# mdolab/dafoam

Hardware: AMD Instinct MI355X
Metric: adjoint_gmres_iterations_per_sec (higher is better)
Workload: dtype f64

## Files before the change

dafoam_amd/_capi.py:

```python
from __future__ import annotations

import ctypes as C
import os

import numpy as np

from .meshgen import FoamCase

_HERE = os.path.dirname(os.path.abspath(__file__))
LIB_PATH = os.environ.get("DAFOAM_AMD_LIB") or os.path.join(_HERE, "lib", "libdafoam_amd.so")

SOLVER_IDS = {"DASimpleFoam": 0, "DAScalarTransportFoam": 1, "DARhoSimpleFoam": 2, "DATurboFoam": 3}
PATCH_TYPES = {"patch": 0, "wall": 1, "symmetry": 2, "cyclic": 3}

c_double_p = C.POINTER(C.c_double)
c_int_p = C.POINTER(C.c_int)
c_ll_p = C.POINTER(C.c_longlong)


class das_case_t(C.Structure):
    _fields_ = [
        ("solver", C.c_int),
        ("n_points", C.c_int),
        ("n_faces", C.c_int),
# ... 193 lines not shown
    "das_op_format_bytes": (C.c_longlong, [_VP]),
    "das_op_export": (C.c_int, [_VP, c_ll_p, c_int_p, c_double_p]),
    "das_calc_drdwold_t_psi": (C.c_int, [_VP, C.c_int, c_double_p, c_double_p]),
    "das_set_old_time_fields": (C.c_int, [_VP, c_double_p, c_double_p]),
    "das_calc_jac_vec_product": (C.c_int, [_VP, c_double_p, c_double_p]),
    "das_set_patch_value": (C.c_int, [_VP, c_int_p, C.c_int, C.c_char_p, c_double_p]),
    "das_get_patch_value": (C.c_int, [_VP, C.c_int, C.c_char_p, c_double_p]),
    "das_set_field": (C.c_int, [_VP, C.c_char_p, c_double_p]),
    "das_get_field": (C.c_int, [_VP, C.c_char_p, c_double_p]),
    "das_calc_dfield_product": (C.c_int, [_VP, C.c_char_p, C.c_char_p, C.c_char_p, c_double_p, c_double_p]),
    "das_calc_dvolcoord_product": (C.c_int, [_VP, C.c_char_p, C.c_char_p, c_double_p, c_double_p, c_double_p]),
    "das_point_influence_build": (C.c_int, [_VP, C.POINTER(C.c_int), C.POINTER(C.c_longlong)]),
    "das_point_influence_get": (C.c_int, [_VP, c_int_p, c_ll_p, c_int_p, c_double_p]),
    "das_debug_device_geometry": (C.c_int, [_VP, c_double_p, c_double_p, c_double_p]),
    "das_debug_strength_aggregates": (C.c_int, [_VP, C.c_int, c_int_p, C.POINTER(C.c_int)]),
    "das_calc_dbc_product": (C.c_int, [_VP, c_int_p, C.c_int, C.c_char_p, c_double_p, C.c_char_p, C.c_char_p, c_double_p, c_double_p]),
    "das_define_force_function": (C.c_int, [_VP, C.c_char_p, c_int_p, C.c_int, c_double_p, C.c_double]),
    "das_define_face_function": (C.c_int, [_VP, C.c_char_p, C.c_char_p, c_int_p, c_int_p, C.c_int, c_double_p, c_double_p, C.c_double, C.c_double]),
    "das_define_patch_field_function": (C.c_int, [_VP, C.c_char_p, C.c_char_p, c_int_p, C.c_int, C.c_char_p, c_int_p, C.c_int, c_double_p, C.c_int, C.c_double, C.c_double]),
    "das_define_cell_function": (C.c_int, [_VP, C.c_char_p, C.c_char_p, c_int_p, C.c_int, C.c_char_p, c_int_p, C.c_int, c_double_p, C.c_int, C.c_double, C.c_double]),
    "das_calc_function": (C.c_int, [_VP, C.c_char_p, c_double_p]),
    "das_get_input_size": (C.c_int, [_VP, C.c_char_p, C.c_char_p]),
    "das_get_output_size": (C.c_int, [_VP, C.c_char_p, C.c_char_p]),
    "das_calc_jac_t_vec_product": (
        C.c_int,
        [_VP, C.c_char_p, C.c_char_p, c_double_p, C.c_char_p, C.c_char_p, c_double_p, c_double_p],
    ),
    "das_drdwt_mult_device": (C.c_int, [_VP, _VP, _VP]),
    "das_create_ml_rksp_matrix_free": (C.c_int, [_VP, _VP, C.POINTER(_VP)]),
    "das_solve_linear_eqn": (C.c_int, [_VP, _VP, c_double_p, c_double_p]),
    "das_solve_linear_eqn_block": (C.c_int, [_VP, _VP, C.c_int, c_double_p, c_double_p, c_double_p, c_double_p]),
    "das_ksp_apply_pc": (C.c_int, [_VP, _VP, c_double_p, c_double_p]),
    "das_ksp_get_n_blocks": (C.c_int, [_VP]),
    "das_ksp_get_factor_nnz": (C.c_longlong, [_VP]),
    "das_ksp_get_n_ext": (C.c_longlong, [_VP]),
    "das_ksp_get_blocks": (C.c_int, [_VP, c_int_p, c_ll_p]),
    "das_pc_structure_build": (C.c_int, [_VP, c_int_p, c_ll_p, c_int_p, c_int_p]),
    "das_pc_structure_get": (C.c_int, [_VP, c_int_p, c_ll_p, c_int_p, c_int_p, c_int_p]),
    "das_ksp_get_pc_structure_sizes": (C.c_int, [_VP, c_int_p, c_ll_p, c_int_p]),
    "das_ksp_get_pc_structure": (C.c_int, [_VP, c_int_p, c_ll_p, c_int_p, c_int_p, c_int_p]),
    "das_ksp_get_info": (C.c_int, [_VP, c_int_p, c_double_p, c_double_p, c_double_p]),
    "das_ksp_get_history": (C.c_int, [_VP, c_double_p, C.c_int]),
    "das_ksp_get_cycle_lengths": (C.c_int, [_VP, c_int_p, C.c_int]),
    "das_ksp_get_basis_info": (C.c_int, [_VP, c_int_p, c_double_p, c_double_p]),
    "das_ksp_get_n_refine": (C.c_int, [_VP]),
    "das_set_dense_eig_callback": (C.c_int, [_VP]),
    "das_debug_gmres_dr_host": (C.c_int, [C.c_longlong, _VP, _VP, _VP, c_double_p, c_double_p, C.c_int, C.c_int, C.c_double, C.c_double, C.c_longlong, c_double_p, C.c_int,
                                          c_double_p, c_double_p]),
    "das_debug_gmres_dr_restart": (C.c_int, [C.c_int, C.c_int, c_double_p, c_double_p, c_double_p, c_double_p, c_double_p]),
    "das_ksp_get_status": (C.c_int, [_VP, c_int_p, c_int_p, c_int_p, c_int_p]),
    "das_ksp_get_pc_stability": (C.c_int, [_VP, C.POINTER(C.c_double), c_int_p]),
    "das_ksp_get_pc_subdomains": (C.c_int, [_VP, c_int_p, c_double_p]),
    "das_ksp_get_pc_node_out": (C.c_int, [_VP, c_int_p]),
    "das_mesh_metrics": (C.c_int, [C.c_int, c_double_p, C.c_int, C.c_int, C.c_int, c_int_p, c_int_p, c_int_p, c_int_p, c_double_p, c_double_p, c_double_p, c_double_p, c_double_p]),
    "das_ksp_get_coarse": (C.c_int, [_VP, c_int_p]),
    "das_ksp_coarse_sparse_az_active": (C.c_int, [_VP]),
    "das_ksp_set_global_coarse": (C.c_int, [_VP, _VP, C.c_int, C.c_int, c_int_p]),
    "das_ksp_run_fixed_device": (C.c_int, [_VP, _VP, _VP, _VP, C.c_int]),
    "das_ksp_begin_device": (C.c_int, [_VP, _VP, _VP, _VP, C.c_int]),
    "das_ksp_advance": (C.c_int, [_VP, _VP, C.c_int]),
    "das_ksp_end": (C.c_int, [_VP, _VP]),
    "das_ksp_destroy": (None, [_VP]),
    "das_set_owned_mask": (C.c_int, [_VP, C.POINTER(C.c_ubyte)]),
    "das_comm_load_rccl": (C.c_int, []),
    "das_comm_unique_id": (C.c_int, [C.c_char_p]),
    "das_comm_init_rccl": (C.c_int, [_VP, C.c_int, C.c_int, C.c_char_p]),
    "das_comm_set_halo": (C.c_int, [_VP, C.c_int, c_int_p, c_ll_p, c_int_p, c_ll_p, c_int_p, C.c_longlong, c_int_p]),
    "das_set_exchange_cb": (C.c_int, [_VP, _VP, _VP]),
    "das_set_pc_overlap": (C.c_int, [_VP, C.POINTER(C.c_ubyte), C.c_int, c_ll_p, c_int_p, c_ll_p, c_int_p]),
    "das_set_gather_cb": (C.c_int, [_VP, _VP, _VP]),
    "das_comm_is_native": (C.c_int, [_VP]),
    "das_comm_reset": (C.c_int, [_VP]),
    "das_set_comm": (C.c_int, [_VP, _VP, _VP, _VP]),
    "das_set_stream": (C.c_int, [_VP, _VP]),
    "das_get_elapsed_clock_time": (C.c_double, [_VP]),
    "das_get_elapsed_cpu_time": (C.c_double, [_VP]),
    "das_timer_avg_ms": (C.c_double, [_VP, C.c_char_p]),
    "das_debug_orth_bench": (C.c_int, [C.c_longlong, C.c_int, C.c_int, C.c_int, C.c_int, C.c_int, C.POINTER(C.c_double), C.POINTER(C.c_double)]),
    "das_debug_orth_bench_split": (C.c_int, [C.c_longlong, C.c_int, C.c_int, C.c_int, C.c_int, C.c_int, C.c_int, C.c_int, C.POINTER(C.c_double), C.POINTER(C.c_double)]),
    "das_debug_set_orth_wide": (C.c_int, [C.c_int, C.POINTER(C.c_int)]),
    "das_debug_krylov_wide_eligible": (C.c_int, [C.c_longlong, C.c_int, C.c_longlong, C.POINTER(C.c_int), C.POINTER(C.c_int)]),
    "das_debug_krylov_dots2": (C.c_int, [C.c_longlong, C.c_int, C.c_int, _VP, C.c_longlong, c_double_p, c_double_p]),
    "das_debug_krylov_dcgs2_update": (C.c_int, [C.c_longlong, C.c_int, C.c_int, _VP, C.c_longlong, C.c_int, c_double_p, C.c_double, C.c_double, c_double_p]),
    "das_debug_krylov_multidot": (C.c_int, [C.c_longlong, C.c_int, C.c_int, _VP, C.c_longlong, c_double_p, c_double_p]),
    "das_debug_krylov_multiaxpy": (C.c_int, [C.c_longlong, C.c_int, C.c_int, _VP, C.c_longlong, c_double_p, C.c_int, _VP, C.c_longlong]),
    "das_debug_krylov_lincomb": (C.c_int, [C.c_longlong, C.c_int, C.c_int, _VP, C.c_longlong, c_double_p, c_double_p, C.c_longlong]),
    "das_debug_krylov_scale_to": (C.c_int, [C.c_longlong, C.c_double, C.c_int, _VP, _VP, C.c_longlong]),
    "das_debug_krylov_block_tn": (C.c_int, [C.c_longlong, C.c_int, C.c_int, c_double_p, C.c_longlong, C.c_longlong, c_double_p, C.c_longlong, c_double_p]),
    "das_debug_krylov_block_nn_sub": (C.c_int, [C.c_longlong, C.c_int, C.c_int, c_double_p, C.c_longlong, c_double_p, c_double_p, C.c_longlong]),
    "das_debug_krylov_block_right_mult": (C.c_int, [C.c_longlong, C.c_int, c_double_p, C.c_longlong, c_double_p]),
    "das_debug_krylov_block_lincomb": (C.c_int, [C.c_longlong, C.c_int, C.c_int, c_double_p, C.c_longlong, c_double_p, c_double_p, C.c_longlong]),
    "das_debug_krylov_block_spmm": (C.c_int, [C.c_longlong, C.c_int, c_ll_p, c_int_p, c_double_p, c_double_p, C.c_longlong, c_double_p, C.c_longlong]),
    "das_timer_count": (C.c_longlong, [_VP, C.c_char_p]),
    "das_timer_reset": (None, [_VP]),
    "das_timer_enable": (None, [_VP, C.c_int]),
}

_lib = None


def declared_symbols():
    return sorted(_SIGS)


def lib():
    global _lib
    if _lib is None:
        if not os.path.exists(LIB_PATH):
            raise ImportError(
                f"{LIB_PATH} not found: build the HIP extension first (python -c 'import __graft_entry__ as g; g.build()'). "
                "dafoam_amd has no CPU fallback."
            )
        L = C.CDLL(LIB_PATH)
        for name, (res, args) in _SIGS.items():
            fn = getattr(L, name)
            fn.restype = res
            fn.argtypes = args
        _lib = L
        _install_dense_eig(L)
    return _lib


_DENSE_EIG_FN = C.CFUNCTYPE(C.c_int, C.c_int, c_double_p, c_double_p, c_double_p, c_double_p, c_double_p)
_dense_eig_keepalive = []


def _install_dense_eig(L):

    def eig(m, A, wr, wi, vr, vi):
        try:
            G = np.ctypeslib.as_array(A, shape=(m * m,)).reshape(m, m)
            w, v = np.linalg.eig(G)
            np.ctypeslib.as_array(wr, shape=(m,))[:] = w.real
            np.ctypeslib.as_array(wi, shape=(m,))[:] = w.imag
            np.ctypeslib.as_array(vr, shape=(m * m,))[:] = np.ascontiguousarray(v.T.real).ravel()
            np.ctypeslib.as_array(vi, shape=(m * m,))[:] = np.ascontiguousarray(v.T.imag).ravel()
            return 0
        except Exception:
            return 1

    cb = _DENSE_EIG_FN(eig)
    _dense_eig_keepalive.append(cb)
    L.das_set_dense_eig_callback(C.cast(cb, C.c_void_p))


class DASError(RuntimeError):
    pass


def check(rc):
    if rc < 0:
        raise DASError(f"dafoam_amd error {rc}: {lib().das_last_error().decode()}")
    return rc


def dptr(a: np.ndarray):
    assert a.dtype == np.float64 and a.flags["C_CONTIGUOUS"]
    return a.ctypes.data_as(c_double_p)
```

dafoam_amd/csrc/das_device.hip:

```cpp
#include <algorithm>
#include <cmath>
#include <ctime>
#include <functional>
#include <numeric>
#include <thread>

#include "das_case.hpp"
#include "das_jaccon.hpp"
#include "das_bilu.hpp"
#include "das_comm.hpp"
#include "das_krylov.hpp"
#include "das_block.hpp"
#include "das_krylov_debug.hpp"
#include "das_color.hpp"
#include "das_opmat.hpp"
#include "das_graph.hpp"
#include "das_volcoord.hpp"
#include "das_cellfn.hpp"
#include "das_simple.hpp"

#include <omp.h>

namespace das {

// ... 395 lines not shown
    if (i >= n0 && i < n1 && w < 1e-14) w = 1e-14;
    Wn[i] = w;
}

__global__ __launch_bounds__(256) void k_coarse_assemble(int nagg, const long long* __restrict__ aptrAll, const int* __restrict__ cellsAll, long long N,
                                                         long long off, const long long* __restrict__ rp, const int* __restrict__ ci,
                                                         const double* __restrict__ v, const int* __restrict__ aggCol, double* __restrict__ E,
                                                         int transpose, double diagScale) {
    __shared__ double accs[2048];
    const int I = blockIdx.x, t = threadIdx.x;
    const long long q0 = aptrAll[I], q1 = aptrAll[I + 1];
    if (q0 == q1) return;
    for (int J = t; J < nagg; J += 256) accs[J] = 0.0;
    for (long long q = q0; q < q1; q++) {
        const long long c = cellsAll[q];
        const long long row = off + c;
        for (long long k = rp[row]; k < rp[row + 1]; k++) {
            const long long j = (long long)ci[k] - off;
            if (j < 0 || j >= N) continue;
            const int J = aggCol[j];
            if (J >= 0 && (J & 255) == t) accs[J] += (j == c) ? v[k] * diagScale : v[k];
        }
    }
    for (int J = t; J < nagg; J += 256) E[transpose ? (long long)J * nagg + I : (long long)I * nagg + J] = accs[J];
}
__global__ __launch_bounds__(256) void k_gj_pivot(int n, int k, double* __restrict__ E, double* __restrict__ Inv, int* __restrict__ singular) {
    __shared__ double bv[256];
    __shared__ int bi[256];
    double best = -1.0;
    int br = k;
    for (int r = k + threadIdx.x; r < n; r += 256) { const double a = fabs(E[(long long)r * n + k]); if (a > best) { best = a; br = r; } }
    bv[threadIdx.x] = best; bi[threadIdx.x] = br;
    __syncthreads();
    for (int o = 128; o > 0; o >>= 1) {
        if ((int)threadIdx.x < o && (bv[threadIdx.x + o] > bv[threadIdx.x] || (bv[threadIdx.x + o] == bv[threadIdx.x] && bi[threadIdx.x + o] < bi[threadIdx.x]))) {
            bv[threadIdx.x] = bv[threadIdx.x + o]; bi[threadIdx.x] = bi[threadIdx.x + o];
        }
        __syncthreads();
    }
    const int pr = bi[0];
    if (!(bv[0] > 0.0)) { if (threadIdx.x == 0) *singular = 1; return; }
    const double ip = 1.0 / E[(long long)pr * n + k];
    __syncthreads();
    for (int q = threadIdx.x; q < n; q += 256) {
        const double ek = E[(long long)k * n + q], ep = E[(long long)pr * n + q];
        const double ik = Inv[(long long)k * n + q], ipr = Inv[(long long)pr * n + q];
        if (pr != k) { E[(long long)pr * n + q] = ek; Inv[(long long)pr * n + q] = ik; }
        E[(long long)k * n + q] = ep * ip;
        Inv[(long long)k * n + q] = ipr * ip;
    }
}
__global__ __launch_bounds__(256) void k_gj_elim(int n, int k, double* __restrict__ E, double* __restrict__ Inv) {
    const int r = blockIdx.x;
    if (r == k) return;
    __shared__ double fs;
    if (threadIdx.x == 0) fs = E[(long long)r * n + k];
    __syncthreads();
    const double f = fs;
    if (f == 0.0) return;
    for (int q = threadIdx.x; q < n; q += 256) {
        E[(long long)r * n + q] -= f * E[(long long)k * n + q];
        Inv[(long long)r * n + q] -= f * Inv[(long long)k * n + q];
    }
}
__global__ __launch_bounds__(256) void k_coarse_restrict(const long long* __restrict__ aptr, const int* __restrict__ cells, long long off,
                                                         const double* __restrict__ r, double* __restrict__ t) {
    __shared__ double red[4];
    const int I = blockIdx.x;
    double acc = 0.0;
    for (long long q = aptr[I] + threadIdx.x; q < aptr[I + 1]; q += 256) acc += r[off + cells[q]];
#pragma unroll
    for (int o = 32; o > 0; o >>= 1) acc += __shfl_down(acc, o, 64);
    if ((threadIdx.x & 63) == 0) red[threadIdx.x >> 6] = acc;
    __syncthreads();
    if (threadIdx.x == 0) t[I] = red[0] + red[1] + red[2] + red[3];
}
__global__ void k_coarse_solve(int nagg, const double* __restrict__ Einv, const double* __restrict__ t, double* __restrict__ u) {
    const int I = blockIdx.x * blockDim.x + threadIdx.x;
    if (I >= nagg) return;
    double acc = 0.0;
    for (int J = 0; J < nagg; J++) acc += Einv[(long long)I * nagg + J] * t[J];
    u[I] = acc;
}
__global__ void k_coarse_prolong(long long N, long long n, long long off, const int* __restrict__ agg, const double* __restrict__ u,
                                 double* __restrict__ y, int set) {
    const long long i = (long long)blockIdx.x * blockDim.x + threadIdx.x;
    if (i >= n) return;
    const long long c = i - off;
    const double add = (c >= 0 && c < N && agg[c] >= 0) ? u[agg[c]] : 0.0;
    y[i] = set ? add : y[i] + add;
}

constexpr int AZ_CAP = 64;
__global__ __launch_bounds__(256) void k_az_build(long long n, const long long* __restrict__ rp, const int* __restrict__ ci, const double* __restrict__ v,
                                                  long long N, long long off, const int* __restrict__ agg, int pass, int* __restrict__ cnt,
                                                  const long long* __restrict__ ptr, int* __restrict__ oa, double* __restrict__ ov, int* __restrict__ overflow) {
    const long long i = (long long)blockIdx.x * blockDim.x + threadIdx.x;
    if (i >= n) return;
    int la[AZ_CAP];
    double ls[AZ_CAP];
    int m = 0;
    for (long long k = rp[i]; k < rp[i + 1]; k++) {
        const long long j = (long long)ci[k] - off;
        if (j < 0 || j >= N) continue;
        const int a = agg[j];
        if (a < 0) continue;
        int q = 0;
        while (q < m && la[q] != a) q++;
        if (q == m) {
            if (m == AZ_CAP) { *overflow = 1; continue; }
            la[m] = a; ls[m] = 0.0; m++;
        }
        ls[q] += v[k];
    }
    if (pass == 0) { cnt[i] = m; return; }
    const long long b = ptr[i];
    for (int q = 0; q < m; q++) { oa[b + q] = la[q]; ov[b + q] = ls[q]; }
}
__global__ __launch_bounds__(256) void k_az_apply(long long n, const long long* __restrict__ ptr, const int* __restrict__ oa, const double* __restrict__ ov,
                                                  const double* __restrict__ u, const double* __restrict__ v, double* __restrict__ out) {
    const long long i = (long long)blockIdx.x * blockDim.x + threadIdx.x;
    if (i >= n) return;
    double acc = 0.0;
    for (long long k = ptr[i]; k < ptr[i + 1]; k++) acc += ov[k] * u[oa[k]];
    out[i] = v ? v[i] - acc : acc;
}

#ifndef PC_THREADS
#define PC_THREADS 1024
#endif
#ifndef PC_PF
#define PC_PF 8
#endif
struct PCView {
    int nBlocks;
    const long long* boff;
    const int* gidx;
    const int* gout;
    const double* invd;
    int factor32;
    const double* sval[2];
    const float* svalf[2];
    const unsigned* srowcol[2];
    const long long* slev[2];
    const long long* slevOff[2];
    double* xglob;
};

#ifndef PC_SEGREDUCE
#define PC_SEGREDUCE 1
#endif
template <int CTRL>
__device__ __forceinline__ unsigned dpp_u32(unsigned v, unsigned old) {
    return (unsigned)__builtin_amdgcn_update_dpp((int)old, (int)v, CTRL, 0xF, 0xF, false);
}
template <int CTRL>
__device__ __forceinline__ double dpp_f64(double v) {
    int lo = __builtin_amdgcn_update_dpp(0, __double2loint(v), CTRL, 0xF, 0xF, false);
    int hi = __builtin_amdgcn_update_dpp(0, __double2hiint(v), CTRL, 0xF, 0xF, false);
    return __hiloint2double(hi, lo);
}
template <bool USE_LDS>
__device__ __forceinline__ void ras_apply_entry(double* xw, double v, unsigned rc, bool valid) {
#if PC_SEGREDUCE
    const unsigned key = valid ? (rc & 0xffffu) : (0x10000u + (threadIdx.x & 63u));
    double val = valid ? -v * xw[rc >> 16] : 0.0;
    unsigned k;
    double w;
    k = dpp_u32<0x111>(key, 0xffffffffu); w = dpp_f64<0x111>(val); if (k == key) val += w;
    k = dpp_u32<0x112>(key, 0xffffffffu); w = dpp_f64<0x112>(val); if (k == key) val += w;
    k = dpp_u32<0x114>(key, 0xffffffffu); w = dpp_f64<0x114>(val); if (k == key) val += w;
    k = dpp_u32<0x118>(key, 0xffffffffu); w = dpp_f64<0x118>(val); if (k == key) val += w;
    const unsigned knext = dpp_u32<0x101>(key, 0xffffffffu);
    if (valid && knext != key) {
        if (USE_LDS) __hip_atomic_fetch_add(&xw[key], val, __ATOMIC_RELAXED, __HIP_MEMORY_SCOPE_WORKGROUP);
        else atomicAdd(&xw[key], val);
    }
#else
    if (!valid) return;
    const double contrib = -v * xw[rc >> 16];
#ifdef PC_EXP_NOATOMIC
    xw[rc & 0xffffu] = contrib;
#else
    if (USE_LDS) __hip_atomic_fetch_add(&xw[rc & 0xffffu], contrib, __ATOMIC_RELAXED, __HIP_MEMORY_SCOPE_WORKGROUP);
    else atomicAdd(&xw[rc & 0xffffu], contrib);
#endif
#endif
}

template <class VT> struct RingVal;
template <> struct RingVal<float> {
    unsigned a;
    __device__ __forceinline__ void load(const float* __restrict__ p, int e) { a = __float_as_uint(p[e]); }
    __device__ __forceinline__ double get() const { return (double)__uint_as_float(a); }
    __device__ __forceinline__ void clear() { a = 0u; }
};
template <> struct RingVal<double> {
    unsigned lo, hi;
    __device__ __forceinline__ void load(const double* __restrict__ p, int e) {
        const unsigned* __restrict__ q = reinterpret_cast<const unsigned*>(p);
        lo = q[2 * (long long)e];
        hi = q[2 * (long long)e + 1];
    }
    __device__ __forceinline__ double get() const { return __hiloint2double((int)hi, (int)lo); }
    __device__ __forceinline__ void clear() { lo = 0u; hi = 0u; }
};

template <bool USE_LDS, class VT>
// ... 83 lines not shown
        if (!on) return;
        hipEvent_t b = get();
        DAS_HIP(hipEventRecord(b, st));
        recs[name].pending.push_back({a, b});
    }
    void resolve() {
        for (auto& kv : recs) {
            for (auto& pr : kv.second.pending) {
                DAS_HIP(hipEventSynchronize(pr.second));
                float ms = 0;
                DAS_HIP(hipEventElapsedTime(&ms, pr.first, pr.second));
                kv.second.ms += ms;
                kv.second.cnt++;
                pool.push_back(pr.first);
                pool.push_back(pr.second);
            }
            kv.second.pending.clear();
        }
    }
    void reset() { resolve(); for (auto& kv : recs) { kv.second.ms = 0; kv.second.cnt = 0; } }
};

struct ConDev {
    bool ready = false;
    bool onDevice = false;
    DevBuf<long long> t_rowptr;
    DevBuf<int> cl_cols;
    DevBuf<int> t_col;
};

struct BlockILU {
    long long n = 0, next = 0;
    int nBlocks = 0;
    long long fnnz = 0;
    int maxLocal = 0;
    DevBuf<long long> boff, slev[2], slevOff[2];
    DevBuf<int> gidx, gout;
    DevBuf<unsigned> srowcol[2];
    DevBuf<double> sval[2], invd, xw;
    DevBuf<float> svalf[2];
    bool factor32 = false;
    PCView view;
    int maxLevels = 0;
    bool useLDS = false;
    double setup_seconds = 0;
    std::vector<int> h_core_perm;
    std::vector<long long> h_core_off;
};

}

using namespace das;

struct das_mat {
    Mat m;
};

struct das_ksp {
    das_mat* pcmat = nullptr;
    BlockILU pc;
    NodeILU bilu;
    bool useBilu = false;
    bool pcTranspose = false;
    double pcDiagScale = 1.0;
    long long shiftExLo = 0, shiftExHi = 0, shiftEnd = (long long)1 << 62;
    struct CoarsePC {
        bool active = false, deflated = false;
        bool global = false;
        int nagg = 0;
        int naggG = 0, aggOff = 0;
        long long off = 0, N = 0;
        DevBuf<int> agg;
        DevBuf<int> aggRow;
        DevBuf<int> cells, cellsAll;
        DevBuf<long long> aptr, aptrAll;
        DevBuf<double> Einv, t, u, c, rr;
        std::vector<int> h_agg;
        DevBuf<long long> azPtr;
        DevBuf<int> azAgg;
        DevBuf<double> azVal;
        long long azOpId = -1;
        long long azEpoch = -1, azNnz = 0;
        bool azReady = false, azFailed = false;
    } coarse;
    int restart = 0;
    VmBuf<double> V;
    long long Vn = 0;
    bool vf32 = false;
    bool split = false;
    DevBuf<double> ustage;
    DevBuf<double> w, z, r, xdev, bdev, partial, hdev, rich_r, rich_d;
    int nSub = 1;
    std::vector<int> subOrder;
    std::vector<double> subEst;
    int pcOrder = -1;
    int pcOrderUsed = -1;
    double pcStability = -1.0;
    bool rasOverlap = false;
    DevBuf<double> pcin;
    std::unique_ptr<struct GmresRun> run;
    std::unique_ptr<struct BlockWork> block;
    std::vector<double> block_res0, block_res;
    int iters = 0, nrefine = 0, reason = 0, nBreakdown = 0;
    double res0 = 0, res = 0, seconds = 0;
    std::vector<double> hist;
    std::vector<int> cycleLens;
};

struct das_solver {
    Mesh mesh;
    CaseParams cp;
    Options opt;
    int device = -1;
    bool inited = false;
    long long n = 0;
    Stencil st_full, st_pc;
    JacCon con_full, con_pc;
    std::vector<int> colors;
    int nColors = 0;
    bool colored = false;
    DevBuf<FaceGeom> d_fg;
    DevBuf<CellGeom> d_cg;
    DevBuf<int> d_cf_ptr, d_cf_face, d_cf_other, d_owner, d_neigh, d_bpatch, d_cyc;
    DevBuf<PatchBC> d_bc;
    DevBuf<double> d_phiF, d_Told;
    DevMesh dm;
    DevBuf<double> d_W, d_R, d_R0, d_Wp, d_scale, d_tmp1, d_tmp2;
    DevBuf<int> d_colors;
    std::vector<double> h_W, h_scale;
    ResWork<double> wk;
    ResWork<Dual<1>> wk1;
    DevBuf<Dual<1>> d_Wd, d_Rd;
    ConDev cd[2];
    std::unique_ptr<das_mat> op;
    std::vector<double> op_states;
    long long op_geom = -1;
    struct FaceFn {
        int kind = DAS_FN_FORCE;
        bool ratio = false;
        double gammaFn = 1.4, RFn = 287.0;
        std::vector<int> faces;
        std::vector<unsigned char> group;
        std::vector<double> w0, dir;
        DevBuf<int> d_faces;
        DevBuf<unsigned char> d_group;
        DevBuf<double> d_w0, d_weff, d_dir, d_fv;
        bool uploaded = false;
        bool isMoment = false;
        double vecA[3] = {0, 0, 0}, vecB[3] = {0, 0, 0}, scale = 1.0;
        long long geomVersion = -1;
        bool refVar = false, geoWeight = false, hasData = true;
        double ref = 0.0;
        int ncomp = 1;
        FaceFnView view(const double* w) const {
            return FaceFnView{d_faces.p, d_group.p, w, dir.empty() ? nullptr : d_dir.p, (int)faces.size(), kind, gammaFn, RFn};
        }
    };
    std::map<std::string, FaceFn> functions;
    struct CellFn {
        bool variance = false, square = false, multiplyVol = true, divByTotalVol = false, refVar = false, geoWeight = false, hasData = true;
        bool field = false;
        double scale = 1.0, ref = 0.0;
        double coef = 0.0, totalVol = 1.0;
        long long geomVersion = -1;
        std::vector<int> cell;
        std::vector<long long> idx;
        std::vector<double> data;
        DevBuf<int> d_cell;
        DevBuf<long long> d_idx;
        DevBuf<double> d_data, d_part, d_unit;
        bool uploaded = false;
        CellFnView view() const {
            return CellFnView{(long long)cell.size(), d_cell.p, d_idx.p, data.empty() ? nullptr : d_data.p, (int)square, (int)multiplyVol};
// ... 956 lines not shown
    }
    auto fill_mask = [&](const std::vector<unsigned char>& cellIn, std::vector<unsigned char>& out) {
        out.assign(n, 0);
        for (const StateDef& sd : s->st_full.states) {
            if (sd.kind == KIND_VEC) { for (long long c = 0; c < N; c++) if (cellIn[c]) { out[sd.offset + 3 * c] = out[sd.offset + 3 * c + 1] = out[sd.offset + 3 * c + 2] = 1; } }
            else if (sd.kind == KIND_SCL) { for (long long c = 0; c < N; c++) if (cellIn[c]) out[sd.offset + c] = 1; }
            else { for (long long f = 0; f < m.nF; f++) if (cellIn[m.owner[f]]) out[sd.offset + f] = 1; }
        }
    };
    std::vector<unsigned char> subOf(n, 0);
    for (const StateDef& sd : s->st_full.states) {
        if (sd.kind == KIND_VEC) { for (long long c = 0; c < N; c++) for (int q = 0; q < 3; q++) subOf[sd.offset + 3 * c + q] = (unsigned char)blockOf[c]; }
        else if (sd.kind == KIND_SCL) { for (long long c = 0; c < N; c++) subOf[sd.offset + c] = (unsigned char)blockOf[c]; }
        else { for (long long f = 0; f < m.nF; f++) subOf[sd.offset + f] = (unsigned char)blockOf[m.owner[f]]; }
    }
    const int overlap = (int)std::max<long long>(0, s->opt.geti("adjEqnOption.asmOverlap"));
    std::vector<std::vector<unsigned char>> masks(K);
    k->subOrder.assign(K, -1);
    k->subEst.assign(K, -1.0);
    for (int b = 0; b < K; b++) {
        std::vector<unsigned char> cellIn(N, 0), grown;
        for (long long c = 0; c < N; c++) cellIn[c] = blockOf[c] == b;
        for (int ring = 0; ring < overlap; ring++) {
            grown = cellIn;
            for (long long c = 0; c < N; c++) if (cellIn[c]) for (int q = m.cc_ptr[c]; q < m.cc_ptr[c + 1]; q++) grown[m.cc[q]] = 1;
            cellIn.swap(grown);
        }
        fill_mask(cellIn, masks[b]);
        NodeILU F;
        choose_order_and_factorise(s, k, F, masks[b], true, k->subOrder[b], k->subEst[b]);
        if (k->subOrder[b] < 0) k->subOrder[b] = k->pcOrder >= 0 ? k->pcOrder : (pc_ordering_rcm(s) ? 1 : 0);
        if (s->opt.geti("debug") || getenv("DAS_PC_STAB"))
            fprintf(stderr, "[dafoam_amd] sub-domain %d of %d: %d nodes, %d levels, elimination order %d, stability estimate %.3e\n", b, K, F.nNodes, F.nLevels, k->subOrder[b], k->subEst[b]);
        if ((double)F.nLevels > 30.0 * std::cbrt((double)std::max(1, F.nNodes)) && s->opt.geti("amd.pcSubdomains") < 0) {
            fprintf(stderr, "[dafoam_amd] sub-domain %d of %d needs %d dependency levels for %d nodes: the blocks do not suit this mesh, one factorisation instead "
                            "(amd.pcSubdomains K > 1 forces the blocks)\n", b, K, F.nLevels, F.nNodes);
            k->subOrder.clear(); k->subEst.clear();
            return false;
        }
    }
    {
        const Mat& A = k->pcmat->m;
        const int reach = pc_stencil_reach(s);
        const int nthr = (int)std::max<long long>(1, std::min<long long>(das::host_threads(), s->opt.geti("amd.setupThreads")));
        double dir[3];
        pc_flow_direction(s, dir);
        std::vector<const std::vector<unsigned char>*> mp;
        for (int b = 0; b < K; b++) mp.push_back(&masks[b]);
        k->bilu = NodeILU();
        bilu_setup_multi(s->mesh, s->st_full.states, n, mp, k->subOrder, subOf, reach, s->opt.geti("amd.pcFactorFP32") != 0, A.n, A.rowptr.p, A.col.p, A.val.p, s->stream, k->bilu,
                         s->opt.geti("debug") != 0, nthr, dir);
    }
    k->nSub = K;
    k->useBilu = true;
    k->rasOverlap = false;
    k->pcOrderUsed = k->subOrder[0];
    k->pcStability = 0.0;
    for (double e : k->subEst) k->pcStability = std::max(k->pcStability, e);
    k->pc.setup_seconds = wall_seconds() - t0;
    k->pc.nBlocks = K;
    k->pc.fnnz = (k->bilu.nL + k->bilu.nU + k->bilu.nNodes) * (long long)BILU_NB2;
    k->pc.next = (long long)k->bilu.nNodes * BILU_NB;
    if (s->opt.geti("debug") || getenv("DAS_PC_STAB"))
        fprintf(stderr, "[dafoam_amd] %d sub-domains merged: %d nodes, %d levels (%.0f nodes per level)\n", K, k->bilu.nNodes, k->bilu.nLevels, (double)k->bilu.nNodes / std::max(1, k->bilu.nLevels));
    return true;
}

static void coarse_build_operator(das_solver* s, das_ksp* k, int naggG, int aggOff, const std::vector<int>& aggRowG) {
    das_ksp::CoarsePC& C = k->coarse;
    C.active = false;
    DAS_CHECK(naggG >= C.nagg && naggG <= 2048, DAS_ERR_ARG, "coarse space: at most 2048 aggregates in total (dense inverse)");
    const long long N = C.N;
    std::vector<int> aggOwn(N, -1);
    for (long long c = 0; c < N; c++) if (C.h_agg[c] >= 0) aggOwn[c] = aggOff + C.h_agg[c];
    std::vector<long long> aptrAll(naggG + 1, 0);
    for (long long c = 0; c < N; c++) if (aggRowG[c] >= 0) aptrAll[aggRowG[c] + 1]++;
    for (int a = 0; a < naggG; a++) aptrAll[a + 1] += aptrAll[a];
    std::vector<int> cellsAll(aptrAll[naggG]);
    {
        std::vector<long long> pos(aptrAll.begin(), aptrAll.end() - 1);
        for (long long c = 0; c < N; c++) if (aggRowG[c] >= 0) cellsAll[pos[aggRowG[c]]++] = (int)c;
    }
    C.naggG = naggG; C.aggOff = aggOff; C.global = naggG > C.nagg;
    C.azOpId = -1; C.azReady = false;
    C.agg.upload(aggOwn); C.aggRow.upload(aggRowG); C.cellsAll.upload(cellsAll); C.aptrAll.upload(aptrAll);
    DevBuf<double> E((size_t)naggG * naggG);
    E.zero();
    const Mat& P = k->pcmat->m;
    hipLaunchKernelGGL(k_coarse_assemble, dim3(naggG), dim3(256), 0, s->stream, naggG, C.aptrAll.p, C.cellsAll.p, N, C.off, P.rowptr.p, P.col.p, P.val.p,
                       k->pcTranspose ? C.aggRow.p : C.agg.p, E.p, k->pcTranspose ? 1 : 0,
                       (C.off < k->shiftEnd && !(C.off >= k->shiftExLo && C.off < k->shiftExHi)) ? k->pcDiagScale : 1.0);
    if (C.global) {
        DAS_CHECK(!k->pcTranspose, DAS_ERR_ARG, "global coarse space: adjoint preconditioner only");
        rank_allreduce(s, E.p, naggG * naggG, s->stream);
    }
    {
        std::vector<double> I0((size_t)naggG * naggG, 0.0);
        for (int i = 0; i < naggG; i++) I0[(size_t)i * naggG + i] = 1.0;
        C.Einv.upload(I0);
        DevBuf<int> sing(1);
        DAS_HIP(hipMemsetAsync(sing.p, 0, sizeof(int), s->stream));
        for (int kk = 0; kk < naggG; kk++) {
            hipLaunchKernelGGL(k_gj_pivot, dim3(1), dim3(256), 0, s->stream, naggG, kk, E.p, C.Einv.p, sing.p);
            hipLaunchKernelGGL(k_gj_elim, dim3(naggG), dim3(256), 0, s->stream, naggG, kk, E.p, C.Einv.p);
        }
        int hs = 0;
        DAS_HIP(hipMemcpyAsync(&hs, sing.p, sizeof(int), hipMemcpyDeviceToHost, s->stream));
        DAS_HIP(hipStreamSynchronize(s->stream));
        if (hs) return;
    }
    C.t.alloc(naggG); C.u.alloc(naggG);
    C.active = true;
}

static void setup_coarse(das_solver* s, das_ksp* k) {
    das_ksp::CoarsePC& C = k->coarse;
    C.active = false;
    long long want = s->opt.geti("amd.pcCoarseAggregates");
    if (want == 0) return;
    const std::string field = s->opt.gets("amd.pcCoarseField");
    const StateDef* sd = nullptr;
    for (const StateDef& q : s->st_full.states) if (q.name == field && q.kind == KIND_SCL) sd = &q;
    if (!sd) return;
    const Mesh& m = s->mesh;
    const long long N = m.nC;
    std::vector<int> owned;
    owned.reserve(N);
    for (long long c = 0; c < N; c++) if (s->owned.empty() || s->owned[sd->offset + c]) owned.push_back((int)c);
    if (owned.size() < 64) return;
    if (want < 0) want = std::min<long long>(1024, std::max<long long>(16, (long long)owned.size() / 2048));
    int nagg = (int)std::min<long long>(want, std::min<long long>(2048, (long long)owned.size() / 4));
    if (nagg < 2) return;
    std::vector<int> agg(N, -1);
    const bool byStrength = s->opt.gets("amd.pcCoarseAggregation") == "strength";
    DAS_CHECK(byStrength || s->opt.gets("amd.pcCoarseAggregation") == "rcb", DAS_ERR_ARG, "amd.pcCoarseAggregation: rcb | strength");
    if (byStrength) {
        std::vector<unsigned char> mask;
        if (!s->owned.empty()) { mask.resize(N); for (long long c = 0; c < N; c++) mask[c] = s->owned[sd->offset + c]; }
        nagg = strength_aggregates(m, s->owned.empty() ? nullptr : &mask, nagg, agg);
        if (nagg < 2) return;
    } else {
        struct Rg { long long b, e; int a0, na; };
        std::vector<Rg> stack{{0, (long long)owned.size(), 0, nagg}};
        while (!stack.empty()) {
            Rg r = stack.back();
            stack.pop_back();
            if (r.na == 1) { for (long long q = r.b; q < r.e; q++) agg[owned[q]] = r.a0; continue; }
            double lo[3] = {1e300, 1e300, 1e300}, hi[3] = {-1e300, -1e300, -1e300};
            for (long long q = r.b; q < r.e; q++)
                for (int d = 0; d < 3; d++) { const double x = m.cg[owned[q]].C[d]; lo[d] = std::min(lo[d], x); hi[d] = std::max(hi[d], x); }
            int ax = 0;
            for (int d = 1; d < 3; d++) if (hi[d] - lo[d] > hi[ax] - lo[ax]) ax = d;
            const int nl = r.na / 2;
            const long long mid = r.b + (r.e - r.b) * nl / r.na;
            std::nth_element(owned.begin() + r.b, owned.begin() + mid, owned.begin() + r.e, [&](int a, int b2) {
                const double xa = m.cg[a].C[ax], xb = m.cg[b2].C[ax];
                return xa < xb || (xa == xb && a < b2);
            });
            stack.push_back({mid, r.e, r.a0 + nl, r.na - nl});
            stack.push_back({r.b, mid, r.a0, nl});
        }
    }
    std::vector<long long> aptr(nagg + 1, 0);
    for (long long c = 0; c < N; c++) if (agg[c] >= 0) aptr[agg[c] + 1]++;
    for (int a = 0; a < nagg; a++) aptr[a + 1] += aptr[a];
    std::vector<int> cells(aptr[nagg]);
    {
        std::vector<long long> pos(aptr.begin(), aptr.end() - 1);
        for (long long c = 0; c < N; c++) if (agg[c] >= 0) cells[pos[agg[c]]++] = (int)c;
    }
    C.nagg = nagg; C.off = sd->offset; C.N = N; C.h_agg = agg;
    C.cells.upload(cells); C.aptr.upload(aptr);
    C.deflated = s->opt.gets("amd.pcCoarseMode") == "deflated";
    if (C.deflated) { C.c.alloc(s->n); C.rr.alloc(s->n); }
    coarse_build_operator(s, k, nagg, 0, agg);
    if (C.active && s->opt.geti("debug")) fprintf(stderr, "[dafoam_amd] coarse space: %d aggregates on field %s (%s)\n", nagg, field.c_str(), C.deflated ? "deflated" : "additive");
}
static void coarse_solve(das_solver* s, das_ksp* k, const double* r) {
    das_ksp::CoarsePC& C = k->coarse;
    if (C.global) DAS_HIP(hipMemsetAsync(C.t.p, 0, (size_t)C.naggG * sizeof(double), s->stream));
    if (C.nagg > 0) hipLaunchKernelGGL(k_coarse_restrict, dim3(C.nagg), dim3(256), 0, s->stream, C.aptr.p, C.cells.p, C.off, r, C.t.p + C.aggOff);
    if (C.global) rank_allreduce(s, C.t.p, C.naggG, s->stream);
    hipLaunchKernelGGL(k_coarse_solve, dim3(nblk(C.naggG, 64)), dim3(64), 0, s->stream, C.naggG, C.Einv.p, C.t.p, C.u.p);
}

static void pc_apply(das_solver* s, das_ksp* k, const double* b, double* x) {
    hipEvent_t ev = nullptr;
    s->timer.begin("pc", s->stream, ev);
    if (k->useBilu) {
        if (k->rasOverlap) {
            DAS_HIP(hipMemcpyAsync(k->pcin.p, b, (size_t)s->n * sizeof(double), hipMemcpyDeviceToDevice, s->stream));
            s->halo.gather_overlap(k->pcin.p, s->stream);
            bilu_apply(k->bilu, k->pcin.p, x, s->stream);
            s->halo.zero_overlap(x, s->stream);
        } else {
            bilu_apply(k->bilu, b, x, s->stream);
        }
        s->timer.end("pc", s->stream, ev);
        return;
    }
    const int mlv = k->pc.maxLevels;
    const size_t lvlBytes = (size_t)((mlv + 2 * PC_PF + 4) >> 1) * sizeof(double);
    if (k->pc.useLDS)
        hipLaunchKernelGGL(k_ras_apply<true>, dim3(k->pc.nBlocks), dim3(PC_THREADS), lvlBytes + (size_t)k->pc.maxLocal * sizeof(double), s->stream,
                           k->pc.view, b, x, mlv);
    else
        hipLaunchKernelGGL(k_ras_apply<false>, dim3(k->pc.nBlocks), dim3(PC_THREADS), lvlBytes, s->stream, k->pc.view, b, x, mlv);
    s->timer.end("pc", s->stream, ev);
}

static void gmres_ws(das_solver* s, das_ksp* k) {
    const long long n = s->n;
    long long restart = std::min<long long>(s->opt.geti("adjEqnOption.gmresRestart"), s->opt.geti("adjEqnOption.gmresMaxIters"));
    long long budget = (long long)(32.0 * 1024 * 1024 * 1024);
    auto it = s->opt.i.find("amd.maxKrylovBytes");
    if (it != s->opt.i.end()) budget = it->second;
    const long long nr = (n + 3) / 4 * 4;
    const long long maxVec = std::max<long long>(3, budget / (8 * nr));
    restart = std::max<long long>(1, std::min<long long>(restart, maxVec - 2));
    long long wantVec = std::max<long long>(restart + 2, std::min<long long>(maxVec, 1002));
    if ((size_t)wantVec * (size_t)nr * sizeof(double) < ((size_t)4 << 30) || getenv("DAS_NO_VMM")) wantVec = restart + 2;
    if (k->V.n < (size_t)((restart + 2) * nr) || k->Vn != n) {
        k->V.reserve((size_t)(wantVec * nr));
        k->Vn = n;
    }
    {
        std::string prec = "auto";
        { auto ip = s->opt.s.find("amd.krylovBasisPrecision"); if (ip != s->opt.s.end()) prec = ip->second; }
        DAS_CHECK(prec == "auto" || prec == "fp64" || prec == "fp32" || prec == "split", DAS_ERR_ARG, "amd.krylovBasisPrecision: auto | fp64 | split | fp32");
        const bool eligible = s->opt.geti("adjEqnOption.useMGSO") == 0 && !s->fwd.on;
        const bool dcgs2 = s->opt.gets("amd.gmresOrthogonalization") == "dcgs2" && s->opt.geti("adjEqnOption.useMGSO") == 0;
        bool big = (size_t)(restart + 2) * (size_t)n * 8 >= ((size_t)1 << 30);
        if (s->halo.active || s->allreduce_cb) {
            DevBuf<double> f(1);
            const double fv = big ? 1.0 : 0.0;
            DAS_HIP(hipMemcpyAsync(f.p, &fv, sizeof(double), hipMemcpyHostToDevice, s->stream));
            rank_allreduce(s, f.p, 1, s->stream);
            DAS_HIP(hipStreamSynchronize(s->stream));
            big = f.to_host()[0] > 0.5;
        }
        k->split = eligible && (prec == "split" || (prec == "auto" && dcgs2 && big));
        k->vf32 = k->split || (eligible && prec == "fp32");
        if (k->vf32 && k->ustage.n != (size_t)n) k->ustage.alloc(n);
    }
    if (k->restart != restart || k->w.n != (size_t)n) {
        k->restart = (int)restart;
        k->w.alloc(n); k->z.alloc(n); k->r.alloc(n); k->xdev.alloc(n); k->bdev.alloc(n);
        k->z.zero();
        k->partial.alloc(std::max<size_t>(multidot_partial_size(n, (int)restart + 1), multidot2_partial_size(n, (int)restart + 2)));
        k->hdev.alloc(4 * (restart + 3));
    }
}
static inline long long basis_n4(das_solver* s) { return (s->n + 3) / 4 * 4; }
static inline long long basis_ld(das_solver* s, das_ksp* k) { return k->split ? 2 * basis_n4(s) : (k->vf32 ? basis_n4(s) : s->n); }
static inline bool gmres_map_basis(das_solver* s, das_ksp* k, long long nvec) {
    const long long per = basis_ld(s, k) / (k->vf32 ? 2 : 1);
    k->V.request((size_t)((nvec + 64) * per));
    return k->V.try_ensure((size_t)(nvec * per));
}
template <class VT>
static inline VT* basis_slot(das_solver* s, das_ksp* k, long long j) { return reinterpret_cast<VT*>(k->V.p) + j * basis_ld(s, k); }
static inline float* basis_lo(das_solver* s, das_ksp* k, long long j) { return k->split ? reinterpret_cast<float*>(k->V.p) + j * basis_ld(s, k) + basis_n4(s) : nullptr; }

template <class VT>
static void multidot_dev(das_solver* s, das_ksp* k, const VT* Vbase, int m, const double* w, double* dev_out) {
    launch_multidot<VT>(s->stream, s->n, m, Vbase, basis_ld(s, k), w, k->partial.p, dev_out);
    rank_allreduce(s, dev_out, m + 1, s->stream);
}
template <class VT = double>
static void multidot(das_solver* s, das_ksp* k, int m, const double* w, double* h_host) {
    multidot_dev<VT>(s, k, basis_slot<VT>(s, k, 0), m, w, k->hdev.p);
    DAS_HIP(hipMemcpyAsync(h_host, k->hdev.p, (m + 1) * sizeof(double), hipMemcpyDeviceToHost, s->stream));
    DAS_HIP(hipStreamSynchronize(s->stream));
}

static void apply_operator(das_solver* s, const double* x, double* y);

static bool coarse_az_ready(das_solver* s, das_ksp* k) {
    das_ksp::CoarsePC& C = k->coarse;
    if (!s->op || s->fwd.on) return false;
    { auto it = s->opt.i.find("amd.pcCoarseSparseAZ"); if (it != s->opt.i.end() && it->second == 0) return false; }
    const Mat& A = s->op->m;
    if (C.azOpId == s->opId && C.azEpoch == s->op_epoch) return C.azReady;
    C.azOpId = s->opId; C.azEpoch = s->op_epoch; C.azReady = false; C.azFailed = false;
    const long long n = s->n;
    hipStream_t st = s->stream;
    DevBuf<int> cnt(n), ovf(1);
    DAS_HIP(hipMemsetAsync(ovf.p, 0, sizeof(int), st));
    hipLaunchKernelGGL(k_az_build, dim3(nblk(n, 256)), dim3(256), 0, st, n, A.rowptr.p, A.col.p, A.val.p, C.N, C.off, C.agg.p, 0, cnt.p, (const long long*)nullptr,
                       (int*)nullptr, (double*)nullptr, ovf.p);
    DAS_HIP(hipStreamSynchronize(st));
    int ovfAny = ovf.to_host()[0];
    if (s->halo.active || s->allreduce_cb) {
        DevBuf<double> f(1);
        const double fv = ovfAny ? 1.0 : 0.0;
        DAS_HIP(hipMemcpyAsync(f.p, &fv, sizeof(double), hipMemcpyHostToDevice, st));
        rank_allreduce(s, f.p, 1, st);
        DAS_HIP(hipStreamSynchronize(st));
        ovfAny = f.to_host()[0] > 0.5 ? 1 : 0;
    }
    if (ovfAny) {
        C.azFailed = true;
        fprintf(stderr, "[dafoam_amd] deflated coarse mode: a row of the operator touches more than %d aggregates - keeping the full operator product per apply\n", AZ_CAP);
        return false;
    }
    std::vector<int> h = cnt.to_host();
    std::vector<long long> ptr(n + 1, 0);
    for (long long i = 0; i < n; i++) ptr[i + 1] = ptr[i] + h[i];
    C.azNnz = ptr[n];
    C.azPtr.upload(ptr);
    C.azAgg.alloc((size_t)std::max<long long>(1, C.azNnz)); C.azVal.alloc((size_t)std::max<long long>(1, C.azNnz));
    hipLaunchKernelGGL(k_az_build, dim3(nblk(n, 256)), dim3(256), 0, st, n, A.rowptr.p, A.col.p, A.val.p, C.N, C.off, C.agg.p, 1, cnt.p, C.azPtr.p, C.azAgg.p, C.azVal.p,
                       ovf.p);
    DAS_HIP(hipStreamSynchronize(st));
    if (s->opt.geti("debug")) fprintf(stderr, "[dafoam_amd] deflated coarse mode: sparse A Z with %lld entries (%.2f per row)\n", C.azNnz, (double)C.azNnz / (double)n);
    C.azReady = true;
    return true;
}

static void pc_apply_full(das_solver* s, das_ksp* k, const double* v, double* z) {
    const long long sweeps = std::max<long long>(1, s->opt.geti("adjEqnOption.globalPCIters")) * std::max<long long>(1, s->opt.geti("adjEqnOption.localPCIters"));
    const long long n = s->n;
    das_ksp::CoarsePC& C = k->coarse;
    if (C.active) {
        hipEvent_t ev = nullptr;
        s->timer.begin("coarse", s->stream, ev);
        coarse_solve(s, k, v);
        if (C.deflated && (s->op || s->fwd.on)) {
            hipLaunchKernelGGL(k_coarse_prolong, dim3(nblk(n, 256)), dim3(256), 0, s->stream, C.N, n, C.off, C.agg.p, C.u.p, C.c.p, 1);
            if (coarse_az_ready(s, k)) {
                if (s->halo.active || s->halo_cb) {
                    hipLaunchKernelGGL(k_az_apply, dim3(nblk(n, 256)), dim3(256), 0, s->stream, n, C.azPtr.p, C.azAgg.p, C.azVal.p, C.u.p, (const double*)nullptr, C.rr.p);
                    if (s->halo.active) s->halo.reduce_vector(C.rr.p, s->stream);
                    else s->halo_cb(C.rr.p, s->comm_user);
                    hipLaunchKernelGGL(k_axpby, dim3(nblk(n, 256)), dim3(256), 0, s->stream, n, 1.0, v, -1.0, C.rr.p);
                } else {
                    hipLaunchKernelGGL(k_az_apply, dim3(nblk(n, 256)), dim3(256), 0, s->stream, n, C.azPtr.p, C.azAgg.p, C.azVal.p, C.u.p, v, C.rr.p);
                }
                s->timer.end("coarse", s->stream, ev);
            } else {
                s->timer.end("coarse", s->stream, ev);
                apply_operator(s, C.c.p, C.rr.p);
                hipLaunchKernelGGL(k_axpby, dim3(nblk(n, 256)), dim3(256), 0, s->stream, n, 1.0, v, -1.0, C.rr.p);
            }
            pc_apply(s, k, C.rr.p, z);
            hipLaunchKernelGGL(k_axpby, dim3(nblk(n, 256)), dim3(256), 0, s->stream, n, 1.0, C.c.p, 1.0, z);
        } else {
            s->timer.end("coarse", s->stream, ev);
            pc_apply(s, k, v, z);
            hipLaunchKernelGGL(k_coarse_prolong, dim3(nblk(n, 256)), dim3(256), 0, s->stream, C.N, n, C.off, C.agg.p, C.u.p, z, 0);
        }
    } else {
        pc_apply(s, k, v, z);
    }
    if (sweeps <= 1) return;
    if (k->rich_r.n != (size_t)n) { k->rich_r.alloc(n); k->rich_d.alloc(n); k->rich_d.zero(); }
    const Mat& P = k->pcmat->m;
    for (long long it = 1; it < sweeps; it++) {
        hipLaunchKernelGGL(k_spmv_wave, SPMV_GRID(P.n), dim3(256), 0, s->stream, P.n, P.rowptr.p, P.col.p, P.val.p, z, k->rich_r.p);
        hipLaunchKernelGGL(k_axpby, dim3(nblk(n, 256)), dim3(256), 0, s->stream, n, 1.0, v, -1.0, k->rich_r.p);
        pc_apply(s, k, k->rich_r.p, k->rich_d.p);
        hipLaunchKernelGGL(k_axpby, dim3(nblk(n, 256)), dim3(256), 0, s->stream, n, 1.0, k->rich_d.p, 1.0, z);
    }
}

static void pc_apply_block(das_solver* s, das_ksp* k, const double* V, double* Z, int sv) {
    const long long n = s->n;
    const long long sweeps = std::max<long long>(1, s->opt.geti("adjEqnOption.globalPCIters")) * std::max<long long>(1, s->opt.geti("adjEqnOption.localPCIters"));
    das_ksp::CoarsePC& C = k->coarse;
    const bool batched = k->useBilu && sweeps <= 1 && !(C.active && C.deflated) && sv > 1 && s->opt.geti("amd.blockBatchedPC") != 0;
    if (!batched) {
        for (int r = 0; r < sv; r++) pc_apply_full(s, k, V + (size_t)r * n, Z + (size_t)r * n);
        return;
    }
    hipEvent_t ev = nullptr;
    s->timer.begin("pc", s->stream, ev);
    bilu_apply_multi(k->bilu, V, Z, n, sv, s->stream);
    s->timer.end("pc", s->stream, ev);
    if (C.active)
        for (int r = 0; r < sv; r++) {
            coarse_solve(s, k, V + (size_t)r * n);
            hipLaunchKernelGGL(k_coarse_prolong, dim3(nblk(n, 256)), dim3(256), 0, s->stream, C.N, n, C.off, C.agg.p, C.u.p, Z + (size_t)r * n, 0);
        }
}

static void apply_operator(das_solver* s, const double* x, double* y) {
    if (!s->fwd.on) { spmv(s, s->op->m, x, y); return; }
    const long long n = s->n;
    const int B = 256;
    hipStream_t st = s->stream;
    hipEvent_t ev = nullptr;
    s->timer.begin("jvp", st, ev);
    ResParams prm = make_params(s->cp, s->opt, 0);
    if (s->d_Wd.n != (size_t)n) { s->d_Wd.alloc(n); s->d_Rd.alloc(n); }
    hipLaunchKernelGGL(k_seed_dir, dim3(nblk(n, B)), dim3(B), 0, st, n, s->d_W.p, s->d_scale.p, x, s->d_Wd.p);
    eval_residual<Dual<1>>(s->dm, s->cp, prm, s->d_Wd.p, s->d_Rd.p, s->wk1, s->d_phiF.p, s->d_Told.p, st);
    hipLaunchKernelGGL(k_tangent_out, dim3(nblk(n, B)), dim3(B), 0, st, n, s->d_Rd.p, y);
    if (s->fwd.invTau != 0.0) hipLaunchKernelGGL(k_add_diag_prod, dim3(nblk(n, B)), dim3(B), 0, st, n, s->fwd.invTau, s->fwd.diag.p, x, y);
    s->timer.end("jvp", st, ev);
}

struct GmresRun {
    bool open = false;
    bool fixed = false;
    int m = 0, j = 0;
    bool memWarned = false;
    long long its = 0, maxIts = 0;
    double beta = 0, target = 0, rtol = 0, atol = 0, t0 = 0;
    double recTarget = 0;
    const double* d_rhs = nullptr;
    double* d_x = nullptr;
    std::vector<double> H, cs, sn, g, hh, h2, y;
    bool dcgs2 = false;
    int pend = 0;
    std::vector<double> Hraw, h1;
    bool earlyClose = false;
    bool safeOrth = false;
    bool stalled = false;
    int nonImproving = 0, nBreakdown = 0;
    double betaStart = 0;
};
static bool gmres_trace() { static const bool on = [] { const char* e = getenv("DAS_GMRES_TRACE"); return e && *e && *e != '0'; }(); return on; }
static constexpr double GMRES_BREAKDOWN_TOL = 1e-13;

static void gmres_true_residual(das_solver* s, das_ksp* k, GmresRun& G, bool haveGuess) {
    const long long n = s->n;
    hipStream_t st = s->stream;
    if (haveGuess) {
        apply_operator(s, G.d_x, k->r.p);
        hipLaunchKernelGGL(k_axpby, dim3(nblk(n, 256)), dim3(256), 0, st, n, 1.0, G.d_rhs, -1.0, k->r.p);
    } else {
        DAS_HIP(hipMemsetAsync(G.d_x, 0, n * sizeof(double), st));
        DAS_HIP(hipMemcpyAsync(k->r.p, G.d_rhs, n * sizeof(double), hipMemcpyDeviceToDevice, st));
    }
    multidot(s, k, 0, k->r.p, G.hh.data());
    G.beta = std::sqrt(G.hh[0]);
}

static void gmres_begin(das_solver* s, das_ksp* k, const double* d_rhs, double* d_x, bool fixed) {
    need_init(s);
    DAS_CHECK(s->op || s->fwd.on, DAS_ERR_STATE, "initializedRdWTMatrixFree() must be called before solveLinearEqn()");
    gmres_ws(s, k);
    if (k->useBilu) bilu_clear_abort(k->bilu, s->stream);
    if (!k->run) k->run.reset(new GmresRun);
    GmresRun& G = *k->run;
    const int m = k->restart;
    G = GmresRun();
    G.m = m; G.fixed = fixed; G.d_rhs = d_rhs; G.d_x = d_x;
    G.maxIts = s->opt.geti("adjEqnOption.gmresMaxIters");
    G.rtol = s->opt.getd("adjEqnOption.gmresRelTol"); G.atol = s->opt.getd("adjEqnOption.gmresAbsTol");
    G.H.assign((size_t)(m + 1) * m, 0.0); G.cs.assign(m, 0.0); G.sn.assign(m, 0.0); G.g.assign(m + 1, 0.0);
    G.hh.assign(2 * (m + 2), 0.0); G.h2.assign(2 * (m + 2), 0.0); G.y.assign(m, 0.0);
    const std::string& orth = s->opt.gets("amd.gmresOrthogonalization");
    DAS_CHECK(orth == "dcgs2" || orth == "cgs", DAS_ERR_ARG, "amd.gmresOrthogonalization \"" + orth + "\" is not one of dcgs2 | cgs");
    G.dcgs2 = orth == "dcgs2" && s->opt.geti("adjEqnOption.useMGSO") == 0;
    if (G.dcgs2) { G.Hraw.assign((size_t)(m + 1) * m, 0.0); G.h1.assign(m + 2, 0.0); }
    k->nrefine = 0;
    k->hist.clear();
    k->cycleLens.clear();
    G.t0 = wall_seconds();
    gmres_true_residual(s, k, G, s->opt.geti("adjEqnOption.useNonZeroInitGuess") != 0);
    k->res0 = G.beta;
    k->hist.push_back(G.beta);
    G.target = std::max(G.rtol * G.beta, G.atol);
    G.recTarget = k->split ? 0.98 * G.target : (k->vf32 ? 0.5 * G.target : G.target);
}
static void gmres_cycle_start(das_solver* s, das_ksp* k) {
    GmresRun& G = *k->run;
    const long long n = s->n;
    DAS_CHECK(gmres_map_basis(s, k, 3), DAS_ERR_INTERNAL, "GMRES: no device memory for three Krylov vectors (" + k->V.workerError + ")");
    if (k->vf32) launch_scale_to(s->stream, n, 1.0 / G.beta, (const double*)k->r.p, basis_slot<float>(s, k, 0), (const float*)nullptr, basis_lo(s, k, 0));
    else launch_scale_to(s->stream, n, 1.0 / G.beta, (const double*)k->r.p, (double*)k->V.p, (const float*)nullptr, (float*)nullptr);
    std::fill(G.g.begin(), G.g.end(), 0.0);
    G.g[0] = G.beta;
    G.j = 0;
    G.pend = 0;
    G.open = true;
    G.earlyClose = false;
    G.betaStart = G.beta;
}
template <class VT>
static const double* basis_as_double(das_solver* s, das_ksp* k, long long j) {
    if (sizeof(VT) == sizeof(double)) return reinterpret_cast<const double*>(basis_slot<VT>(s, k, j));
    launch_scale_to(s->stream, s->n, 1.0, (const VT*)basis_slot<VT>(s, k, j), (double*)k->ustage.p, (const float*)basis_lo(s, k, j), (float*)nullptr);
    return k->ustage.p;
}
template <class VT>
static double gmres_iter_dcgs2(das_solver* s, das_ksp* k);
template <class VT>
static double gmres_iter_t(das_solver* s, das_ksp* k) {
    GmresRun& G = *k->run;
    if (G.dcgs2 && !G.safeOrth) return gmres_iter_dcgs2<VT>(s, k);
    const long long n = s->n;
    const int B = 256, m = G.m, j = G.j;
    hipStream_t st = s->stream;
    const bool alwaysRefine = s->opt.geti("amd.cgsAlwaysRefine") != 0;
    const bool mgs = s->opt.geti("adjEqnOption.useMGSO") != 0;
    std::vector<double>&H = G.H, &hh = G.hh, &h2 = G.h2, &cs = G.cs, &sn = G.sn, &g = G.g;
    VT* const Vb = basis_slot<VT>(s, k, 0);
    const long long ld = basis_ld(s, k);
    pc_apply_full(s, k, basis_as_double<VT>(s, k, j), k->z.p);
    apply_operator(s, k->z.p, k->w.p);
    double hn;
    std::fill(h2.begin(), h2.end(), 0.0);
    if (mgs) {
        double* hcol = k->hdev.p + (m + 2);
        for (int i = 0; i <= j; i++) {
            multidot_dev<VT>(s, k, Vb + (long long)i * ld, 1, k->w.p, k->hdev.p);
            DAS_HIP(hipMemcpyAsync(hcol + i, k->hdev.p, sizeof(double), hipMemcpyDeviceToDevice, st));
            launch_multiaxpy(st, n, 1, (const VT*)(Vb + (long long)i * ld), ld, (const double*)k->hdev.p, (double*)k->w.p, (const float*)basis_lo(s, k, i));
        }
        multidot_dev<VT>(s, k, Vb, 0, k->w.p, k->hdev.p);
        DAS_HIP(hipMemcpyAsync(hcol + j + 1, k->hdev.p, sizeof(double), hipMemcpyDeviceToDevice, st));
        DAS_HIP(hipMemcpyAsync(hh.data(), hcol, (j + 2) * sizeof(double), hipMemcpyDeviceToHost, st));
        DAS_HIP(hipStreamSynchronize(st));
        hn = std::sqrt(std::max(hh[j + 1], 0.0));
    } else {
        multidot<VT>(s, k, j + 1, k->w.p, hh.data());
        launch_multiaxpy(st, n, j + 1, (const VT*)Vb, ld, (const double*)k->hdev.p, (double*)k->w.p, (const float*)basis_lo(s, k, 0));
        double hsq = 0.0;
        for (int i = 0; i <= j; i++) hsq += hh[i] * hh[i];
        const double ww = hh[j + 1];
        const double est = ww - hsq;
        if (alwaysRefine || !(est > hsq) || !(est > 0.0)) {
            multidot<VT>(s, k, j + 1, k->w.p, h2.data());
            launch_multiaxpy(st, n, j + 1, (const VT*)Vb, ld, (const double*)k->hdev.p, (double*)k->w.p, (const float*)basis_lo(s, k, 0));
            double hn2;
            multidot<VT>(s, k, 0, k->w.p, &hn2);
            hn = std::sqrt(std::max(hn2, 0.0));
            k->nrefine++;
        } else {
            hn = std::sqrt(est);
        }
    }
    if (!mgs && !(hn > GMRES_BREAKDOWN_TOL * std::sqrt(std::max(hh[j + 1], 0.0)))) { hn = 0.0; G.nBreakdown++; }
    for (int i = 0; i <= j; i++) H[(size_t)i * m + j] = hh[i] + h2[i];
    H[(size_t)(j + 1) * m + j] = hn;
    if (hn > 0.0) launch_scale_to(st, n, 1.0 / hn, (const double*)k->w.p, Vb + (long long)(j + 1) * ld, (const float*)nullptr, basis_lo(s, k, j + 1));
    for (int i = 0; i < j; i++) {
        double a = H[(size_t)i * m + j], b2 = H[(size_t)(i + 1) * m + j];
        H[(size_t)i * m + j] = cs[i] * a + sn[i] * b2;
        H[(size_t)(i + 1) * m + j] = -sn[i] * a + cs[i] * b2;
    }
    double a = H[(size_t)j * m + j], b2 = H[(size_t)(j + 1) * m + j];
    double d = std::hypot(a, b2);
    cs[j] = d > 0 ? a / d : 1.0;
    sn[j] = d > 0 ? b2 / d : 0.0;
    H[(size_t)j * m + j] = d;
    H[(size_t)(j + 1) * m + j] = 0.0;
    g[j + 1] = -sn[j] * g[j];
    g[j] = cs[j] * g[j];
    G.its++;
    G.j++;
    const double res = std::fabs(g[G.j]);
    k->hist.push_back(res);
    if (hn == 0.0) { G.j = -G.j; G.earlyClose = true; }
    return res;
}
static double gmres_iter(das_solver* s, das_ksp* k) { return k->vf32 ? gmres_iter_t<float>(s, k) : gmres_iter_t<double>(s, k); }
static double gmres_rotate_column(GmresRun& G, int col) {
    const int m = G.m;
    std::vector<double>&H = G.H, &cs = G.cs, &sn = G.sn, &g = G.g;
    for (int i = 0; i < col; i++) {
        const double a = H[(size_t)i * m + col], b2 = H[(size_t)(i + 1) * m + col];
        H[(size_t)i * m + col] = cs[i] * a + sn[i] * b2;
        H[(size_t)(i + 1) * m + col] = -sn[i] * a + cs[i] * b2;
    }
    const double a = H[(size_t)col * m + col], b2 = H[(size_t)(col + 1) * m + col];
    const double d = std::hypot(a, b2);
    cs[col] = d > 0 ? a / d : 1.0;
    sn[col] = d > 0 ? b2 / d : 0.0;
    H[(size_t)col * m + col] = d;
    H[(size_t)(col + 1) * m + col] = 0.0;
    g[col + 1] = -sn[col] * g[col];
    g[col] = cs[col] * g[col];
    return std::fabs(g[col + 1]);
}
template <class VT>
static double gmres_iter_dcgs2(das_solver* s, das_ksp* k) {
    GmresRun& G = *k->run;
    const long long n = s->n;
    const int m = G.m, j = G.pend;
    hipStream_t st = s->stream;
    VT* const Vb = basis_slot<VT>(s, k, 0);
    const long long ld = basis_ld(s, k);
    VT* u = Vb + (long long)j * ld;
    pc_apply_full(s, k, basis_as_double<VT>(s, k, j), k->z.p);
    apply_operator(s, k->z.p, k->w.p);
    const int K = j + 1;
    launch_multidot2<VT>(st, n, K, (const VT*)Vb, ld, (const VT*)u, (const double*)k->w.p, k->partial.p, k->hdev.p);
    rank_allreduce(s, k->hdev.p, 2 * K, st);
    std::vector<double>& o = G.hh;
    DAS_HIP(hipMemcpyAsync(o.data(), k->hdev.p, 2 * K * sizeof(double), hipMemcpyDeviceToHost, st));
    DAS_HIP(hipStreamSynchronize(st));
    const double* sv = o.data();
    const double* tv = o.data() + K;
    const double uu = sv[j], uv = tv[j];
    double ss = 0.0, stt = 0.0;
    for (int i = 0; i < j; i++) { ss += sv[i] * sv[i]; stt += sv[i] * tv[i]; }
    double al2 = uu - ss, num = uv - stt;
    double normBq2 = uu;
    for (int i = 0; i < j; i++) normBq2 += G.h1[i] * G.h1[i];
    bool explicitProj = false;
    if (j > 0 && !(ss <= 1e-2 * uu)) {
        if (gmres_trace()) fprintf(stderr, "[dafoam_amd] dcgs2 step %d: s.s / u.u = %.3e > 1e-2: explicit projection, cycle closes\n", j, ss / uu);
        double* dsc = k->hdev.p + 2 * (m + 3);
        DAS_HIP(hipMemcpyAsync(dsc, sv, j * sizeof(double), hipMemcpyHostToDevice, st));
        if (k->split) {
            const double* ud = basis_as_double<VT>(s, k, j);
            launch_multiaxpy(st, n, j, (const VT*)Vb, ld, (const double*)dsc, const_cast<double*>(ud), (const float*)basis_lo(s, k, 0));
            launch_scale_to(st, n, 1.0, ud, u, (const float*)nullptr, basis_lo(s, k, j));
        } else {
            launch_multiaxpy(st, n, j, (const VT*)Vb, ld, (const double*)dsc, u, (const float*)nullptr);
        }
        launch_multidot2<VT>(st, n, 1, (const VT*)u, ld, (const VT*)u, (const double*)k->w.p, k->partial.p, k->hdev.p);
        rank_allreduce(s, k->hdev.p, 2, st);
        double cc[2] = {0.0, 0.0};
        DAS_HIP(hipMemcpyAsync(cc, k->hdev.p, 2 * sizeof(double), hipMemcpyDeviceToHost, st));
        DAS_HIP(hipStreamSynchronize(st));
        al2 = cc[0]; num = cc[1];
        explicitProj = true;
        k->nrefine++;
    }
    const bool breakdown = !(al2 > GMRES_BREAKDOWN_TOL * GMRES_BREAKDOWN_TOL * normBq2);
    const double al = breakdown ? 0.0 : std::sqrt(al2);
    double res = k->hist.back();
    if (j == 0) {
        DAS_CHECK(!breakdown, DAS_ERR_INTERNAL, "GMRES: the start vector of an Arnoldi cycle is not finite (preconditioner or operator returned NaN)");
        G.g[0] = G.beta * al;
    } else {
        const int col = j - 1;
        for (int i = 0; i < j; i++) G.Hraw[(size_t)i * m + col] = G.H[(size_t)i * m + col] = G.h1[i] + (breakdown ? 0.0 : sv[i]);
        G.Hraw[(size_t)j * m + col] = G.H[(size_t)j * m + col] = al;
        res = gmres_rotate_column(G, col);
        G.its++;
        G.j = j;
        k->hist.push_back(res);
        if (breakdown || explicitProj) {
            if (breakdown) G.nBreakdown++; else G.safeOrth = true;
            G.j = -G.j; G.earlyClose = true;
            return res;
        }
        const bool stop = !G.fixed && (res <= G.recTarget || G.its >= G.maxIts);
        if (stop || G.j >= m) return res;
    }
    const double gam = num / al2;
    std::vector<double>& co = G.h2;
    for (int i = 0; i < j; i++) { co[i] = sv[i]; co[j + i] = tv[i] - gam * sv[i]; }
    double* dco = k->hdev.p + 2 * (m + 3);
    if (j > 0) DAS_HIP(hipMemcpyAsync(dco, co.data(), 2 * j * sizeof(double), hipMemcpyHostToDevice, st));
    launch_dcgs2_update<DCGS2_UNROLL, DCGS2_RPT, VT>(st, n, j, Vb, ld, (const double*)dco, gam, 1.0 / al, (const double*)k->w.p, basis_lo(s, k, 0));
    for (int i = 0; i < j; i++) {
        double a = tv[i];
        for (int q = std::max(0, i - 1); q < j; q++) a -= G.Hraw[(size_t)i * m + q] * sv[q];
        G.h1[i] = a / al;
    }
    G.h1[j] = gam - (j > 0 ? sv[j - 1] : 0.0);
    G.pend = j + 1;
    return res;
}
template <class VT>
static void gmres_cycle_end_t(das_solver* s, das_ksp* k) {
    GmresRun& G = *k->run;
    const long long n = s->n;
    const int B = 256, m = G.m, j = std::abs(G.j);
    hipStream_t st = s->stream;
    for (int i = j - 1; i >= 0; i--) {
        double sacc = G.g[i];
        for (int q = i + 1; q < j; q++) sacc -= G.H[(size_t)i * m + q] * G.y[q];
        G.y[i] = sacc / G.H[(size_t)i * m + i];
    }
    DAS_HIP(hipMemcpyAsync(k->hdev.p, G.y.data(), j * sizeof(double), hipMemcpyHostToDevice, st));
    launch_lincomb(st, n, j, (const VT*)basis_slot<VT>(s, k, 0), basis_ld(s, k), (const double*)k->hdev.p, (double*)k->w.p, (const float*)basis_lo(s, k, 0));
    pc_apply_full(s, k, k->w.p, k->z.p);
    hipLaunchKernelGGL(k_axpby, dim3(nblk(n, B)), dim3(B), 0, st, n, 1.0, k->z.p, 1.0, G.d_x);
    const double recRes = k->hist.back();
    gmres_true_residual(s, k, G, true);
    k->hist.back() = G.beta;
    k->cycleLens.push_back(j);
    G.open = false;
    if (gmres_trace()) {
        double ymax = 0.0;
        for (int i = 0; i < j; i++) ymax = std::max(ymax, std::fabs(G.y[i]));
        fprintf(stderr, "[dafoam_amd] GMRES cycle closed after %d columns (its %lld): recurrence |r| %.6e, true |r| %.6e (|r0| %.3e), max |y| %.3e, explicit projections %d, basis %s%s\n",
                j, G.its, recRes, G.beta, k->res0, ymax, k->nrefine, k->split ? "split" : (k->vf32 ? "fp32" : "fp64"), G.safeOrth ? ", two-pass scheme from here" : "");
    }
}
static void gmres_cycle_end(das_solver* s, das_ksp* k) {
    if (k->vf32) gmres_cycle_end_t<float>(s, k); else gmres_cycle_end_t<double>(s, k);
}
static bool gmres_over(const GmresRun& G) { return !G.fixed && !G.open && (G.beta <= G.target || G.its >= G.maxIts || G.stalled); }
static bool gmres_advance(das_solver* s, das_ksp* k, long long nsteps) {
    GmresRun& G = *k->run;
    for (long long t = 0; t < nsteps; t++) {
        if (gmres_over(G)) return true;
        if (G.beta == 0.0) return true;
        if (!G.open) gmres_cycle_start(s, k);
        const long long wantSlots = std::min<long long>(((G.dcgs2 && !G.safeOrth) ? G.pend : G.j) + 3, (long long)G.m + 2);
        if (!gmres_map_basis(s, k, wantSlots)) {
            if (k->V.workerError.empty())
                k->V.workerError = "request for " + std::to_string(wantSlots) + " basis vectors beyond the reserved range of " + std::to_string(k->V.n / (size_t)std::max<long long>(1, s->n)) + " (internal)";
            DAS_CHECK(G.j >= 1, DAS_ERR_INTERNAL, "GMRES: the Krylov basis cannot grow beyond its first vectors (" + k->V.workerError + ")");
            if (!G.memWarned) fprintf(stderr, "[dafoam_amd] GMRES restarts after %d vectors: %s\n", G.j, k->V.workerError.c_str());
            G.memWarned = true;
            gmres_cycle_end(s, k);
            t--;
            continue;
        }
        const double res = gmres_iter(s, k);
        const bool stop = !G.fixed && (res <= G.recTarget || G.its >= G.maxIts);
        if (G.j < 0 || G.j >= G.m || stop) {
            const bool judged = G.earlyClose || (res <= G.recTarget && G.its < G.maxIts);
            gmres_cycle_end(s, k);
            if (!G.fixed && judged && G.beta > G.target) {
                if (G.beta < 0.5 * G.betaStart) G.nonImproving = 0;
                else if (++G.nonImproving >= 2) G.stalled = true;
            }
        }
    }
    return gmres_over(G);
}
static int gmres_end(das_solver* s, das_ksp* k) {
    GmresRun& G = *k->run;
    if (G.open) gmres_cycle_end(s, k);
    DAS_HIP(hipStreamSynchronize(s->stream));
    if (k->useBilu) DAS_CHECK(!bilu_aborted(k->bilu, s->stream), DAS_ERR_INTERNAL, "preconditioner sweep timed out (bounded spin)");
    k->iters = (int)G.its;
    k->nBreakdown = G.nBreakdown;
    k->res = k->hist.back();
    k->reason = G.beta <= G.target ? 0 : (G.stalled ? 2 : 1);
    k->seconds = wall_seconds() - G.t0;
    double absRatio = k->res / G.atol;
    double relRatio = k->res0 > 0 ? k->res / k->res0 / G.rtol : 0.0;
    double diff = s->opt.getd("adjEqnOption.gmresTolDiff");
// ... 2251 lines not shown
    DAS_CATCH
}
int das_drdwt_mult_device(das_solver_t* s, const double* d_x, double* d_y) {
    DAS_TRY
    need_init(s);
    DAS_CHECK(s->op, DAS_ERR_STATE, "initializedRdWTMatrixFree() has not been called");
    spmv(s, s->op->m, d_x, d_y);
    return DAS_OK;
    DAS_CATCH
}

int das_create_ml_rksp_matrix_free(das_solver_t* s, das_mat_t* pc, das_ksp_t** ksp) {
    DAS_TRY
    need_init(s);
    DAS_CHECK(pc && ksp, DAS_ERR_ARG, "null argument");
    std::unique_ptr<das_ksp> k(new das_ksp);
    k->pcmat = pc;
    const std::string pcType = s->opt.gets("amd.pcType");
    DAS_CHECK(pcType == "bilu" || pcType == "ras", DAS_ERR_ARG, "amd.pcType must be \"bilu\" or \"ras\"");
    if (pcType == "bilu") {
        if (getenv("DAS_BILU_ORDER")) k->pcOrder = atoi(getenv("DAS_BILU_ORDER"));
        const long long K = pc_subdomain_count(s);
        if (!(K > 1 && setup_subdomain_ilus(s, k.get(), (int)K))) {
            const double t0 = wall_seconds();
            choose_order_and_factorise(s, k.get(), k->bilu, (s->pcMask.empty() || k->pcTranspose) ? s->owned : s->pcMask, !s->owned.empty(), k->pcOrderUsed, k->pcStability,  s->owned.empty());
            if (k->pcOrderUsed >= 0) k->pcOrder = k->pcOrderUsed;
            k->useBilu = true;
            k->rasOverlap = !s->pcMask.empty() && !k->pcTranspose && s->halo.ovActive;
            if (k->rasOverlap && k->pcin.n != (size_t)s->n) k->pcin.alloc(s->n);
            k->pc.setup_seconds = wall_seconds() - t0;
            k->pc.nBlocks = 1;
            k->pc.fnnz = (k->bilu.nL + k->bilu.nU + k->bilu.nNodes) * (long long)BILU_NB2;
            k->pc.next = (long long)k->bilu.nNodes * BILU_NB;
        }
    } else setup_block_ilu(s, k.get());
    setup_coarse(s, k.get());
    *ksp = k.release();
    return DAS_OK;
    DAS_CATCH
}
int das_solve_linear_eqn(das_solver_t* s, das_ksp_t* ksp, const double* rhs, double* sol) {
    DAS_TRY
    need_init(s);
    DAS_CHECK(ksp && rhs && sol, DAS_ERR_ARG, "null argument");
    gmres_ws(s, ksp);
    ksp->bdev.upload(rhs, s->n);
    ksp->xdev.upload(sol, s->n);
    int rc = run_gmres(s, ksp, ksp->bdev.p, ksp->xdev.p, 0);
    ksp->xdev.download(sol, s->n);
    if (s->opt.geti("adjEqnOption.printInfo"))
        fprintf(stderr, "Main iteration %d KSP Residual norm %14.12e %.2f s\n", ksp->iters, ksp->res, ksp->seconds);
    return rc;
    DAS_CATCH
}
int das_solve_linear_eqn_block(das_solver_t* s, das_ksp_t* ksp, int nrhs, const double* rhs, double* sol, double* res0, double* res) {
    DAS_TRY
    need_init(s);
    DAS_CHECK(ksp && rhs && sol && nrhs >= 1, DAS_ERR_ARG, "bad argument");
    DevBuf<double> dB((size_t)nrhs * s->n), dX((size_t)nrhs * s->n);
    dB.upload(rhs, (size_t)nrhs * s->n);
    int rc = run_block_gmres(s, ksp, nrhs, dB.p, dX.p);
    dX.download(sol, (size_t)nrhs * s->n);
    for (int r = 0; r < nrhs; r++) { if (res0) res0[r] = ksp->block_res0[r]; if (res) res[r] = ksp->block_res[r]; }
    if (s->opt.geti("adjEqnOption.printInfo"))
        fprintf(stderr, "Block solve (%d systems): iteration %d max KSP Residual norm %14.12e %.2f s\n", nrhs, ksp->iters, ksp->res, ksp->seconds);
    return rc;
    DAS_CATCH
}
int das_ksp_apply_pc(das_solver_t* s, das_ksp_t* ksp, const double* x, double* y) {
    DAS_TRY
    need_init(s);
    DAS_CHECK(ksp && x && y, DAS_ERR_ARG, "null argument");
    DevBuf<double> dx(s->n), dy(s->n);
    dx.upload(x, s->n);
    DAS_HIP(hipDeviceSynchronize());
    dy.zero();
    pc_apply_full(s, ksp, dx.p, dy.p);
    DAS_HIP(hipStreamSynchronize(s->stream));
    if (ksp->useBilu) DAS_CHECK(!bilu_aborted(ksp->bilu, s->stream), DAS_ERR_INTERNAL, "preconditioner sweep timed out (bounded spin)");
    dy.download(y, s->n);
    return DAS_OK;
    DAS_CATCH
}
static void copy_pc_structure(const NodeILU& P, int* nodeUnk, long long* bptr, int* bcol, int* lvlPtr, int* natural) {
    if (natural) std::copy(P.h_natural.begin(), P.h_natural.end(), natural);
    if (nodeUnk) std::copy(P.h_nodeUnk.begin(), P.h_nodeUnk.end(), nodeUnk);
    if (bptr) std::copy(P.h_bptr.begin(), P.h_bptr.end(), bptr);
    if (bcol) std::copy(P.h_bcol.begin(), P.h_bcol.end(), bcol);
    if (lvlPtr) std::copy(P.h_lvlPtr.begin(), P.h_lvlPtr.end(), lvlPtr);
}
int das_pc_structure_build(das_solver_t* s, int* nNodes, long long* nBlocks, int* nLevels, int* reach) {
    DAS_TRY
    DAS_CHECK(s, DAS_ERR_ARG, "null solver handle");
    const int rch = pc_stencil_reach(s);
    std::vector<char> cellOwned(s->mesh.nC, 1);
    if (!s->owned.empty()) {
        const StateDef& s0 = s->st_full.states[0];
        const int stride = s0.kind == KIND_VEC ? 3 : 1;
        for (int c = 0; c < s->mesh.nC; c++) cellOwned[c] = s->owned[s0.offset + (long long)stride * c] ? 1 : 0;
    }
    std::vector<int> unkNode, bcol;
    std::vector<unsigned char> unkSlot;
    std::vector<long long> bptr, bdiag;
    const int nthr = (int)std::max<long long>(1, std::min<long long>(das::host_threads(), s->opt.geti("amd.setupThreads")));
    bilu_build_structure(s->mesh, s->st_full.states, s->n, s->owned, cellOwned, rch, s->pcStruct, unkNode, unkSlot, bptr, bdiag, bcol, nthr, pc_ordering_rcm(s));
    if (nNodes) *nNodes = s->pcStruct.nNodes;
    if (nBlocks) *nBlocks = s->pcStruct.nnzB;
    if (nLevels) *nLevels = s->pcStruct.nLevels;
    if (reach) *reach = rch;
    return DAS_OK;
    DAS_CATCH
}
int das_pc_structure_get(das_solver_t* s, int* nodeUnk, long long* bptr, int* bcol, int* lvlPtr, int* natural) {
    DAS_TRY
    DAS_CHECK(s && s->pcStruct.nNodes > 0, DAS_ERR_STATE, "das_pc_structure_build has not been called");
    copy_pc_structure(s->pcStruct, nodeUnk, bptr, bcol, lvlPtr, natural);
    return DAS_OK;
    DAS_CATCH
}
int das_ksp_get_pc_structure_sizes(das_ksp_t* ksp, int* nNodes, long long* nBlocks, int* nLevels) {
    DAS_TRY
    DAS_CHECK(ksp && ksp->useBilu, DAS_ERR_STATE, "the KSP does not hold a node-block ILU preconditioner (amd.pcType \"bilu\")");
    if (nNodes) *nNodes = ksp->bilu.nNodes;
    if (nBlocks) *nBlocks = ksp->bilu.nnzB;
    if (nLevels) *nLevels = ksp->bilu.nLevels;
    return DAS_OK;
    DAS_CATCH
}
int das_ksp_get_pc_structure(das_ksp_t* ksp, int* nodeUnk, long long* bptr, int* bcol, int* lvlPtr, int* natural) {
    DAS_TRY
    DAS_CHECK(ksp && ksp->useBilu, DAS_ERR_STATE, "the KSP does not hold a node-block ILU preconditioner (amd.pcType \"bilu\")");
    copy_pc_structure(ksp->bilu, nodeUnk, bptr, bcol, lvlPtr, natural);
    return DAS_OK;
    DAS_CATCH
}
int das_ksp_get_pc_node_out(das_ksp_t* ksp, int* nodeOut) {
    DAS_TRY
    DAS_CHECK(ksp && ksp->useBilu && nodeOut, DAS_ERR_STATE, "the KSP does not hold a node-block ILU preconditioner (amd.pcType \"bilu\")");
    const std::vector<int>& src = ksp->bilu.h_nodeOut.empty() ? ksp->bilu.h_nodeUnk : ksp->bilu.h_nodeOut;
    std::copy(src.begin(), src.end(), nodeOut);
    return DAS_OK;
    DAS_CATCH
}
int das_ksp_get_n_blocks(das_ksp_t* ksp) { return ksp ? ksp->pc.nBlocks : -1; }
long long das_ksp_get_factor_nnz(das_ksp_t* ksp) { return ksp ? ksp->pc.fnnz : -1; }
long long das_ksp_get_n_ext(das_ksp_t* ksp) { return ksp ? ksp->pc.next : -1; }
int das_ksp_get_blocks(das_ksp_t* ksp, int* perm, long long* block_off) {
    DAS_TRY
    DAS_CHECK(ksp && perm && block_off, DAS_ERR_ARG, "null argument");
    DAS_CHECK(!ksp->useBilu, DAS_ERR_STATE, "das_ksp_get_blocks describes the \"ras\" preconditioner; use das_ksp_get_pc_structure");
    std::copy(ksp->pc.h_core_perm.begin(), ksp->pc.h_core_perm.end(), perm);
    std::copy(ksp->pc.h_core_off.begin(), ksp->pc.h_core_off.end(), block_off);
    return DAS_OK;
    DAS_CATCH
}
int das_ksp_get_info(das_ksp_t* k, int* iters, double* res0, double* res, double* seconds) {
    DAS_TRY
    DAS_CHECK(k, DAS_ERR_ARG, "null ksp");
    if (iters) *iters = k->iters;
    if (res0) *res0 = k->res0;
    if (res) *res = k->res;
    if (seconds) *seconds = k->seconds;
    return DAS_OK;
    DAS_CATCH
}
int das_set_dense_eig_callback(void* fn) { g_dense_eig = (das_dense_eig_fn)fn; return DAS_OK; }
int das_debug_gmres_dr_restart(int m, int kwant, const double* Hbar, const double* rvec, double* P1, double* Hnew, double* cnew) {
    DAS_TRY
    DAS_CHECK(m >= 2 && kwant >= 1 && Hbar && rvec && P1 && Hnew && cnew, DAS_ERR_ARG, "bad argument");
    std::vector<double> Hb(Hbar, Hbar + (size_t)(m + 1) * m), rv(rvec, rvec + m + 1), p, h, c;
    int kk = 0;
    if (gmres_dr_restart_host(m, kwant, Hb, rv, kk, p, h, c) != 0) return -1;
    std::copy(p.begin(), p.end(), P1); std::copy(h.begin(), h.end(), Hnew); std::copy(c.begin(), c.end(), cnew);
    return kk;
    DAS_CATCH
}
int das_debug_gmres_dr_host(long long n, void* A, void* M, void* user, const double* b, double* x, int m, int kdef, double rtol, double atol,
                            long long maxIts, double* hist, int histCap, double* info4, double* res2) {
    DAS_TRY
    DAS_CHECK(n > 0 && A && M && b && x && m >= 4, DAS_ERR_ARG, "bad argument");
    DrHostOps ops{n, (das_host_apply_fn)A, (das_host_apply_fn)M, user, b, x, std::vector<double>((size_t)(m + 2) * n, 0.0), std::vector<double>(n), std::vector<double>(n), std::vector<double>(n), m};
    std::fill(x, x + n, 0.0);
    const double beta0 = ops.true_residual();
    std::vector<double> h{beta0};
    const double target = std::max(rtol * beta0, atol);
    const DrResult R = gmres_dr_loop(ops, m, kdef, beta0, target, maxIts, h);
    if (hist) for (int i = 0; i < histCap && i < (int)h.size(); i++) hist[i] = h[i];
    if (info4) { info4[0] = (double)R.its; info4[1] = R.nDeflated; info4[2] = R.nRestarts; info4[3] = R.nBreakdown; }
    if (res2) { res2[0] = R.res0; res2[1] = R.res; }
    const double absRatio = R.res / atol, relRatio = beta0 > 0 ? R.res / beta0 / rtol : 0.0;
    return (relRatio > 1e2 && absRatio > 1e2) ? 1 : 0;
    DAS_CATCH
}
int das_ksp_get_n_refine(das_ksp_t* k) { return k ? k->nrefine : -1; }
int das_ksp_get_status(das_ksp_t* k, int* reason, int* nBreakdown, int* nSweepGrid, int* sweepPerXcd) {
    DAS_TRY
    DAS_CHECK(k, DAS_ERR_ARG, "null ksp handle");
    if (reason) *reason = k->reason;
    if (nBreakdown) *nBreakdown = k->nBreakdown;
    if (nSweepGrid) *nSweepGrid = k->useBilu ? k->bilu.launchGrid : 0;
    if (sweepPerXcd) *sweepPerXcd = k->useBilu ? k->bilu.launchPerXcd : 0;
    return DAS_OK;
    DAS_CATCH
}
int das_ksp_get_pc_stability(das_ksp_t* k, double* estimate, int* orderUsed) {
    DAS_TRY
    DAS_CHECK(k, DAS_ERR_ARG, "null ksp handle");
    if (estimate) *estimate = k->pcStability;
    if (orderUsed) *orderUsed = k->pcOrderUsed;
    return DAS_OK;
    DAS_CATCH
}
int das_ksp_get_pc_subdomains(das_ksp_t* k, int* orders, double* estimates) {
    if (!k) return -1;
    for (int b = 0; b < k->nSub && k->nSub > 1; b++) {
        if (orders) orders[b] = k->subOrder[b];
        if (estimates) estimates[b] = k->subEst[b];
    }
    return k->nSub;
}
int das_ksp_coarse_sparse_az_active(das_ksp_t* k) { return k ? (k->coarse.active && k->coarse.deflated && k->coarse.azReady ? 1 : 0) : -1; }
int das_ksp_get_coarse(das_ksp_t* k, int* aggOfCell) {
    if (!k || !k->coarse.active) return 0;
    if (aggOfCell) std::copy(k->coarse.h_agg.begin(), k->coarse.h_agg.end(), aggOfCell);
    return k->coarse.nagg;
}
int das_ksp_set_global_coarse(das_solver_t* s, das_ksp_t* k, int naggGlobal, int aggOffset, const int* aggRowGlobal) {
    DAS_TRY
    need_init(s);
    DAS_CHECK(k && aggRowGlobal, DAS_ERR_ARG, "null argument");
    das_ksp::CoarsePC& C = k->coarse;
    DAS_CHECK(C.N > 0 && !C.h_agg.empty(), DAS_ERR_STATE, "the preconditioner of this KSP has no coarse space (amd.pcCoarseAggregates)");
    DAS_CHECK(aggOffset >= 0 && aggOffset + C.nagg <= naggGlobal, DAS_ERR_ARG, "aggregate offset out of range");
    std::vector<int> rows(aggRowGlobal, aggRowGlobal + C.N);
    for (long long c = 0; c < C.N; c++) {
        DAS_CHECK(rows[c] >= -1 && rows[c] < naggGlobal, DAS_ERR_ARG, "global aggregate id out of range");
        if (C.h_agg[c] >= 0) DAS_CHECK(rows[c] == aggOffset + C.h_agg[c], DAS_ERR_ARG, "owned cells must carry offset + local aggregate");
    }
    coarse_build_operator(s, k, naggGlobal, aggOffset, rows);
    if (C.active) return DAS_OK;
    coarse_build_operator(s, k, C.nagg, 0, C.h_agg);
    return 1;
    DAS_CATCH
}
int das_ksp_get_history(das_ksp_t* k, double* hist, int cap) {
    DAS_TRY
    DAS_CHECK(k && hist, DAS_ERR_ARG, "null argument");
    int m = std::min<int>(cap, (int)k->hist.size());
    std::copy(k->hist.begin(), k->hist.begin() + m, hist);
    return m;
    DAS_CATCH
}
int das_ksp_get_basis_info(das_ksp_t* k, int* fp32, double* mappedBytes, double* bytesPerVector) {
    DAS_TRY
    DAS_CHECK(k, DAS_ERR_ARG, "null argument");
    if (fp32) *fp32 = ((k->vf32 && !k->split) ? 1 : 0) | (k->split ? 2 : 0);
    if (mappedBytes) *mappedBytes = (double)k->V.mappedBytes;
    if (bytesPerVector) *bytesPerVector = k->vf32 ? (double)((k->Vn + 3) / 4 * 4) * (k->split ? 8.0 : 4.0) : (double)k->Vn * 8.0;
    return DAS_OK;
    DAS_CATCH
}
int das_ksp_get_cycle_lengths(das_ksp_t* k, int* lens, int cap) {
    DAS_TRY
    DAS_CHECK(k && (lens || cap == 0), DAS_ERR_ARG, "null argument");
    int m = std::min<int>(cap, (int)k->cycleLens.size());
    std::copy(k->cycleLens.begin(), k->cycleLens.begin() + m, lens);
    return (int)k->cycleLens.size();
    DAS_CATCH
}
int das_ksp_run_fixed_device(das_solver_t* s, das_ksp_t* ksp, const double* d_rhs, double* d_sol, int iters) {
    DAS_TRY
    DAS_CHECK(ksp && d_rhs && d_sol && iters > 0, DAS_ERR_ARG, "bad argument");
    return run_gmres(s, ksp, d_rhs, d_sol, iters);
    DAS_CATCH
}
int das_ksp_begin_device(das_solver_t* s, das_ksp_t* ksp, const double* d_rhs, double* d_sol, int fixed) {
    DAS_TRY
    DAS_CHECK(ksp && d_rhs && d_sol, DAS_ERR_ARG, "bad argument");
    gmres_begin(s, ksp, d_rhs, d_sol, fixed != 0);
    return DAS_OK;
    DAS_CATCH
}
int das_ksp_advance(das_solver_t* s, das_ksp_t* ksp, int iters) {
    DAS_TRY
    DAS_CHECK(ksp && ksp->run && iters > 0, DAS_ERR_STATE, "das_ksp_begin_device has not been called");
    return gmres_advance(s, ksp, iters) ? 1 : 0;
    DAS_CATCH
}
int das_ksp_end(das_solver_t* s, das_ksp_t* ksp) {
    DAS_TRY
    DAS_CHECK(ksp && ksp->run, DAS_ERR_STATE, "das_ksp_begin_device has not been called");
    return gmres_end(s, ksp);
    DAS_CATCH
}
void das_ksp_destroy(das_ksp_t* k) { delete k; }

int das_set_owned_mask(das_solver_t* s, const unsigned char* owned) {
    DAS_TRY
    DAS_CHECK(s, DAS_ERR_ARG, "null solver handle");
    if (!owned) { s->owned.clear(); return DAS_OK; }
    s->owned.assign(owned, owned + s->n);
    if (s->inited) s->d_owned.upload(s->owned);
    return DAS_OK;
    DAS_CATCH
// ... 130 lines not shown
    *ms_update = orth_bench_ms(reps, [&] { launch_dcgs2w_update<U, R, NT>(0, n, j, V.p, ld, sc.p, 0.5, 1.0, w.p, lo); }); } while (0)
#define DAS_WIDE(NT) do { DAS_DOTW(1, NT); DAS_DOTW(2, NT); DAS_DOTW(4, NT); \
    DAS_UPDW(2, 1, NT); DAS_UPDW(4, 1, NT); DAS_UPDW(8, 1, NT); DAS_UPDW(2, 2, NT); DAS_UPDW(4, 2, NT); } while (0)
int das_debug_orth_bench(long long n, int K, int reps, int rows, int unroll, int rpt, double* ms_dots, double* ms_update) {
    DAS_TRY
    DAS_CHECK(n > 0 && K > 1 && reps > 0 && ms_dots && ms_update, DAS_ERR_ARG, "das_debug_orth_bench: bad arguments");
    const long long ld = n;
    DevBuf<double> V((size_t)(K + 2) * ld), w(n), partial, sc(2 * (size_t)K);
    V.zero(); w.zero(); sc.zero();
    float* lo = nullptr;
    const double* u = V.p + (long long)(K - 1) * ld;
    *ms_dots = -1.0; *ms_update = -1.0;
    const int j = K - 1;
    DAS_DOT(double, 4); DAS_DOT(double, 8); DAS_DOT(double, 16);
    DAS_UPD(double, 4, 1); DAS_UPD(double, 8, 1); DAS_UPD(double, 16, 1); DAS_UPD(double, 4, 2); DAS_UPD(double, 8, 2); DAS_UPD(double, 4, 4);
    DAS_UPD(double, 8, 4);
    return DAS_OK;
    DAS_CATCH
}

int das_debug_orth_bench_split(long long n, int K, int reps, int fmt, int variant, int rows, int unroll, int rpt, double* ms_dots, double* ms_update) {
    DAS_TRY
    DAS_CHECK(n > 0 && n < (1LL << 30) && K > 1 && reps > 0 && ms_dots && ms_update, DAS_ERR_ARG, "das_debug_orth_bench_split: bad arguments");
    DAS_CHECK((fmt == KRY_FP32 || fmt == KRY_SPLIT) && variant >= 0 && variant <= 2, DAS_ERR_ARG, "das_debug_orth_bench_split: fmt 1 | 2, variant 0 | 1 | 2");
    const long long n4 = (n + 3) / 4 * 4, ld = fmt == KRY_SPLIT ? 2 * n4 : n4;
    DevBuf<float> V((size_t)(K + 2) * ld);
    DevBuf<double> w(n4), partial, sc(2 * (size_t)K);
    V.zero(); w.zero(); sc.zero();
    float* lo = fmt == KRY_SPLIT ? V.p + n4 : nullptr;
    const float* u = V.p + (long long)(K - 1) * ld;
    *ms_dots = -1.0; *ms_update = -1.0;
    const int j = K - 1;
    if (variant == 0) {
        DAS_DOT(float, 4); DAS_DOT(float, 8); DAS_DOT(float, 16);
        DAS_UPD(float, 4, 1); DAS_UPD(float, 8, 1); DAS_UPD(float, 4, 2); DAS_UPD(float, 8, 2); DAS_UPD(float, 4, 4);
    }
    if (variant == 1) DAS_WIDE(false);
    if (variant == 2) DAS_WIDE(true);
    return DAS_OK;
    DAS_CATCH
}
#undef DAS_DOT
#undef DAS_UPD
#undef DAS_DOTW
#undef DAS_UPDW
#undef DAS_WIDE
int das_debug_set_orth_wide(int on, int* previous) {
    if (previous) *previous = g_orth_wide;
    g_orth_wide = on ? 1 : 0;
    return DAS_OK;
}
int das_debug_krylov_wide_eligible(long long n, int fmt, long long ld, int* dots, int* update) {
    DAS_TRY
    DAS_CHECK(dots && update, DAS_ERR_ARG, "das_debug_krylov_wide_eligible: null pointer");
    const float* base = reinterpret_cast<const float*>((uintptr_t)1 << 20);
    const bool f = fmt == KRY_FP32 || fmt == KRY_SPLIT;
    *dots = (f && g_orth_wide && orth_wide_ok(n, base, nullptr, ld, base + ld, base)) ? 1 : 0;
    *update = (f && g_orth_wide && orth_wide_ok(n, base, fmt == KRY_SPLIT ? base + n : nullptr, ld, nullptr, base)) ? 1 : 0;
    return DAS_OK;
    DAS_CATCH
}

int das_debug_krylov_dots2(long long n, int K, int fmt, const void* V, long long ld, const double* v, double* out) {
    DAS_TRY
    krylov_check_basis("das_debug_krylov_dots2", n, K, fmt, V, ld);
    DAS_CHECK(v && out, DAS_ERR_ARG, "das_debug_krylov_dots2: null pointer");
    if (fmt == KRY_FP64) debug_krylov_dots2<double>(n, K, V, ld, v, out);
    else debug_krylov_dots2<float>(n, K, V, ld, v, out);
    return DAS_OK;
    DAS_CATCH
}
int das_debug_krylov_dcgs2_update(long long n, int j, int fmt, void* V, long long ld, int nslots, const double* sc, double gamma, double ralpha,
                                  const double* v) {
    DAS_TRY
    DAS_CHECK(j >= 0, DAS_ERR_ARG, "das_debug_krylov_dcgs2_update: j must not be negative");
    krylov_check_basis("das_debug_krylov_dcgs2_update", n, nslots, fmt, V, ld);
    DAS_CHECK(nslots >= j + 2, DAS_ERR_ARG, "das_debug_krylov_dcgs2_update: the basis needs slots 0 .. j + 1");
    DAS_CHECK(v && (sc || j == 0), DAS_ERR_ARG, "das_debug_krylov_dcgs2_update: null pointer");
    if (fmt == KRY_FP64) debug_krylov_dcgs2_update<double>(n, j, false, V, ld, nslots, sc, gamma, ralpha, v);
    else debug_krylov_dcgs2_update<float>(n, j, fmt == KRY_SPLIT, V, ld, nslots, sc, gamma, ralpha, v);
    return DAS_OK;
    DAS_CATCH
}
int das_debug_krylov_multidot(long long n, int m, int fmt, const void* V, long long ld, const double* w, double* out) {
    DAS_TRY
    DAS_CHECK(m >= 0, DAS_ERR_ARG, "das_debug_krylov_multidot: m must not be negative");
    krylov_check_basis("das_debug_krylov_multidot", n, std::max(m, 1), fmt, m > 0 ? V : (const void*)w, ld);
    DAS_CHECK(w && out, DAS_ERR_ARG, "das_debug_krylov_multidot: null pointer");
    if (fmt == KRY_FP64) debug_krylov_multidot<double>(n, m, V, ld, w, out);
    else debug_krylov_multidot<float>(n, m, V, ld, w, out);
    return DAS_OK;
    DAS_CATCH
}
int das_debug_krylov_multiaxpy(long long n, int m, int fmt, const void* V, long long ld, const double* h, int wfloat, void* w, long long wlen) {
    DAS_TRY
    krylov_check_basis("das_debug_krylov_multiaxpy", n, m, fmt, V, ld);
    DAS_CHECK(h && w, DAS_ERR_ARG, "das_debug_krylov_multiaxpy: null pointer");
    DAS_CHECK(wlen >= n, DAS_ERR_ARG, "das_debug_krylov_multiaxpy: w shorter than n");
    DAS_CHECK(!wfloat || fmt == KRY_FP32, DAS_ERR_ARG, "das_debug_krylov_multiaxpy: a float w goes with the fp32 basis only");
    if (fmt == KRY_FP64) debug_krylov_multiaxpy<double, double>(n, m, false, V, ld, h, w, wlen);
    else if (wfloat) debug_krylov_multiaxpy<float, float>(n, m, false, V, ld, h, w, wlen);
    else debug_krylov_multiaxpy<float, double>(n, m, fmt == KRY_SPLIT, V, ld, h, w, wlen);
    return DAS_OK;
    DAS_CATCH
}
int das_debug_krylov_lincomb(long long n, int m, int fmt, const void* V, long long ld, const double* c, double* y, long long ylen) {
    DAS_TRY
    krylov_check_basis("das_debug_krylov_lincomb", n, m, fmt, V, ld);
    DAS_CHECK(c && y, DAS_ERR_ARG, "das_debug_krylov_lincomb: null pointer");
    DAS_CHECK(ylen >= n, DAS_ERR_ARG, "das_debug_krylov_lincomb: y shorter than n");
    if (fmt == KRY_FP64) debug_krylov_lincomb<double>(n, m, false, V, ld, c, y, ylen);
    else debug_krylov_lincomb<float>(n, m, fmt == KRY_SPLIT, V, ld, c, y, ylen);
    return DAS_OK;
    DAS_CATCH
}
int das_debug_krylov_scale_to(long long n, double a, int use, const void* x, void* y, long long ylen) {
    DAS_TRY
    DAS_CHECK(n > 0, DAS_ERR_ARG, "das_debug_krylov_scale_to: n must be positive");
    DAS_CHECK(use >= 0 && use <= 4, DAS_ERR_ARG, "das_debug_krylov_scale_to: use is 0 (double -> double), 1 (double -> float), 2 (double -> split), 3 (split -> double) or 4 (float -> double)");
    DAS_CHECK(x && y, DAS_ERR_ARG, "das_debug_krylov_scale_to: null pointer");
    DAS_CHECK(ylen >= (use == 2 ? 2 * n : n), DAS_ERR_ARG, "das_debug_krylov_scale_to: y shorter than n (split: 2 n)");
    if (use == 0) debug_krylov_scale_to<double, double>(n, a, false, false, x, y, ylen);
    else if (use == 1) debug_krylov_scale_to<double, float>(n, a, false, false, x, y, ylen);
    else if (use == 2) debug_krylov_scale_to<double, float>(n, a, false, true, x, y, ylen);
    else if (use == 3) debug_krylov_scale_to<float, double>(n, a, true, false, x, y, ylen);
    else debug_krylov_scale_to<float, double>(n, a, false, false, x, y, ylen);
    return DAS_OK;
    DAS_CATCH
}
int das_debug_krylov_block_tn(long long n, int K, int s, const double* V, long long ldv, long long voff, const double* W, long long ldw, double* C) {
    DAS_TRY
    krylov_check_block("das_debug_krylov_block_tn", n, K, s);
    DAS_CHECK(V && W && C, DAS_ERR_ARG, "das_debug_krylov_block_tn: null pointer");
    DAS_CHECK(ldv >= n && ldw >= n && voff >= 0, DAS_ERR_ARG, "das_debug_krylov_block_tn: leading dimension below n or negative offset");
    debug_krylov_block_tn(n, K, s, V, ldv, voff, W, ldw, C);
    return DAS_OK;
    DAS_CATCH
}
int das_debug_krylov_block_nn_sub(long long n, int K, int s, const double* V, long long ldv, const double* C, double* W, long long ldw) {
    DAS_TRY
    krylov_check_block("das_debug_krylov_block_nn_sub", n, K, s);
    DAS_CHECK(V && W && C, DAS_ERR_ARG, "das_debug_krylov_block_nn_sub: null pointer");
    DAS_CHECK(ldv >= n && ldw >= n, DAS_ERR_ARG, "das_debug_krylov_block_nn_sub: leading dimension below n");
    debug_krylov_block_nn_sub(n, K, s, V, ldv, C, W, ldw);
    return DAS_OK;
    DAS_CATCH
}
int das_debug_krylov_block_right_mult(long long n, int s, double* W, long long ldw, const double* T) {
    DAS_TRY
    krylov_check_block("das_debug_krylov_block_right_mult", n, 1, s);
    DAS_CHECK(W && T, DAS_ERR_ARG, "das_debug_krylov_block_right_mult: null pointer");
    DAS_CHECK(ldw >= n, DAS_ERR_ARG, "das_debug_krylov_block_right_mult: leading dimension below n");
    debug_krylov_block_right_mult(n, s, W, ldw, T);
    return DAS_OK;
    DAS_CATCH
}
int das_debug_krylov_block_lincomb(long long n, int K, int s, const double* V, long long ldv, const double* C, double* Y, long long ldy) {
    DAS_TRY
    krylov_check_block("das_debug_krylov_block_lincomb", n, K, s);
    DAS_CHECK(V && C && Y, DAS_ERR_ARG, "das_debug_krylov_block_lincomb: null pointer");
    DAS_CHECK(ldv >= n && ldy >= n, DAS_ERR_ARG, "das_debug_krylov_block_lincomb: leading dimension below n");
    debug_krylov_block_lincomb(n, K, s, V, ldv, C, Y, ldy);
    return DAS_OK;
    DAS_CATCH
}
int das_debug_krylov_block_spmm(long long n, int s, const long long* rp, const int* ci, const double* val, const double* X, long long ldx, double* Y,
// ... 39 lines not shown
```

dafoam_amd/csrc/das_krylov.hpp:

```cpp
#pragma once
#include "das_common.hpp"

namespace das {

#define MD_CHUNK 1024
template <class VT>
__global__ __launch_bounds__(256) void k_multidot(long long n, int m, const VT* __restrict__ V, long long ldv, const double* __restrict__ w,
                                                  double* __restrict__ partial, int nb) {
    __shared__ double red[4];
    long long base = (long long)blockIdx.x * MD_CHUNK;
    double wr[4];
#pragma unroll
    for (int t = 0; t < 4; t++) {
        long long k = base + threadIdx.x + 256 * t;
        wr[t] = k < n ? w[k] : 0.0;
    }
    for (int i = 0; i <= m; i++) {
        double s = 0.0;
        if (i < m) {
            const VT* vi = V + (long long)i * ldv;
#pragma unroll
            for (int t = 0; t < 4; t++) {
                long long k = base + threadIdx.x + 256 * t;
                if (k < n) s += (double)vi[k] * wr[t];
// ... 27 lines not shown
    long long k = (long long)blockIdx.x * blockDim.x + threadIdx.x;
    if (k >= n) return;
    double s = (double)w[k];
    if (Vlo) for (int i = 0; i < m; i++) s -= h[i] * ((double)V[(long long)i * ldv + k] + (double)Vlo[(long long)i * ldv + k]);
    else for (int i = 0; i < m; i++) s -= h[i] * (double)V[(long long)i * ldv + k];
    w[k] = (WT)s;
}
__device__ __forceinline__ void multidot2_reduce_scatter(const double (&acc)[8], int lane, int g, int i0, int K, double* __restrict__ partial, long long nbw,
                                                         long long slot) {
    double a4[4], a2[2], a1;
#pragma unroll
    for (int i = 0; i < 4; i++) {
        const double snd = (g & 4) ? acc[i] : acc[i + 4], keep = (g & 4) ? acc[i + 4] : acc[i];
        a4[i] = keep + __shfl_xor(snd, 32, 64);
    }
#pragma unroll
    for (int i = 0; i < 2; i++) {
        const double snd = (g & 2) ? a4[i] : a4[i + 2], keep = (g & 2) ? a4[i + 2] : a4[i];
        a2[i] = keep + __shfl_xor(snd, 16, 64);
    }
    {
        const double snd = (g & 1) ? a2[0] : a2[1], keep = (g & 1) ? a2[1] : a2[0];
        a1 = keep + __shfl_xor(snd, 8, 64);
    }
    a1 += __shfl_xor(a1, 1, 64);
    a1 += __shfl_xor(a1, 2, 64);
    a1 += __shfl_xor(a1, 4, 64);
    const int i = i0 + (g >> 1);
    if ((lane & 7) == 0 && i < K) partial[((long long)(g & 1) * K + i) * nbw + slot] = a1;
}
#ifndef MD2_ROWS
#define MD2_ROWS 16
#endif
template <int ROWS, bool FULL, class QT, class VT>
__device__ __forceinline__ void multidot2_body(long long n, int K, const QT* __restrict__ V, long long ldv, const VT* __restrict__ u,
                                               const double* __restrict__ v, double* __restrict__ partial, long long nbw) {
    const int lane = threadIdx.x & 63, g = lane >> 3;
    const long long base = (long long)blockIdx.x * (256 * ROWS) + threadIdx.x;
    const long long slot = (long long)blockIdx.x * 4 + (threadIdx.x >> 6);
    double ur[ROWS], vr[ROWS];
#pragma unroll
    for (int t = 0; t < ROWS; t++) {
        const long long k = FULL ? base + 256 * t : min(base + 256 * t, n - 1);
        const double m = (FULL || base + 256 * t < n) ? 1.0 : 0.0;
        ur[t] = m * (double)u[k];
        vr[t] = m * v[k];
    }
    for (int i0 = 0; i0 < K; i0 += 4) {
        double acc[8], x[4][ROWS];
#pragma unroll
        for (int ii = 0; ii < 4; ii++) {
            const QT* vi = V + (long long)min(i0 + ii, K - 1) * ldv;
#pragma unroll
            for (int t = 0; t < ROWS; t++) x[ii][t] = (double)vi[FULL ? base + 256 * t : min(base + 256 * t, n - 1)];
        }
#pragma unroll
        for (int ii = 0; ii < 4; ii++) {
            double a = 0.0, b = 0.0;
#pragma unroll
            for (int t = 0; t < ROWS; t++) {
                a += x[ii][t] * ur[t];
                b += x[ii][t] * vr[t];
            }
            acc[2 * ii] = a;
            acc[2 * ii + 1] = b;
        }
        multidot2_reduce_scatter(acc, lane, g, i0, K, partial, nbw, slot);
    }
}
template <int ROWS, class QT, class VT>
__global__ __launch_bounds__(256) void k_multidot2(long long n, int K, const QT* __restrict__ V, long long ldv, const VT* __restrict__ u,
                                                   const double* __restrict__ v, double* __restrict__ partial, long long nbw) {
    if ((long long)(blockIdx.x + 1) * (256 * ROWS) <= n) multidot2_body<ROWS, true, QT, VT>(n, K, V, ldv, u, v, partial, nbw);
    else multidot2_body<ROWS, false, QT, VT>(n, K, V, ldv, u, v, partial, nbw);
}
#ifndef DCGS2_UNROLL
#define DCGS2_UNROLL 4
#endif
#ifndef DCGS2_RPT
#define DCGS2_RPT 2
#endif
template <int UNROLL, int RPT, class VT>
__global__ __launch_bounds__(256) void k_dcgs2_update(long long n, int j, VT* __restrict__ V, long long ldv, const double* __restrict__ sc,
                                                      double gamma, double ralpha, const double* __restrict__ v, float* __restrict__ Vlo = nullptr) {
    const long long k0 = ((long long)blockIdx.x * RPT) * blockDim.x + threadIdx.x;
    const double* s = sc;
    const double* c = sc + j;
    double as[RPT], ac[RPT];
    long long kk[RPT];
#pragma unroll
    for (int r = 0; r < RPT; r++) { as[r] = 0.0; ac[r] = 0.0; kk[r] = min(k0 + (long long)r * blockDim.x, n - 1); }
    int i = 0;
    for (; i + UNROLL <= j; i += UNROLL) {
        double q[UNROLL][RPT];
#pragma unroll
        for (int t = 0; t < UNROLL; t++)
#pragma unroll
            for (int r = 0; r < RPT; r++) q[t][r] = (double)V[(long long)(i + t) * ldv + kk[r]];
        if (Vlo) {
#pragma unroll
            for (int t = 0; t < UNROLL; t++)
#pragma unroll
                for (int r = 0; r < RPT; r++) q[t][r] += (double)Vlo[(long long)(i + t) * ldv + kk[r]];
        }
#pragma unroll
        for (int t = 0; t < UNROLL; t++)
#pragma unroll
            for (int r = 0; r < RPT; r++) { as[r] += s[i + t] * q[t][r]; ac[r] += c[i + t] * q[t][r]; }
    }
    for (; i < j; i++)
#pragma unroll
        for (int r = 0; r < RPT; r++) {
            const double q = (double)V[(long long)i * ldv + kk[r]] + (Vlo ? (double)Vlo[(long long)i * ldv + kk[r]] : 0.0);
            as[r] += s[i] * q; ac[r] += c[i] * q;
        }
#pragma unroll
    for (int r = 0; r < RPT; r++) {
        const long long k = k0 + (long long)r * blockDim.x;
        if (k >= n) continue;
        const double u = (double)V[(long long)j * ldv + k] + (Vlo ? (double)Vlo[(long long)j * ldv + k] : 0.0);
        const double qj = (u - as[r]) * ralpha, un = (v[k] - gamma * u - ac[r]) * ralpha;
        const VT qh = (VT)qj, uh = (VT)un;
        V[(long long)j * ldv + k] = qh;
        V[(long long)(j + 1) * ldv + k] = uh;
        if (Vlo) { Vlo[(long long)j * ldv + k] = (float)(qj - (double)qh); Vlo[(long long)(j + 1) * ldv + k] = (float)(un - (double)uh); }
    }
}
typedef float f32x4 __attribute__((ext_vector_type(4)));
typedef double f64x2 __attribute__((ext_vector_type(2)));
template <bool FULL, bool NT>
__device__ __forceinline__ f32x4 ld_group(const float* __restrict__ vec, const unsigned (&bo)[4]) {
    const char* b = reinterpret_cast<const char*>(vec);
    if (FULL) {
        const f32x4* p = reinterpret_cast<const f32x4*>(b + bo[0]);
        return NT ? __builtin_nontemporal_load(p) : *p;
    }
    f32x4 r;
    r.x = *reinterpret_cast<const float*>(b + bo[0]);
    r.y = *reinterpret_cast<const float*>(b + bo[1]);
    r.z = *reinterpret_cast<const float*>(b + bo[2]);
    r.w = *reinterpret_cast<const float*>(b + bo[3]);
    return r;
}
template <bool FULL>
__device__ __forceinline__ void group_offsets(long long k, long long n, unsigned (&bo)[4]) {
#pragma unroll
    for (int e = 0; e < 4; e++) bo[e] = (unsigned)((FULL ? k + e : min(k + e, n - 1)) * 4);
}
template <int R4, bool FULL, bool NT>
__device__ __forceinline__ void multidot2w_body(long long n, int K, const float* __restrict__ V, long long ldv, const float* __restrict__ u,
                                                const double* __restrict__ v, double* __restrict__ partial, long long nbw) {
    const int lane = threadIdx.x & 63, g = lane >> 3;
    const long long base = ((long long)blockIdx.x * (256 * R4) + threadIdx.x) * 4;
    const long long slot = (long long)blockIdx.x * 4 + (threadIdx.x >> 6);
    unsigned bo[R4][4];
    float ur[R4][4];
    double vr[R4][4];
#pragma unroll
    for (int t = 0; t < R4; t++) {
        const long long k = base + 1024LL * t;
        group_offsets<FULL>(k, n, bo[t]);
        const f32x4 uu = ld_group<FULL, false>(u, bo[t]);
        ur[t][0] = uu.x; ur[t][1] = uu.y; ur[t][2] = uu.z; ur[t][3] = uu.w;
        if (FULL) {
            const f64x2 a = *reinterpret_cast<const f64x2*>(v + k), b = *reinterpret_cast<const f64x2*>(v + k + 2);
            vr[t][0] = a.x; vr[t][1] = a.y; vr[t][2] = b.x; vr[t][3] = b.y;
        } else {
#pragma unroll
            for (int e = 0; e < 4; e++) {
                const bool in = k + e < n;
                vr[t][e] = in ? v[min(k + e, n - 1)] : 0.0;
                ur[t][e] = in ? ur[t][e] : 0.f;
            }
        }
    }
    const float* v0 = V;
    for (int i0 = 0; i0 < K; i0 += 4, v0 += 4 * ldv) {
        f32x4 x[4][R4];
        double acc[8];
#pragma unroll
        for (int ii = 0; ii < 4; ii++) {
            const float* vi = v0 + (long long)min(ii, K - 1 - i0) * ldv;
#pragma unroll
            for (int t = 0; t < R4; t++) x[ii][t] = ld_group<FULL, NT>(vi, bo[t]);
        }
#pragma unroll
        for (int ii = 0; ii < 4; ii++) {
            double a = 0.0, b = 0.0;
#pragma unroll
            for (int t = 0; t < R4; t++) {
                const double x0 = (double)x[ii][t].x, x1 = (double)x[ii][t].y, x2 = (double)x[ii][t].z, x3 = (double)x[ii][t].w;
                a += x0 * (double)ur[t][0]; b += x0 * vr[t][0];
                a += x1 * (double)ur[t][1]; b += x1 * vr[t][1];
                a += x2 * (double)ur[t][2]; b += x2 * vr[t][2];
                a += x3 * (double)ur[t][3]; b += x3 * vr[t][3];
            }
            acc[2 * ii] = a;
            acc[2 * ii + 1] = b;
        }
        multidot2_reduce_scatter(acc, lane, g, i0, K, partial, nbw, slot);
    }
}
template <int R4, bool NT>
__global__ __launch_bounds__(256) void k_multidot2w(long long n, int K, const float* __restrict__ V, long long ldv, const float* __restrict__ u,
                                                    const double* __restrict__ v, double* __restrict__ partial, long long nbw) {
    if ((long long)(blockIdx.x + 1) * (1024 * R4) <= n) multidot2w_body<R4, true, NT>(n, K, V, ldv, u, v, partial, nbw);
    else multidot2w_body<R4, false, NT>(n, K, V, ldv, u, v, partial, nbw);
}
template <int UNROLL, int RPT4, bool FULL, bool NT>
__device__ __forceinline__ void dcgs2w_body(long long n, int j, float* __restrict__ V, long long ldv, const double* __restrict__ sc, double gamma,
                                            double ralpha, const double* __restrict__ v, float* __restrict__ Vlo) {
    const long long base = ((long long)blockIdx.x * (256 * RPT4) + threadIdx.x) * 4;
    const double* s = sc;
    const double* c = sc + j;
    unsigned bo[RPT4][4];
    double as[RPT4][4], ac[RPT4][4];
#pragma unroll
    for (int r = 0; r < RPT4; r++) {
        group_offsets<FULL>(base + 1024LL * r, n, bo[r]);
#pragma unroll
        for (int e = 0; e < 4; e++) { as[r][e] = 0.0; ac[r][e] = 0.0; }
    }
    const float* h0 = V;
    const float* l0 = Vlo;
    for (int i = 0; i < j; i += UNROLL, h0 += UNROLL * ldv, l0 += (Vlo ? UNROLL * ldv : 0)) {
        f32x4 qh[UNROLL][RPT4], ql[UNROLL][RPT4];
#pragma unroll
        for (int t = 0; t < UNROLL; t++) {
            const float* hv = h0 + (long long)min(t, j - 1 - i) * ldv;
#pragma unroll
            for (int r = 0; r < RPT4; r++) qh[t][r] = ld_group<FULL, NT>(hv, bo[r]);
        }
        if (Vlo) {
#pragma unroll
            for (int t = 0; t < UNROLL; t++) {
                const float* lv = l0 + (long long)min(t, j - 1 - i) * ldv;
#pragma unroll
                for (int r = 0; r < RPT4; r++) ql[t][r] = ld_group<FULL, NT>(lv, bo[r]);
            }
        }
#pragma unroll
        for (int t = 0; t < UNROLL; t++) {
            const bool in = i + t < j;
            const double st = in ? s[min(i + t, j - 1)] : 0.0, ct = in ? c[min(i + t, j - 1)] : 0.0;
#pragma unroll
            for (int r = 0; r < RPT4; r++) {
                double q[4] = {(double)qh[t][r].x, (double)qh[t][r].y, (double)qh[t][r].z, (double)qh[t][r].w};
                if (Vlo) { q[0] += (double)ql[t][r].x; q[1] += (double)ql[t][r].y; q[2] += (double)ql[t][r].z; q[3] += (double)ql[t][r].w; }
#pragma unroll
                for (int e = 0; e < 4; e++) { as[r][e] += st * q[e]; ac[r][e] += ct * q[e]; }
            }
        }
    }
    float* uh = V + (long long)j * ldv;
    float* nh = uh + ldv;
    float* ul = Vlo ? Vlo + (long long)j * ldv : nullptr;
    float* nl = Vlo ? ul + ldv : nullptr;
#pragma unroll
    for (int r = 0; r < RPT4; r++) {
        const long long k = base + 1024LL * r;
        if (k >= n) continue;
        const f32x4 u4 = ld_group<FULL, false>(uh, bo[r]);
        double u[4] = {(double)u4.x, (double)u4.y, (double)u4.z, (double)u4.w}, vv[4];
        if (Vlo) {
            const f32x4 l4 = ld_group<FULL, false>(ul, bo[r]);
            u[0] += (double)l4.x; u[1] += (double)l4.y; u[2] += (double)l4.z; u[3] += (double)l4.w;
        }
        if (FULL) {
            const f64x2 a = *reinterpret_cast<const f64x2*>(v + k), b = *reinterpret_cast<const f64x2*>(v + k + 2);
            vv[0] = a.x; vv[1] = a.y; vv[2] = b.x; vv[3] = b.y;
        } else {
#pragma unroll
            for (int e = 0; e < 4; e++) vv[e] = v[min(k + e, n - 1)];
        }
        float qh[4], qlo[4], nhh[4], nlo[4];
#pragma unroll
        for (int e = 0; e < 4; e++) {
            const double qj = (u[e] - as[r][e]) * ralpha, un = (vv[e] - gamma * u[e] - ac[r][e]) * ralpha;
            qh[e] = (float)qj; nhh[e] = (float)un;
            qlo[e] = (float)(qj - (double)qh[e]); nlo[e] = (float)(un - (double)nhh[e]);
        }
        if (FULL) {
            *reinterpret_cast<f32x4*>(uh + k) = f32x4{qh[0], qh[1], qh[2], qh[3]};
            *reinterpret_cast<f32x4*>(nh + k) = f32x4{nhh[0], nhh[1], nhh[2], nhh[3]};
            if (Vlo) {
                *reinterpret_cast<f32x4*>(ul + k) = f32x4{qlo[0], qlo[1], qlo[2], qlo[3]};
                *reinterpret_cast<f32x4*>(nl + k) = f32x4{nlo[0], nlo[1], nlo[2], nlo[3]};
            }
        } else {
#pragma unroll
            for (int e = 0; e < 4; e++) {
                if (k + e >= n) continue;
                uh[k + e] = qh[e]; nh[k + e] = nhh[e];
                if (Vlo) { ul[k + e] = qlo[e]; nl[k + e] = nlo[e]; }
            }
        }
    }
}
template <int UNROLL, int RPT4, bool NT>
__global__ __launch_bounds__(256) void k_dcgs2w_update(long long n, int j, float* __restrict__ V, long long ldv, const double* __restrict__ sc,
                                                       double gamma, double ralpha, const double* __restrict__ v, float* __restrict__ Vlo) {
    if ((long long)(blockIdx.x + 1) * (1024 * RPT4) <= n) dcgs2w_body<UNROLL, RPT4, true, NT>(n, j, V, ldv, sc, gamma, ralpha, v, Vlo);
    else dcgs2w_body<UNROLL, RPT4, false, NT>(n, j, V, ldv, sc, gamma, ralpha, v, Vlo);
}
template <class VT>
__global__ __launch_bounds__(256) void k_lincomb(long long n, int m, const VT* __restrict__ V, long long ldv, const double* __restrict__ c,
                                                 double* __restrict__ y, const float* __restrict__ Vlo = nullptr) {
    long long k = (long long)blockIdx.x * blockDim.x + threadIdx.x;
    if (k >= n) return;
    double s = 0.0;
    if (Vlo) for (int i = 0; i < m; i++) s += c[i] * ((double)V[(long long)i * ldv + k] + (double)Vlo[(long long)i * ldv + k]);
    else for (int i = 0; i < m; i++) s += c[i] * (double)V[(long long)i * ldv + k];
    y[k] = s;
}
template <class TI, class TO>
__global__ void k_scale_to(long long n, double a, const TI* __restrict__ x, TO* __restrict__ y, const float* __restrict__ xlo = nullptr,
                           float* __restrict__ ylo = nullptr) {
    long long k = (long long)blockIdx.x * blockDim.x + threadIdx.x;
    if (k >= n) return;
    const double val = a * ((double)x[k] + (xlo ? (double)xlo[k] : 0.0));
    const TO yh = (TO)val;
    y[k] = yh;
    if (ylo) ylo[k] = (float)(val - (double)yh);
}
static inline size_t multidot_partial_size(long long n, int m) { return (size_t)(m + 1) * nblk(n, MD_CHUNK); }
template <class VT>
static void launch_multidot(hipStream_t st, long long n, int m, const VT* V, long long ldv, const double* w, double* partial, double* out) {
    const int nb = nblk(n, MD_CHUNK);
    hipLaunchKernelGGL(k_multidot, dim3(nb), dim3(256), 0, st, n, m, V, ldv, w, partial, nb);
    hipLaunchKernelGGL(k_reduce, dim3(m + 1), dim3(256), 0, st, nb, (const double*)partial, out);
}
template <int ROWS>
static inline long long multidot2_nbw(long long n) { return 4LL * nblk(n, 256 * ROWS); }
#ifndef MD2W_R4
#define MD2W_R4 4
#endif
#ifndef MD2W_NT
#define MD2W_NT 1
#endif
#ifndef DCGS2W_UNROLL
#define DCGS2W_UNROLL 4
#endif
#ifndef DCGS2W_RPT4
#define DCGS2W_RPT4 2
#endif
#ifndef DCGS2W_NT
#define DCGS2W_NT 0
#endif
#ifndef ORTH_WIDE_DEFAULT
#define ORTH_WIDE_DEFAULT 1
#endif
static int g_orth_wide = ORTH_WIDE_DEFAULT;
static inline bool orth_wide_ok(long long n, const void* V, const void* Vlo, long long ldv, const void* u, const void* v) {
    return n >= 4 && n < (1LL << 30) && (ldv & 3) == 0 && ((((uintptr_t)V | (uintptr_t)Vlo | (uintptr_t)u | (uintptr_t)v) & 15) == 0);
}
static inline long long multidot2w_nbw(long long n, int r4) { return 4LL * nblk(n, 1024 * r4); }
static inline size_t multidot2_partial_size(long long n, int K) {
    return (size_t)2 * K * (size_t)std::max(multidot2_nbw<MD2_ROWS>(n), multidot2w_nbw(n, MD2W_R4));
}
template <int ROWS, class VT>
static void launch_multidot2_pass(hipStream_t st, long long n, int K, const VT* V, long long ldv, const VT* u, const double* v, double* partial) {
    hipLaunchKernelGGL((k_multidot2<ROWS, VT, VT>), dim3(nblk(n, 256 * ROWS)), dim3(256), 0, st, n, K, V, ldv, u, v, partial, multidot2_nbw<ROWS>(n));
}
template <int R4, bool NT>
static void launch_multidot2w_pass(hipStream_t st, long long n, int K, const float* V, long long ldv, const float* u, const double* v, double* partial) {
    hipLaunchKernelGGL((k_multidot2w<R4, NT>), dim3(nblk(n, 1024 * R4)), dim3(256), 0, st, n, K, V, ldv, u, v, partial, multidot2w_nbw(n, R4));
}
template <int UNROLL, int RPT, class VT>
static void launch_dcgs2_update_pass(hipStream_t st, long long n, int j, VT* V, long long ldv, const double* sc, double gamma, double ralpha,
                                     const double* v, float* Vlo) {
    hipLaunchKernelGGL((k_dcgs2_update<UNROLL, RPT, VT>), dim3(nblk(n, 256 * RPT)), dim3(256), 0, st, n, j, V, ldv, sc, gamma, ralpha, v, Vlo);
}
template <int UNROLL, int RPT4, bool NT>
static void launch_dcgs2w_update(hipStream_t st, long long n, int j, float* V, long long ldv, const double* sc, double gamma, double ralpha,
                                 const double* v, float* Vlo) {
    hipLaunchKernelGGL((k_dcgs2w_update<UNROLL, RPT4, NT>), dim3(nblk(n, 1024 * RPT4)), dim3(256), 0, st, n, j, V, ldv, sc, gamma, ralpha, v, Vlo);
}
template <class VT>
static void launch_multidot2(hipStream_t st, long long n, int K, const VT* V, long long ldv, const VT* u, const double* v, double* partial, double* out) {
    if constexpr (std::is_same<VT, float>::value) {
        if (g_orth_wide && orth_wide_ok(n, V, nullptr, ldv, u, v)) {
            launch_multidot2w_pass<MD2W_R4, MD2W_NT != 0>(st, n, K, V, ldv, u, v, partial);
            hipLaunchKernelGGL(k_reduce, dim3(2 * K), dim3(256), 0, st, (int)multidot2w_nbw(n, MD2W_R4), (const double*)partial, out);
            return;
        }
    }
    launch_multidot2_pass<MD2_ROWS, VT>(st, n, K, V, ldv, u, v, partial);
    hipLaunchKernelGGL(k_reduce, dim3(2 * K), dim3(256), 0, st, (int)multidot2_nbw<MD2_ROWS>(n), (const double*)partial, out);
}
template <int UNROLL, int RPT, class VT>
static void launch_dcgs2_update(hipStream_t st, long long n, int j, VT* V, long long ldv, const double* sc, double gamma, double ralpha, const double* v,
                                float* Vlo) {
    if constexpr (std::is_same<VT, float>::value) {
        if (g_orth_wide && orth_wide_ok(n, V, Vlo, ldv, nullptr, v)) {
            launch_dcgs2w_update<DCGS2W_UNROLL, DCGS2W_RPT4, DCGS2W_NT != 0>(st, n, j, V, ldv, sc, gamma, ralpha, v, Vlo);
            return;
        }
    }
    launch_dcgs2_update_pass<UNROLL, RPT, VT>(st, n, j, V, ldv, sc, gamma, ralpha, v, Vlo);
}
template <class VT, class WT>
static void launch_multiaxpy(hipStream_t st, long long n, int m, const VT* V, long long ldv, const double* h, WT* w, const float* Vlo) {
    hipLaunchKernelGGL(k_multiaxpy, dim3(nblk(n, 256)), dim3(256), 0, st, n, m, V, ldv, h, w, Vlo);
}
template <class VT>
static void launch_lincomb(hipStream_t st, long long n, int m, const VT* V, long long ldv, const double* c, double* y, const float* Vlo) {
    hipLaunchKernelGGL(k_lincomb, dim3(nblk(n, 256)), dim3(256), 0, st, n, m, V, ldv, c, y, Vlo);
}
template <class TI, class TO>
static void launch_scale_to(hipStream_t st, long long n, double a, const TI* x, TO* y, const float* xlo, float* ylo) {
    hipLaunchKernelGGL(k_scale_to, dim3(nblk(n, 256)), dim3(256), 0, st, n, a, x, y, xlo, ylo);
}

}
```

dafoam_amd/csrc/das_krylov_debug.hpp:

```cpp
#pragma once
#include "das_krylov.hpp"
#include "das_block.hpp"

namespace das {

enum { KRY_FP64 = 0, KRY_FP32 = 1, KRY_SPLIT = 2 };
static void krylov_check_basis(const std::string& who, long long n, long long nvec, int fmt, const void* V, long long ld) {
    DAS_CHECK(n > 0 && nvec > 0, DAS_ERR_ARG, who + ": sizes must be positive");
    DAS_CHECK(fmt == KRY_FP64 || fmt == KRY_FP32 || fmt == KRY_SPLIT, DAS_ERR_ARG, who + ": fmt is 0 (fp64), 1 (fp32) or 2 (split)");
    DAS_CHECK(V, DAS_ERR_ARG, who + ": null basis");
    DAS_CHECK(ld >= (fmt == KRY_SPLIT ? 2 * n : n), DAS_ERR_ARG, who + ": leading dimension below n (split: below 2 n)");
}
static void krylov_check_block(const std::string& who, long long n, int K, int sv) {
    DAS_CHECK(n > 0 && K > 0, DAS_ERR_ARG, who + ": sizes must be positive");
    DAS_CHECK(sv >= 1 && sv <= 8, DAS_ERR_ARG, who + ": 1 to 8 right-hand sides");
}
static void krylov_debug_sync() {
    DAS_HIP(hipGetLastError());
    DAS_HIP(hipStreamSynchronize(0));
}
template <class VT>
static float* krylov_lo(VT* V, long long n, bool split) { return split ? reinterpret_cast<float*>(V) + n : nullptr; }
template <class T>
static DevBuf<T> krylov_up(const void* h, size_t cnt) {
    DevBuf<T> d(std::max<size_t>(cnt, 1));
    d.upload((const T*)h, cnt);
    return d;
}
template <class T, class F>
static void krylov_run(F&& launch, const DevBuf<T>& res, void* h, size_t cnt) {
    launch();
    krylov_debug_sync();
    res.download((T*)h, cnt);
}

template <class VT>
static void debug_krylov_dots2(long long n, int K, const void* V, long long ld, const double* v, double* out) {
    const DevBuf<VT> dV = krylov_up<VT>(V, (size_t)K * ld);
    const DevBuf<double> dv = krylov_up<double>(v, n), partial(multidot2_partial_size(n, K)), dout((size_t)2 * K);
    krylov_run([&] { launch_multidot2<VT>(0, n, K, dV.p, ld, dV.p + (long long)(K - 1) * ld, dv.p, partial.p, dout.p); }, dout, out, (size_t)2 * K);
}
template <class VT>
static void debug_krylov_dcgs2_update(long long n, int j, bool split, void* V, long long ld, int nslots, const double* sc, double gamma, double ralpha,
                                      const double* v) {
    const DevBuf<VT> dV = krylov_up<VT>(V, (size_t)nslots * ld);
    const DevBuf<double> dsc = krylov_up<double>(sc, (size_t)2 * j), dv = krylov_up<double>(v, n);
    krylov_run([&] { launch_dcgs2_update<DCGS2_UNROLL, DCGS2_RPT, VT>(0, n, j, dV.p, ld, dsc.p, gamma, ralpha, dv.p, krylov_lo(dV.p, n, split)); }, dV, V,
               (size_t)nslots * ld);
}
template <class VT>
static void debug_krylov_multidot(long long n, int m, const void* V, long long ld, const double* w, double* out) {
    const DevBuf<VT> dV = krylov_up<VT>(V, (size_t)m * ld);
    const DevBuf<double> dw = krylov_up<double>(w, n), partial(multidot_partial_size(n, m)), dout((size_t)m + 1);
    krylov_run([&] { launch_multidot<VT>(0, n, m, dV.p, ld, dw.p, partial.p, dout.p); }, dout, out, (size_t)m + 1);
}
template <class VT, class WT>
static void debug_krylov_multiaxpy(long long n, int m, bool split, const void* V, long long ld, const double* h, void* w, long long wlen) {
    const DevBuf<VT> dV = krylov_up<VT>(V, (size_t)m * ld);
    const DevBuf<double> dh = krylov_up<double>(h, m);
    const DevBuf<WT> dw = krylov_up<WT>(w, (size_t)wlen);
    krylov_run([&] { launch_multiaxpy<VT, WT>(0, n, m, dV.p, ld, dh.p, dw.p, krylov_lo(dV.p, n, split)); }, dw, w, (size_t)wlen);
}
template <class VT>
static void debug_krylov_lincomb(long long n, int m, bool split, const void* V, long long ld, const double* c, double* y, long long ylen) {
    const DevBuf<VT> dV = krylov_up<VT>(V, (size_t)m * ld);
    const DevBuf<double> dc = krylov_up<double>(c, m), dy = krylov_up<double>(y, (size_t)ylen);
    krylov_run([&] { launch_lincomb<VT>(0, n, m, dV.p, ld, dc.p, dy.p, krylov_lo(dV.p, n, split)); }, dy, y, (size_t)ylen);
}
template <class TI, class TO>
static void debug_krylov_scale_to(long long n, double a, bool xsplit, bool ysplit, const void* x, void* y, long long ylen) {
    const DevBuf<TI> dx = krylov_up<TI>(x, (size_t)(xsplit ? 2 * n : n));
    const DevBuf<TO> dy = krylov_up<TO>(y, (size_t)ylen);
    krylov_run([&] { launch_scale_to<TI, TO>(0, n, a, dx.p, dy.p, krylov_lo(dx.p, n, xsplit), krylov_lo(dy.p, n, ysplit)); }, dy, y, (size_t)ylen);
}
static void debug_krylov_block_tn(long long n, int K, int s, const double* V, long long ldv, long long voff, const double* W, long long ldw, double* C) {
    const DevBuf<double> dV = krylov_up<double>(V, (size_t)(voff + (long long)K * ldv)), dW = krylov_up<double>(W, (size_t)s * ldw);
    const DevBuf<double> partial(tsgemm_partial_size(K)), dC((size_t)K * s);
    krylov_run([&] { launch_tsgemm_tn(0, n, K, s, dV.p + voff, ldv, dW.p, ldw, partial.p, dC.p); }, dC, C, (size_t)K * s);
}
static void debug_krylov_block_nn_sub(long long n, int K, int s, const double* V, long long ldv, const double* C, double* W, long long ldw) {
    const DevBuf<double> dV = krylov_up<double>(V, (size_t)K * ldv), dW = krylov_up<double>(W, (size_t)s * ldw), dC = krylov_up<double>(C, (size_t)K * s);
    krylov_run([&] { launch_tsgemm_nn_sub(0, n, K, s, dV.p, ldv, dC.p, dW.p, ldw); }, dW, W, (size_t)s * ldw);
}
static void debug_krylov_block_right_mult(long long n, int s, double* W, long long ldw, const double* T) {
    const DevBuf<double> dW = krylov_up<double>(W, (size_t)s * ldw), dT = krylov_up<double>(T, (size_t)s * s);
    krylov_run([&] { launch_block_right_mult(0, n, s, dW.p, ldw, dT.p); }, dW, W, (size_t)s * ldw);
}
static void debug_krylov_block_lincomb(long long n, int K, int s, const double* V, long long ldv, const double* C, double* Y, long long ldy) {
    const DevBuf<double> dV = krylov_up<double>(V, (size_t)K * ldv), dC = krylov_up<double>(C, (size_t)K * s), dY = krylov_up<double>(Y, (size_t)s * ldy);
    krylov_run([&] { launch_block_lincomb(0, n, K, s, dV.p, ldv, dC.p, dY.p, ldy); }, dY, Y, (size_t)s * ldy);
}
static void debug_krylov_block_spmm(long long n, int s, const long long* rp, const int* ci, const double* val, const double* X, long long ldx, double* Y,
                                    long long ldy) {
    const size_t nnz = (size_t)rp[n];
    const DevBuf<long long> drp = krylov_up<long long>(rp, (size_t)n + 1);
    const DevBuf<int> dci = krylov_up<int>(ci, nnz);
    const DevBuf<double> dval = krylov_up<double>(val, nnz), dX = krylov_up<double>(X, (size_t)s * ldx), dY = krylov_up<double>(Y, (size_t)s * ldy);
    const DevBuf<double> dXr((size_t)n * spmm_width(s));
    krylov_run([&] {
        launch_block_to_rows(0, n, s, dX.p, ldx, dXr.p);
        launch_spmm_wave(0, n, s, drp.p, dci.p, dval.p, dXr.p, dY.p, ldy);
    }, dY, Y, (size_t)s * ldy);
}

struct BenchEvent {
    hipEvent_t e = nullptr;
    BenchEvent() { DAS_HIP(hipEventCreate(&e)); }
    ~BenchEvent() { (void)hipEventDestroy(e); }
    BenchEvent(const BenchEvent&) = delete;
    BenchEvent& operator=(const BenchEvent&) = delete;
};
template <class F>
static double orth_bench_ms(int reps, F&& launch) {
    BenchEvent e0, e1;
    launch();
    DAS_HIP(hipEventRecord(e0.e, 0));
    for (int r = 0; r < reps; r++) launch();
    DAS_HIP(hipEventRecord(e1.e, 0));
    DAS_HIP(hipEventSynchronize(e1.e));
    DAS_HIP(hipGetLastError());
    float ms = 0.f;
    DAS_HIP(hipEventElapsedTime(&ms, e0.e, e1.e));
    return (double)ms / reps;
}

}
```

dafoam_amd/csrc/das_mesh.cpp:

```cpp
#include <algorithm>
#include <cmath>

#include "das_common.hpp"
#include "das_geom.hpp"

namespace das {

double wall_seconds() {
    using namespace std::chrono;
    return duration<double>(steady_clock::now().time_since_epoch()).count();
}

Options::Options() {
    s["solverName"] = "DASimpleFoam";
    s["adjStateOrdering"] = "state";
    s["normalizeResiduals"] = "URes,pRes,p_rghRes,nuTildaRes,phiRes,TRes,DRes,kRes,omegaRes,epsilonRes,alpha.waterRes";
    d["adjPartDerivFDStep.State"] = 1.0e-6;
    d["normalizeStates.U"] = 1.0;
    d["normalizeStates.p"] = 1.0;
    d["normalizeStates.nuTilda"] = 1.0;
    d["normalizeStates.phi"] = 1.0;
    d["normalizeStates.T"] = 1.0;
    i["useConstrainHbyA"] = 1;
    i["adjUseColoring"] = 1;
    i["maxCorrectBCCalls"] = 2;
    i["adjPCLag"] = 10000;
    i["printInterval"] = 100;
    i["debug"] = 0;
    i["adjEqnOption.globalPCIters"] = 0;
    i["adjEqnOption.asmOverlap"] = 1;
    i["adjEqnOption.localPCIters"] = 1;
    s["adjEqnOption.jacMatReOrdering"] = "rcm";
    i["adjEqnOption.pcFillLevel"] = 1;
    i["adjEqnOption.gmresMaxIters"] = 1000;
    i["adjEqnOption.gmresRestart"] = 1000;
    d["adjEqnOption.gmresRelTol"] = 1.0e-6;
    d["adjEqnOption.gmresAbsTol"] = 1.0e-14;
    d["adjEqnOption.gmresTolDiff"] = 1.0e2;
    i["adjEqnOption.useNonZeroInitGuess"] = 0;
    i["adjEqnOption.useMGSO"] = 0;
    i["adjEqnOption.printInfo"] = 1;
    i["adjEqnOption.dynAdjustTol"] = 0;
    i["adjEqnOption.readPCMat"] = 0;
    i["maxResConLv4JacPCMat.pRes"] = 2;
    i["maxResConLv4JacPCMat.phiRes"] = 1;
    i["maxResConLv4JacPCMat.URes"] = 2;
    i["maxResConLv4JacPCMat.TRes"] = 2;
    i["maxResConLv4JacPCMat.nuTildaRes"] = 2;
    d["jacLowerBounds.dRdW"] = 1.0e-30;
    d["jacLowerBounds.dRdWPC"] = 1.0e-30;
    s["amd.pcType"] = "bilu";
    i["amd.pcCoarseAggregates"] = -1;
    s["amd.pcCoarseField"] = "p";
    s["amd.pcCoarseAggregation"] = "rcb";
    d["amd.pcUpwindBlend"] = 0.5;
    s["amd.pcCoarseMode"] = "deflated";
    d["amd.pcStabilityLimit"] = 1.0e8;
    s["amd.pcOrderCandidates"] = "1245";
    d["amd.pcStabilityGood"] = 1.0e4;
    i["amd.pcSubdomains"] = -1;
    i["amd.pcCoarseSparseAZ"] = 1;
    i["amd.coloringOnDevice"] = 1;
    s["amd.primalMethod"] = "newton";
    i["amd.simpleSweepsPerCheck"] = 10;
    d["amd.simpleAlphaP"] = 0.3;
    d["amd.simpleLinearTol"] = 1.0e-6;
    i["amd.simpleLinearIters"] = 2000;
    d["amd.primalTau0"] = 1.0;
    d["amd.primalSERExponent"] = 1.5;
    s["amd.primalPseudoTimeFields"] = "all";
    s["amd.primalTauMode"] = "ser";
    d["amd.primalTauGrowth"] = 1.5;
    d["amd.primalTauGrowthMax"] = 10.0;
    d["amd.primalTauMax"] = 1.0e12;
    d["amd.primalTauMin"] = 1.0e-3;
    d["amd.primalAcceptFactor"] = 1.5;
    s["amd.primalDampedSteps"] = "accept";
    d["amd.primalLinearTol"] = 1.0e-3;
    i["amd.primalLinearIters"] = 300;
    i["amd.primalPCLag"] = 3;
    i["amd.setupThreads"] = 32;
    i["amd.pcBlockCells"] = 1024;
    i["amd.jacMode"] = 1;
    i["amd.pcJacMode"] = 0;
    i["amd.pcFactorFP32"] = 0;
    i["amd.keepAssemblyMaps"] = 0;
    i["amd.cgsAlwaysRefine"] = 0;
    i["amd.blockBatchedPC"] = 1;
    i["amd.opPackVector"] = 1;
    s["amd.coloringAlgorithm"] = "auto";
    s["amd.volCoordMode"] = "dual";
    i["amd.volCoordRings"] = 3;
    d["amd.volCoordRelStep"] = 1e-4;
    i["amd.pcCoarseGlobal"] = 1;
    s["amd.gmresOrthogonalization"] = "dcgs2";
    i["amd.gmresDeflation"] = 0;
    s["amd.krylovBasisPrecision"] = "auto";
    i["amd.cellFaceSplit"] = 0;
    i["amd.gradFaceParallel"] = 1;
}
double Options::getd(const std::string& k) const {
    auto it = d.find(k);
    if (it != d.end()) return it->second;
    auto it2 = i.find(k);
    if (it2 != i.end()) return (double)it2->second;
    throw Error(DAS_ERR_ARG, "option not found: " + k);
}
long long Options::geti(const std::string& k) const {
    auto it = i.find(k);
    if (it != i.end()) return it->second;
    auto it2 = d.find(k);
    if (it2 != d.end()) return (long long)it2->second;
    throw Error(DAS_ERR_ARG, "option not found: " + k);
}
const std::string& Options::gets(const std::string& k) const {
    auto it = s.find(k);
    if (it == s.end()) throw Error(DAS_ERR_ARG, "option not found: " + k);
    return it->second;
}
bool Options::list_has(const std::string& k, const std::string& item) const {
    const std::string& v = gets(k);
    size_t pos = 0;
    while (pos <= v.size()) {
        size_t e = v.find(',', pos);
        if (e == std::string::npos) e = v.size();
        if (v.compare(pos, e - pos, item) == 0) return true;
        pos = e + 1;
    }
    return false;
}

void Mesh::build(const das_case_t* c) {
    DAS_CHECK(c && c->points && c->face_ptr && c->face_pts && c->owner, DAS_ERR_ARG, "das_case: null mesh arrays");
    nP = c->n_points; nF = c->n_faces; nIF = c->n_internal_faces; nC = c->n_cells; nPatch = c->n_patches;
    DAS_CHECK(nP > 0 && nF > 0 && nC > 0 && nIF >= 0 && nIF <= nF, DAS_ERR_ARG, "das_case: bad sizes");
    points.assign(c->points, c->points + 3 * (size_t)nP);
    face_ptr.assign(c->face_ptr, c->face_ptr + nF + 1);
    face_pts.assign(c->face_pts, c->face_pts + face_ptr[nF]);
    owner.assign(c->owner, c->owner + nF);
    neighbour.assign(c->neighbour, c->neighbour + nIF);
    patch_start.assign(c->patch_start, c->patch_start + nPatch);
    patch_size.assign(c->patch_size, c->patch_size + nPatch);
    patch_type.assign(c->patch_type, c->patch_type + nPatch);
    for (int f = 0; f < nF; f++) DAS_CHECK(owner[f] >= 0 && owner[f] < nC, DAS_ERR_ARG, "owner out of range");
// ... 308 lines not shown
```

include/dafoam_amd.h:

```cpp
#ifndef DAFOAM_AMD_H
#define DAFOAM_AMD_H

#ifdef __cplusplus
extern "C" {
#endif

#define DAS_OK 0
#define DAS_ERR_ARG -1
#define DAS_ERR_NO_DEVICE -2
#define DAS_ERR_HIP -3
#define DAS_ERR_STATE -4
#define DAS_ERR_INTERNAL -5

#define DAS_SOLVER_SIMPLEFOAM 0
#define DAS_SOLVER_SCALARTRANSPORTFOAM 1
#define DAS_SOLVER_RHOSIMPLEFOAM 2
#define DAS_SOLVER_TURBOFOAM 3
#define DAS_IS_COMPRESSIBLE(s) ((s) == DAS_SOLVER_RHOSIMPLEFOAM || (s) == DAS_SOLVER_TURBOFOAM)

#define DAS_PATCH_PATCH 0
#define DAS_PATCH_WALL 1
#define DAS_PATCH_SYMMETRY 2
#define DAS_PATCH_CYCLIC 3

// ... 123 lines not shown
int das_set_field(das_solver_t* s, const char* fieldName, const double* values);
int das_get_field(das_solver_t* s, const char* fieldName, double* values);
int das_calc_dfield_product(das_solver_t* s, const char* fieldName, const char* outputName, const char* outputType, const double* seeds,
                            double* product);
int das_calc_dbc_product(das_solver_t* s, const int* patch_ids, int npatch, const char* field, const double* tangent, const char* outputName,
                         const char* outputType, const double* seeds, double* product);
int das_define_force_function(das_solver_t* s, const char* name, const int* patch_ids, int npatch, const double* direction, double scale);
int das_define_face_function(das_solver_t* s, const char* name, const char* type, const int* patch_ids, const int* patch_group, int npatch,
                             const double* vecA, const double* vecB, double scale, double gammaFn);
int das_define_patch_field_function(das_solver_t* s, const char* name, const char* type, const int* patch_ids, int npatch, const char* var,
                                    const int* comps, int ncomp, const double* data, int flags, double scale, double ref);
int das_define_cell_function(das_solver_t* s, const char* name, const char* type, const int* cells, int ncells, const char* var, const int* comps,
                             int ncomp, const double* data, int flags, double scale, double ref);
int das_calc_function(das_solver_t* s, const char* name, double* value);

int das_get_input_size(das_solver_t* s, const char* inputName, const char* inputType);
int das_get_output_size(das_solver_t* s, const char* outputName, const char* outputType);
int das_calc_jac_t_vec_product(das_solver_t* s, const char* inputName, const char* inputType, const double* inputs,
                               const char* outputName, const char* outputType, const double* seeds, double* product);
int das_drdwt_mult_device(das_solver_t* s, const double* d_x, double* d_y);

int das_create_ml_rksp_matrix_free(das_solver_t* s, das_mat_t* pc, das_ksp_t** ksp);
int das_solve_linear_eqn(das_solver_t* s, das_ksp_t* ksp, const double* rhs, double* sol);
int das_solve_linear_eqn_block(das_solver_t* s, das_ksp_t* ksp, int nrhs, const double* rhs, double* sol, double* res0, double* res);
int das_ksp_apply_pc(das_solver_t* s, das_ksp_t* ksp, const double* x, double* y);
int das_ksp_get_n_blocks(das_ksp_t* ksp);
long long das_ksp_get_factor_nnz(das_ksp_t* ksp);
long long das_ksp_get_n_ext(das_ksp_t* ksp);
int das_ksp_get_blocks(das_ksp_t* ksp, int* perm, long long* block_off);
int das_pc_structure_build(das_solver_t* s, int* nNodes, long long* nBlocks, int* nLevels, int* reach);
int das_pc_structure_get(das_solver_t* s, int* nodeUnk, long long* bptr, int* bcol, int* lvlPtr, int* natural);
int das_ksp_get_pc_structure_sizes(das_ksp_t* ksp, int* nNodes, long long* nBlocks, int* nLevels);
int das_ksp_get_pc_structure(das_ksp_t* ksp, int* nodeUnk, long long* bptr, int* bcol, int* lvlPtr, int* natural);
int das_ksp_get_pc_node_out(das_ksp_t* ksp, int* nodeOut);
int das_ksp_get_info(das_ksp_t* ksp, int* iters, double* res0, double* res, double* seconds);
int das_ksp_get_history(das_ksp_t* ksp, double* hist, int cap);
int das_ksp_get_basis_info(das_ksp_t* ksp, int* fp32, double* mappedBytes, double* bytesPerVector);
int das_ksp_get_cycle_lengths(das_ksp_t* ksp, int* lens, int cap);
int das_ksp_get_n_refine(das_ksp_t* ksp);
int das_set_dense_eig_callback(void* fn);
int das_debug_gmres_dr_restart(int m, int kwant, const double* Hbar, const double* rvec, double* P1, double* Hnew, double* cnew);
int das_debug_gmres_dr_host(long long n, void* A, void* M, void* user, const double* b, double* x, int m, int kdef, double rtol, double atol,
                            long long maxIts, double* hist, int histCap, double* info4, double* res2);
int das_ksp_get_status(das_ksp_t* ksp, int* reason, int* nBreakdown, int* nSweepGrid, int* sweepPerXcd);
int das_ksp_get_pc_stability(das_ksp_t* ksp, double* estimate, int* orderUsed);
int das_ksp_get_pc_subdomains(das_ksp_t* ksp, int* orders, double* estimates);
int das_ksp_get_coarse(das_ksp_t* ksp, int* aggOfCell);
int das_ksp_coarse_sparse_az_active(das_ksp_t* ksp);
int das_ksp_set_global_coarse(das_solver_t* s, das_ksp_t* ksp, int naggGlobal, int aggOffset, const int* aggRowGlobal);
int das_ksp_run_fixed_device(das_solver_t* s, das_ksp_t* ksp, const double* d_rhs, double* d_sol, int iters);
int das_ksp_begin_device(das_solver_t* s, das_ksp_t* ksp, const double* d_rhs, double* d_sol, int fixed);
int das_ksp_advance(das_solver_t* s, das_ksp_t* ksp, int iters);
int das_ksp_end(das_solver_t* s, das_ksp_t* ksp);
void das_ksp_destroy(das_ksp_t* k);

typedef void (*das_halo_cb)(double* d_vec, void* user);
typedef void (*das_allreduce_cb)(double* d_buf, int n, void* user);
int das_set_owned_mask(das_solver_t* s, const unsigned char* owned );
int das_set_comm(das_solver_t* s, das_halo_cb halo, das_allreduce_cb allreduce, void* user);
int das_comm_load_rccl(void);
typedef void (*das_exchange_cb)(double* d_send, double* d_recv, void* user);
int das_comm_unique_id(char* out128);
int das_comm_init_rccl(das_solver_t* s, int rank, int world, const char* id128);
int das_comm_set_halo(das_solver_t* s, int npeers, const int* peers, const long long* sendOff, const int* sendIdx, const long long* recvOff,
                      const int* recvIdx, long long nGhost, const int* ghostIdx);
int das_set_exchange_cb(das_solver_t* s, das_exchange_cb cb, void* user);
int das_set_pc_overlap(das_solver_t* s, const unsigned char* pcMask , int npeers, const long long* ovSendOff, const int* ovSendIdx,
                       const long long* ovRecvOff, const int* ovRecvIdx);
int das_set_gather_cb(das_solver_t* s, das_exchange_cb cb, void* user);
int das_comm_is_native(das_solver_t* s);
int das_comm_reset(das_solver_t* s);
int das_set_stream(das_solver_t* s, void* hip_stream);

double das_get_elapsed_clock_time(das_solver_t* s);
double das_get_elapsed_cpu_time(das_solver_t* s);
double das_timer_avg_ms(das_solver_t* s, const char* name);
int das_debug_orth_bench(long long n, int K, int reps, int rows, int unroll, int rpt, double* ms_dots, double* ms_update);
int das_debug_orth_bench_split(long long n, int K, int reps, int fmt, int variant, int rows, int unroll, int rpt, double* ms_dots, double* ms_update);
int das_debug_set_orth_wide(int on, int* previous);
int das_debug_krylov_wide_eligible(long long n, int fmt, long long ld, int* dots, int* update);
int das_debug_krylov_dots2(long long n, int K, int fmt, const void* V, long long ld, const double* v, double* out);
int das_debug_krylov_dcgs2_update(long long n, int j, int fmt, void* V, long long ld, int nslots, const double* sc, double gamma, double ralpha,
                                  const double* v);
int das_debug_krylov_multidot(long long n, int m, int fmt, const void* V, long long ld, const double* w, double* out);
int das_debug_krylov_multiaxpy(long long n, int m, int fmt, const void* V, long long ld, const double* h, int wfloat, void* w, long long wlen);
int das_debug_krylov_lincomb(long long n, int m, int fmt, const void* V, long long ld, const double* c, double* y, long long ylen);
int das_debug_krylov_scale_to(long long n, double a, int use, const void* x, void* y, long long ylen);
int das_debug_krylov_block_tn(long long n, int K, int s, const double* V, long long ldv, long long voff, const double* W, long long ldw, double* C);
int das_debug_krylov_block_nn_sub(long long n, int K, int s, const double* V, long long ldv, const double* C, double* W, long long ldw);
int das_debug_krylov_block_right_mult(long long n, int s, double* W, long long ldw, const double* T);
int das_debug_krylov_block_lincomb(long long n, int K, int s, const double* V, long long ldv, const double* C, double* Y, long long ldy);
int das_debug_krylov_block_spmm(long long n, int s, const long long* rowptr, const int* colidx, const double* vals, const double* X, long long ldx,
                                double* Y, long long ldy);
long long das_timer_count(das_solver_t* s, const char* name);
void das_timer_reset(das_solver_t* s);
void das_timer_enable(das_solver_t* s, int on);

#ifdef __cplusplus
}
#endif
#endif
```

Measured before the change: 43.47.

## Fuse deflated coarse correction path and stage f64 basis vector in DCGS2 update

Adds a fused deflated coarse preconditioner path: a wave-per-row dense coarse solve, an A·Z apply whose first aggregate entry per row is stored inline, and a prolong-add straight into z, in place of separate prolong and residual kernels. The DCGS2 update kernel can also write the new basis vector as f64 into a staging buffer, so the next preconditioner apply with f32 basis storage skips a conversion. Host staging for the dot and coefficient transfers moves to pinned buffers. These changes aim to cut kernel launches, memory passes and transfer latency per GMRES iteration, at the cost of extra buffers and more code paths.

```diff
diff --git a/dafoam_amd/_capi.py b/dafoam_amd/_capi.py
--- a/dafoam_amd/_capi.py
+++ b/dafoam_amd/_capi.py
@@ -299,6 +299,13 @@
     "das_debug_krylov_wide_eligible": (C.c_int, [C.c_longlong, C.c_int, C.c_longlong, C.POINTER(C.c_int), C.POINTER(C.c_int)]),
     "das_debug_krylov_dots2": (C.c_int, [C.c_longlong, C.c_int, C.c_int, _VP, C.c_longlong, c_double_p, c_double_p]),
     "das_debug_krylov_dcgs2_update": (C.c_int, [C.c_longlong, C.c_int, C.c_int, _VP, C.c_longlong, C.c_int, c_double_p, C.c_double, C.c_double, c_double_p]),
+    "das_debug_krylov_dcgs2_update_staged": (C.c_int, [C.c_longlong, C.c_int, C.c_int, _VP, C.c_longlong, C.c_int, c_double_p, C.c_double, C.c_double, c_double_p,
+                                                      c_double_p, C.c_longlong]),
+    "das_debug_pc_apply_full": (C.c_int, [_VP, _VP, c_double_p, C.c_int, c_double_p, c_double_p, c_double_p, c_double_p, c_double_p]),
+    "das_debug_coarse_einv": (C.c_int, [_VP, c_double_p]),
+    "das_debug_coarse_az_structure": (C.c_int, [_VP, _VP, c_ll_p, c_int_p, c_ll_p]),
+    "das_debug_coarse_az_apply": (C.c_int, [C.c_longlong, c_ll_p, c_int_p, c_double_p, C.c_longlong, C.c_longlong, c_int_p, C.c_int, c_double_p, c_double_p, c_int_p,
+                                            c_double_p, c_double_p]),
     "das_debug_krylov_multidot": (C.c_int, [C.c_longlong, C.c_int, C.c_int, _VP, C.c_longlong, c_double_p, c_double_p]),
     "das_debug_krylov_multiaxpy": (C.c_int, [C.c_longlong, C.c_int, C.c_int, _VP, C.c_longlong, c_double_p, C.c_int, _VP, C.c_longlong]),
     "das_debug_krylov_lincomb": (C.c_int, [C.c_longlong, C.c_int, C.c_int, _VP, C.c_longlong, c_double_p, c_double_p, C.c_longlong]),
diff --git a/dafoam_amd/csrc/das_device.hip b/dafoam_amd/csrc/das_device.hip
--- a/dafoam_amd/csrc/das_device.hip
+++ b/dafoam_amd/csrc/das_device.hip
@@ -501,6 +501,16 @@
     for (int J = 0; J < nagg; J++) acc += Einv[(long long)I * nagg + J] * t[J];
     u[I] = acc;
 }
+__global__ __launch_bounds__(256) void k_coarse_solve_wave(int nagg, const double* __restrict__ Einv, const double* __restrict__ t, double* __restrict__ u) {
+    const int I = blockIdx.x * 4 + (threadIdx.x >> 6), lane = threadIdx.x & 63;
+    if (I >= nagg) return;
+    const double* row = Einv + (long long)I * nagg;
+    double acc = 0.0;
+    for (int J = lane; J < nagg; J += 64) acc += row[J] * t[J];
+#pragma unroll
+    for (int o = 32; o > 0; o >>= 1) acc += __shfl_down(acc, o, 64);
+    if (lane == 0) u[I] = acc;
+}
 __global__ void k_coarse_prolong(long long N, long long n, long long off, const int* __restrict__ agg, const double* __restrict__ u,
                                  double* __restrict__ y, int set) {
     const long long i = (long long)blockIdx.x * blockDim.x + threadIdx.x;
@@ -509,11 +519,19 @@
     const double add = (c >= 0 && c < N && agg[c] >= 0) ? u[agg[c]] : 0.0;
     y[i] = set ? add : y[i] + add;
 }
+__global__ __launch_bounds__(256) void k_coarse_prolong_add(long long N, long long off, const int* __restrict__ agg, const double* __restrict__ u,
+                                                            double* __restrict__ z) {
+    const long long c = (long long)blockIdx.x * blockDim.x + threadIdx.x;
+    if (c >= N) return;
+    const int a = agg[c];
+    if (a >= 0) z[off + c] += u[a];
+}
 
 constexpr int AZ_CAP = 64;
 __global__ __launch_bounds__(256) void k_az_build(long long n, const long long* __restrict__ rp, const int* __restrict__ ci, const double* __restrict__ v,
                                                   long long N, long long off, const int* __restrict__ agg, int pass, int* __restrict__ cnt,
-                                                  const long long* __restrict__ ptr, int* __restrict__ oa, double* __restrict__ ov, int* __restrict__ overflow) {
+                                                  const long long* __restrict__ ptr, int* __restrict__ oa, double* __restrict__ ov, int* __restrict__ overflow,
+                                                  int* __restrict__ a0 = nullptr, double* __restrict__ v0 = nullptr) {
     const long long i = (long long)blockIdx.x * blockDim.x + threadIdx.x;
     if (i >= n) return;
     int la[AZ_CAP];
@@ -534,6 +552,12 @@
     }
     if (pass == 0) { cnt[i] = m; return; }
     const long long b = ptr[i];
+    if (pass == 2) {
+        a0[i] = m == 0 ? 0 : (m > 1 ? ~la[0] : la[0]);
+        v0[i] = m == 0 ? 0.0 : ls[0];
+        for (int q = 1; q < m; q++) { oa[b + q - 1] = la[q]; ov[b + q - 1] = ls[q]; }
+        return;
+    }
     for (int q = 0; q < m; q++) { oa[b + q] = la[q]; ov[b + q] = ls[q]; }
 }
 __global__ __launch_bounds__(256) void k_az_apply(long long n, const long long* __restrict__ ptr, const int* __restrict__ oa, const double* __restrict__ ov,
@@ -543,6 +567,29 @@
     double acc = 0.0;
     for (long long k = ptr[i]; k < ptr[i + 1]; k++) acc += ov[k] * u[oa[k]];
     out[i] = v ? v[i] - acc : acc;
+}
+constexpr int AZI_ROWS = 4;
+__global__ __launch_bounds__(256) void k_az_apply_inline(long long n, const int* __restrict__ a0, const double* __restrict__ v0, const long long* __restrict__ ptr,
+                                                         const int* __restrict__ oa, const double* __restrict__ ov, const double* __restrict__ u,
+                                                         const double* __restrict__ v, double* __restrict__ out) {
+    const long long base = (long long)blockIdx.x * (256 * AZI_ROWS) + threadIdx.x;
+    int a[AZI_ROWS];
+    double w0[AZI_ROWS], vi[AZI_ROWS];
+#pragma unroll
+    for (int r = 0; r < AZI_ROWS; r++) {
+        const long long i = min(base + 256LL * r, n - 1);
+        a[r] = a0[i]; w0[r] = v0[i]; vi[r] = v[i];
+    }
+#pragma unroll
+    for (int r = 0; r < AZI_ROWS; r++) {
+        const long long i = base + 256LL * r;
+        if (i >= n) continue;
+        const bool more = a[r] < 0;
+        double acc = 0.0;
+        acc += w0[r] * u[more ? ~a[r] : a[r]];
+        if (more) for (long long k = ptr[i]; k < ptr[i + 1]; k++) acc += ov[k] * u[oa[k]];
+        out[i] = vi[r] - acc;
+    }
 }
 
 #ifndef PC_THREADS
@@ -792,6 +839,12 @@
         long long azOpId = -1;
         long long azEpoch = -1, azNnz = 0;
         bool azReady = false, azFailed = false;
+        DevBuf<int> aziAgg0, aziAgg;
+        DevBuf<double> aziVal0, aziVal;
+        DevBuf<long long> aziPtr;
+        bool aziReady = false;
+        bool fused = true;
+        const double* dbgU = nullptr;
     } coarse;
     int restart = 0;
     VmBuf<double> V;
@@ -799,6 +852,21 @@
     bool vf32 = false;
     bool split = false;
     DevBuf<double> ustage;
+    struct PinBuf {
+        double* p = nullptr;
+        size_t n = 0;
+        PinBuf() = default;
+        PinBuf(const PinBuf&) = delete;
+        PinBuf& operator=(const PinBuf&) = delete;
+        ~PinBuf() { if (p) (void)hipHostFree(p); }
+        void alloc(size_t n_) {
+            if (p) { (void)hipHostFree(p); p = nullptr; }
+            n = 0;
+            DAS_HIP(hipHostMalloc((void**)&p, std::max<size_t>(n_, 1) * sizeof(double), hipHostMallocDefault));
+            n = n_;
+            std::fill(p, p + n, 0.0);
+        }
+    } dotsPin, coefPin;
     DevBuf<double> w, z, r, xdev, bdev, partial, hdev, rich_r, rich_d;
     int nSub = 1;
     std::vector<int> subOrder;
@@ -1921,7 +1989,7 @@
         for (long long c = 0; c < N; c++) if (aggRowG[c] >= 0) cellsAll[pos[aggRowG[c]]++] = (int)c;
     }
     C.naggG = naggG; C.aggOff = aggOff; C.global = naggG > C.nagg;
-    C.azOpId = -1; C.azReady = false;
+    C.azOpId = -1; C.azReady = false; C.aziReady = false;
     C.agg.upload(aggOwn); C.aggRow.upload(aggRowG); C.cellsAll.upload(cellsAll); C.aptrAll.upload(aptrAll);
     DevBuf<double> E((size_t)naggG * naggG);
     E.zero();
@@ -1955,6 +2023,7 @@
 static void setup_coarse(das_solver* s, das_ksp* k) {
     das_ksp::CoarsePC& C = k->coarse;
     C.active = false;
+    C.fused = s->opt.geti("amd.pcCoarseFused") != 0;
     long long want = s->opt.geti("amd.pcCoarseAggregates");
     if (want == 0) return;
     const std::string field = s->opt.gets("amd.pcCoarseField");
@@ -2015,12 +2084,14 @@
     coarse_build_operator(s, k, nagg, 0, agg);
     if (C.active && s->opt.geti("debug")) fprintf(stderr, "[dafoam_amd] coarse space: %d aggregates on field %s (%s)\n", nagg, field.c_str(), C.deflated ? "deflated" : "additive");
 }
-static void coarse_solve(das_solver* s, das_ksp* k, const double* r) {
+static void coarse_solve(das_solver* s, das_ksp* k, const double* r, bool wavePerRow = false) {
     das_ksp::CoarsePC& C = k->coarse;
     if (C.global) DAS_HIP(hipMemsetAsync(C.t.p, 0, (size_t)C.naggG * sizeof(double), s->stream));
     if (C.nagg > 0) hipLaunchKernelGGL(k_coarse_restrict, dim3(C.nagg), dim3(256), 0, s->stream, C.aptr.p, C.cells.p, C.off, r, C.t.p + C.aggOff);
     if (C.global) rank_allreduce(s, C.t.p, C.naggG, s->stream);
-    hipLaunchKernelGGL(k_coarse_solve, dim3(nblk(C.naggG, 64)), dim3(64), 0, s->stream, C.naggG, C.Einv.p, C.t.p, C.u.p);
+    if (wavePerRow) hipLaunchKernelGGL(k_coarse_solve_wave, dim3(nblk(C.naggG, 4)), dim3(256), 0, s->stream, C.naggG, C.Einv.p, C.t.p, C.u.p);
+    else hipLaunchKernelGGL(k_coarse_solve, dim3(nblk(C.naggG, 64)), dim3(64), 0, s->stream, C.naggG, C.Einv.p, C.t.p, C.u.p);
+    if (C.dbgU) DAS_HIP(hipMemcpyAsync(C.u.p, C.dbgU, (size_t)C.naggG * sizeof(double), hipMemcpyDeviceToDevice, s->stream));
 }
 
 static void pc_apply(das_solver* s, das_ksp* k, const double* b, double* x) {
@@ -2088,6 +2159,7 @@
         k->z.zero();
         k->partial.alloc(std::max<size_t>(multidot_partial_size(n, (int)restart + 1), multidot2_partial_size(n, (int)restart + 2)));
         k->hdev.alloc(4 * (restart + 3));
+        k->dotsPin.alloc(2 * (restart + 2)); k->coefPin.alloc(2 * (restart + 2));
     }
 }
 static inline long long basis_n4(das_solver* s) { return (s->n + 3) / 4 * 4; }
@@ -2115,13 +2187,14 @@
 
 static void apply_operator(das_solver* s, const double* x, double* y);
 
-static bool coarse_az_ready(das_solver* s, das_ksp* k) {
+static bool coarse_az_ready(das_solver* s, das_ksp* k, bool inlineLayout = false) {
     das_ksp::CoarsePC& C = k->coarse;
     if (!s->op || s->fwd.on) return false;
     { auto it = s->opt.i.find("amd.pcCoarseSparseAZ"); if (it != s->opt.i.end() && it->second == 0) return false; }
     const Mat& A = s->op->m;
-    if (C.azOpId == s->opId && C.azEpoch == s->op_epoch) return C.azReady;
-    C.azOpId = s->opId; C.azEpoch = s->op_epoch; C.azReady = false; C.azFailed = false;
+    if (C.azOpId != s->opId || C.azEpoch != s->op_epoch) { C.azOpId = s->opId; C.azEpoch = s->op_epoch; C.azReady = false; C.aziReady = false; C.azFailed = false; }
+    if (C.azFailed) return false;
+    if (inlineLayout ? C.aziReady : C.azReady) return true;
     const long long n = s->n;
     hipStream_t st = s->stream;
     DevBuf<int> cnt(n), ovf(1);
@@ -2145,6 +2218,22 @@
     }
     std::vector<int> h = cnt.to_host();
     std::vector<long long> ptr(n + 1, 0);
+    if (inlineLayout) {
+        long long nnz = 0;
+        for (long long i = 0; i < n; i++) { ptr[i + 1] = ptr[i] + std::max(h[i] - 1, 0); nnz += h[i]; }
+        C.azNnz = nnz;
+        C.aziPtr.upload(ptr);
+        C.aziAgg0.alloc((size_t)n); C.aziVal0.alloc((size_t)n);
+        C.aziAgg.alloc((size_t)std::max<long long>(1, ptr[n])); C.aziVal.alloc((size_t)std::max<long long>(1, ptr[n]));
+        hipLaunchKernelGGL(k_az_build, dim3(nblk(n, 256)), dim3(256), 0, st, n, A.rowptr.p, A.col.p, A.val.p, C.N, C.off, C.agg.p, 2, cnt.p, C.aziPtr.p, C.aziAgg.p,
+                           C.aziVal.p, ovf.p, C.aziAgg0.p, C.aziVal0.p);
+        DAS_HIP(hipStreamSynchronize(st));
+        if (s->opt.geti("debug"))
+            fprintf(stderr, "[dafoam_amd] deflated coarse mode: sparse A Z with %lld entries (%.2f per row), %lld of them behind the first of their row\n", C.azNnz,
+                    (double)C.azNnz / (double)n, ptr[n]);
+        C.aziReady = true;
+        return true;
+    }
     for (long long i = 0; i < n; i++) ptr[i + 1] = ptr[i] + h[i];
     C.azNnz = ptr[n];
     C.azPtr.upload(ptr);
@@ -2164,8 +2253,15 @@
     if (C.active) {
         hipEvent_t ev = nullptr;
         s->timer.begin("coarse", s->stream, ev);
-        coarse_solve(s, k, v);
-        if (C.deflated && (s->op || s->fwd.on)) {
+        const bool fused = C.fused && C.deflated && !C.global && !(s->halo.active || s->halo_cb) && coarse_az_ready(s, k, true);
+        coarse_solve(s, k, v, fused);
+        if (fused) {
+            hipLaunchKernelGGL(k_az_apply_inline, dim3(nblk(n, 256 * AZI_ROWS)), dim3(256), 0, s->stream, n, C.aziAgg0.p, C.aziVal0.p, C.aziPtr.p, C.aziAgg.p,
+                               C.aziVal.p, C.u.p, v, C.rr.p);
+            s->timer.end("coarse", s->stream, ev);
+            pc_apply(s, k, C.rr.p, z);
+            hipLaunchKernelGGL(k_coarse_prolong_add, dim3(nblk(C.N, 256)), dim3(256), 0, s->stream, C.N, C.off, C.agg.p, C.u.p, z);
+        } else if (C.deflated && (s->op || s->fwd.on)) {
             hipLaunchKernelGGL(k_coarse_prolong, dim3(nblk(n, 256)), dim3(256), 0, s->stream, C.N, n, C.off, C.agg.p, C.u.p, C.c.p, 1);
             if (coarse_az_ready(s, k)) {
                 if (s->halo.active || s->halo_cb) {
@@ -2253,6 +2349,7 @@
     bool dcgs2 = false;
     int pend = 0;
     std::vector<double> Hraw, h1;
+    int staged = -1;
     bool earlyClose = false;
     bool safeOrth = false;
     bool stalled = false;
@@ -2314,6 +2411,7 @@
     G.g[0] = G.beta;
     G.j = 0;
     G.pend = 0;
+    G.staged = -1;
     G.open = true;
     G.earlyClose = false;
     G.betaStart = G.beta;
@@ -2424,16 +2522,16 @@
     VT* const Vb = basis_slot<VT>(s, k, 0);
     const long long ld = basis_ld(s, k);
     VT* u = Vb + (long long)j * ld;
-    pc_apply_full(s, k, basis_as_double<VT>(s, k, j), k->z.p);
+    pc_apply_full(s, k, (k->vf32 && G.staged == j) ? (const double*)k->ustage.p : basis_as_double<VT>(s, k, j), k->z.p);
     apply_operator(s, k->z.p, k->w.p);
     const int K = j + 1;
     launch_multidot2<VT>(st, n, K, (const VT*)Vb, ld, (const VT*)u, (const double*)k->w.p, k->partial.p, k->hdev.p);
     rank_allreduce(s, k->hdev.p, 2 * K, st);
-    std::vector<double>& o = G.hh;
-    DAS_HIP(hipMemcpyAsync(o.data(), k->hdev.p, 2 * K * sizeof(double), hipMemcpyDeviceToHost, st));
+    double* const o = k->dotsPin.p;
+    DAS_HIP(hipMemcpyAsync(o, k->hdev.p, 2 * K * sizeof(double), hipMemcpyDeviceToHost, st));
     DAS_HIP(hipStreamSynchronize(st));
-    const double* sv = o.data();
-    const double* tv = o.data() + K;
+    const double* sv = o;
+    const double* tv = o + K;
     const double uu = sv[j], uv = tv[j];
     double ss = 0.0, stt = 0.0;
     for (int i = 0; i < j; i++) { ss += sv[i] * sv[i]; stt += sv[i] * tv[i]; }
@@ -2459,6 +2557,7 @@
         DAS_HIP(hipStreamSynchronize(st));
         al2 = cc[0]; num = cc[1];
         explicitProj = true;
+        G.staged = -1;
         k->nrefine++;
     }
     const bool breakdown = !(al2 > GMRES_BREAKDOWN_TOL * GMRES_BREAKDOWN_TOL * normBq2);
@@ -2484,11 +2583,13 @@
         if (stop || G.j >= m) return res;
     }
     const double gam = num / al2;
-    std::vector<double>& co = G.h2;
+    double* const co = k->coefPin.p;
     for (int i = 0; i < j; i++) { co[i] = sv[i]; co[j + i] = tv[i] - gam * sv[i]; }
     double* dco = k->hdev.p + 2 * (m + 3);
-    if (j > 0) DAS_HIP(hipMemcpyAsync(dco, co.data(), 2 * j * sizeof(double), hipMemcpyHostToDevice, st));
-    launch_dcgs2_update<DCGS2_UNROLL, DCGS2_RPT, VT>(st, n, j, Vb, ld, (const double*)dco, gam, 1.0 / al, (const double*)k->w.p, basis_lo(s, k, 0));
+    if (j > 0) DAS_HIP(hipMemcpyAsync(dco, co, 2 * j * sizeof(double), hipMemcpyHostToDevice, st));
+    double* const stage = (k->vf32 && k->coarse.fused) ? k->ustage.p : nullptr;
+    launch_dcgs2_update<DCGS2_UNROLL, DCGS2_RPT, VT>(st, n, j, Vb, ld, (const double*)dco, gam, 1.0 / al, (const double*)k->w.p, basis_lo(s, k, 0), stage);
+    G.staged = stage ? j + 1 : -1;
     for (int i = 0; i < j; i++) {
         double a = tv[i];
         for (int q = std::max(0, i - 1); q < j; q++) a -= G.Hraw[(size_t)i * m + q] * sv[q];
@@ -4906,6 +5007,89 @@
     return DAS_OK;
     DAS_CATCH
 }
+int das_debug_pc_apply_full(das_solver_t* s, das_ksp_t* ksp, const double* x, int fused, const double* uIn, double* z, double* t, double* u, double* rr) {
+    DAS_TRY
+    need_init(s);
+    DAS_CHECK(ksp && x && z, DAS_ERR_ARG, "das_debug_pc_apply_full: null argument");
+    das_ksp::CoarsePC& C = ksp->coarse;
+    DAS_CHECK(C.active || !(uIn || t || u || rr), DAS_ERR_STATE, "das_debug_pc_apply_full: the preconditioner of this KSP has no coarse space");
+    DAS_CHECK(!rr || C.deflated, DAS_ERR_STATE, "das_debug_pc_apply_full: rr exists in the deflated coarse mode only");
+    DevBuf<double> dx(s->n), dz(s->n), du;
+    dx.upload(x, s->n);
+    if (uIn) du.upload(uIn, (size_t)C.naggG);
+    DAS_HIP(hipDeviceSynchronize());
+    dz.zero();
+    struct Restore {
+        das_ksp::CoarsePC& C;
+        bool fused;
+        ~Restore() { C.fused = fused; C.dbgU = nullptr; }
+    } restore{C, C.fused};
+    if (fused >= 0) C.fused = fused != 0;
+    C.dbgU = uIn ? du.p : nullptr;
+    pc_apply_full(s, ksp, dx.p, dz.p);
+    DAS_HIP(hipStreamSynchronize(s->stream));
+    if (ksp->useBilu) DAS_CHECK(!bilu_aborted(ksp->bilu, s->stream), DAS_ERR_INTERNAL, "preconditioner sweep timed out (bounded spin)");
+    dz.download(z, s->n);
+    if (t) C.t.download(t, (size_t)C.naggG);
+    if (u) C.u.download(u, (size_t)C.naggG);
+    if (rr) C.rr.download(rr, s->n);
+    return DAS_OK;
+    DAS_CATCH
+}
+int das_debug_coarse_einv(das_ksp_t* ksp, double* Einv) {
+    DAS_TRY
+    if (!ksp || !ksp->coarse.active) return 0;
+    if (Einv) ksp->coarse.Einv.download(Einv, (size_t)ksp->coarse.naggG * ksp->coarse.naggG);
+    return ksp->coarse.naggG;
+    DAS_CATCH
+}
+int das_debug_coarse_az_structure(das_solver_t* s, das_ksp_t* ksp, long long* ptr, int* a0, long long* optr) {
+    DAS_TRY
+    need_init(s);
+    DAS_CHECK(ksp && ptr && a0 && optr, DAS_ERR_ARG, "das_debug_coarse_az_structure: null argument");
+    das_ksp::CoarsePC& C = ksp->coarse;
+    if (!C.active || !C.deflated || !coarse_az_ready(s, ksp, false) || !coarse_az_ready(s, ksp, true)) return 0;
+    C.azPtr.download(ptr, (size_t)s->n + 1);
+    C.aziAgg0.download(a0, (size_t)s->n);
+    C.aziPtr.download(optr, (size_t)s->n + 1);
+    return 1;
+    DAS_CATCH
+}
+int das_debug_coarse_az_apply(long long n, const long long* rp, const int* ci, const double* val, long long N, long long off, const int* agg, int nagg,
+                              const double* u, const double* v, int* cnt, double* outCsr, double* outInline) {
+    DAS_TRY
+    DAS_CHECK(n > 0 && N > 0 && off >= 0 && nagg > 0 && rp && agg && u && v && cnt && outCsr && outInline, DAS_ERR_ARG, "das_debug_coarse_az_apply: bad argument");
+    DAS_CHECK(rp[0] == 0, DAS_ERR_ARG, "das_debug_coarse_az_apply: rowptr[0] must be 0");
+    for (long long i = 0; i < n; i++) DAS_CHECK(rp[i + 1] >= rp[i], DAS_ERR_ARG, "das_debug_coarse_az_apply: rowptr decreases");
+    DAS_CHECK(rp[n] == 0 || (ci && val), DAS_ERR_ARG, "das_debug_coarse_az_apply: null pointer");
+    for (long long c = 0; c < N; c++) DAS_CHECK(agg[c] >= -1 && agg[c] < nagg, DAS_ERR_ARG, "das_debug_coarse_az_apply: aggregate out of range");
+    const size_t nnz = (size_t)rp[n];
+    const DevBuf<long long> drp = krylov_up<long long>(rp, (size_t)n + 1);
+    const DevBuf<int> dci = krylov_up<int>(ci, nnz), dagg = krylov_up<int>(agg, (size_t)N);
+    const DevBuf<double> dval = krylov_up<double>(val, nnz), du = krylov_up<double>(u, (size_t)nagg), dv = krylov_up<double>(v, (size_t)n);
+    DevBuf<int> dcnt((size_t)n), ovf(1);
+    ovf.zero();
+    hipLaunchKernelGGL(k_az_build, dim3(nblk(n, 256)), dim3(256), 0, 0, n, drp.p, dci.p, dval.p, N, off, dagg.p, 0, dcnt.p, (const long long*)nullptr, (int*)nullptr,
+                       (double*)nullptr, ovf.p);
+    krylov_debug_sync();
+    dcnt.download(cnt, (size_t)n);
+    if (ovf.to_host()[0]) return 1;
+    std::vector<long long> ptr(n + 1, 0), optr(n + 1, 0);
+    for (long long i = 0; i < n; i++) { ptr[i + 1] = ptr[i] + cnt[i]; optr[i + 1] = optr[i] + std::max(cnt[i] - 1, 0); }
+    DevBuf<long long> dptr, doptr;
+    dptr.upload(ptr); doptr.upload(optr);
+    DevBuf<int> oa((size_t)std::max<long long>(1, ptr[n])), oai((size_t)std::max<long long>(1, optr[n])), a0((size_t)n);
+    DevBuf<double> ov((size_t)std::max<long long>(1, ptr[n])), ovi((size_t)std::max<long long>(1, optr[n])), v0((size_t)n), o1((size_t)n), o2((size_t)n);
+    hipLaunchKernelGGL(k_az_build, dim3(nblk(n, 256)), dim3(256), 0, 0, n, drp.p, dci.p, dval.p, N, off, dagg.p, 1, dcnt.p, dptr.p, oa.p, ov.p, ovf.p);
+    hipLaunchKernelGGL(k_az_build, dim3(nblk(n, 256)), dim3(256), 0, 0, n, drp.p, dci.p, dval.p, N, off, dagg.p, 2, dcnt.p, doptr.p, oai.p, ovi.p, ovf.p, a0.p, v0.p);
+    hipLaunchKernelGGL(k_az_apply, dim3(nblk(n, 256)), dim3(256), 0, 0, n, dptr.p, oa.p, ov.p, du.p, dv.p, o1.p);
+    hipLaunchKernelGGL(k_az_apply_inline, dim3(nblk(n, 256 * AZI_ROWS)), dim3(256), 0, 0, n, a0.p, v0.p, doptr.p, oai.p, ovi.p, du.p, dv.p, o2.p);
+    krylov_debug_sync();
+    o1.download(outCsr, (size_t)n);
+    o2.download(outInline, (size_t)n);
+    return DAS_OK;
+    DAS_CATCH
+}
 static void copy_pc_structure(const NodeILU& P, int* nodeUnk, long long* bptr, int* bcol, int* lvlPtr, int* natural) {
     if (natural) std::copy(P.h_natural.begin(), P.h_natural.end(), natural);
     if (nodeUnk) std::copy(P.h_nodeUnk.begin(), P.h_nodeUnk.end(), nodeUnk);
@@ -5043,7 +5227,7 @@
     }
     return k->nSub;
 }
-int das_ksp_coarse_sparse_az_active(das_ksp_t* k) { return k ? (k->coarse.active && k->coarse.deflated && k->coarse.azReady ? 1 : 0) : -1; }
+int das_ksp_coarse_sparse_az_active(das_ksp_t* k) { return k ? (k->coarse.active && k->coarse.deflated && (k->coarse.azReady || k->coarse.aziReady) ? 1 : 0) : -1; }
 int das_ksp_get_coarse(das_ksp_t* k, int* aggOfCell) {
     if (!k || !k->coarse.active) return 0;
     if (aggOfCell) std::copy(k->coarse.h_agg.begin(), k->coarse.h_agg.end(), aggOfCell);
@@ -5340,6 +5524,19 @@
     return DAS_OK;
     DAS_CATCH
 }
+int das_debug_krylov_dcgs2_update_staged(long long n, int j, int fmt, void* V, long long ld, int nslots, const double* sc, double gamma, double ralpha,
+                                         const double* v, double* stage, long long stagelen) {
+    DAS_TRY
+    DAS_CHECK(j >= 0, DAS_ERR_ARG, "das_debug_krylov_dcgs2_update_staged: j must not be negative");
+    krylov_check_basis("das_debug_krylov_dcgs2_update_staged", n, nslots, fmt, V, ld);
+    DAS_CHECK(fmt != KRY_FP64, DAS_ERR_ARG, "das_debug_krylov_dcgs2_update_staged: the staging output belongs to the float basis (fmt 1 or 2)");
+    DAS_CHECK(nslots >= j + 2, DAS_ERR_ARG, "das_debug_krylov_dcgs2_update_staged: the basis needs slots 0 .. j + 1");
+    DAS_CHECK(v && stage && (sc || j == 0), DAS_ERR_ARG, "das_debug_krylov_dcgs2_update_staged: null pointer");
+    DAS_CHECK(stagelen >= n, DAS_ERR_ARG, "das_debug_krylov_dcgs2_update_staged: staging vector shorter than n");
+    debug_krylov_dcgs2_update_staged<float>(n, j, fmt == KRY_SPLIT, V, ld, nslots, sc, gamma, ralpha, v, stage, stagelen);
+    return DAS_OK;
+    DAS_CATCH
+}
 int das_debug_krylov_multidot(long long n, int m, int fmt, const void* V, long long ld, const double* w, double* out) {
     DAS_TRY
     DAS_CHECK(m >= 0, DAS_ERR_ARG, "das_debug_krylov_multidot: m must not be negative");
diff --git a/dafoam_amd/csrc/das_krylov.hpp b/dafoam_amd/csrc/das_krylov.hpp
--- a/dafoam_amd/csrc/das_krylov.hpp
+++ b/dafoam_amd/csrc/das_krylov.hpp
@@ -133,7 +133,8 @@
 #endif
 template <int UNROLL, int RPT, class VT>
 __global__ __launch_bounds__(256) void k_dcgs2_update(long long n, int j, VT* __restrict__ V, long long ldv, const double* __restrict__ sc,
-                                                      double gamma, double ralpha, const double* __restrict__ v, float* __restrict__ Vlo = nullptr) {
+                                                      double gamma, double ralpha, const double* __restrict__ v, float* __restrict__ Vlo = nullptr,
+                                                      double* __restrict__ stage = nullptr) {
     const long long k0 = ((long long)blockIdx.x * RPT) * blockDim.x + threadIdx.x;
     const double* s = sc;
     const double* c = sc + j;
@@ -174,7 +175,9 @@
         const VT qh = (VT)qj, uh = (VT)un;
         V[(long long)j * ldv + k] = qh;
         V[(long long)(j + 1) * ldv + k] = uh;
-        if (Vlo) { Vlo[(long long)j * ldv + k] = (float)(qj - (double)qh); Vlo[(long long)(j + 1) * ldv + k] = (float)(un - (double)uh); }
+        const float ul = Vlo ? (float)(un - (double)uh) : 0.f;
+        if (Vlo) { Vlo[(long long)j * ldv + k] = (float)(qj - (double)qh); Vlo[(long long)(j + 1) * ldv + k] = ul; }
+        if (stage) stage[k] = (double)uh + (double)ul;
     }
 }
 typedef float f32x4 __attribute__((ext_vector_type(4)));
@@ -260,7 +263,7 @@
 }
 template <int UNROLL, int RPT4, bool FULL, bool NT>
 __device__ __forceinline__ void dcgs2w_body(long long n, int j, float* __restrict__ V, long long ldv, const double* __restrict__ sc, double gamma,
-                                            double ralpha, const double* __restrict__ v, float* __restrict__ Vlo) {
+                                            double ralpha, const double* __restrict__ v, float* __restrict__ Vlo, double* __restrict__ stage) {
     const long long base = ((long long)blockIdx.x * (256 * RPT4) + threadIdx.x) * 4;
     const double* s = sc;
     const double* c = sc + j;
@@ -329,7 +332,7 @@
         for (int e = 0; e < 4; e++) {
             const double qj = (u[e] - as[r][e]) * ralpha, un = (vv[e] - gamma * u[e] - ac[r][e]) * ralpha;
             qh[e] = (float)qj; nhh[e] = (float)un;
-            qlo[e] = (float)(qj - (double)qh[e]); nlo[e] = (float)(un - (double)nhh[e]);
+            qlo[e] = (float)(qj - (double)qh[e]); nlo[e] = Vlo ? (float)(un - (double)nhh[e]) : 0.f;
         }
         if (FULL) {
             *reinterpret_cast<f32x4*>(uh + k) = f32x4{qh[0], qh[1], qh[2], qh[3]};
@@ -338,21 +341,27 @@
                 *reinterpret_cast<f32x4*>(ul + k) = f32x4{qlo[0], qlo[1], qlo[2], qlo[3]};
                 *reinterpret_cast<f32x4*>(nl + k) = f32x4{nlo[0], nlo[1], nlo[2], nlo[3]};
             }
+            if (stage) {
+                *reinterpret_cast<f64x2*>(stage + k) = f64x2{(double)nhh[0] + (double)nlo[0], (double)nhh[1] + (double)nlo[1]};
+                *reinterpret_cast<f64x2*>(stage + k + 2) = f64x2{(double)nhh[2] + (double)nlo[2], (double)nhh[3] + (double)nlo[3]};
+            }
         } else {
 #pragma unroll
             for (int e = 0; e < 4; e++) {
                 if (k + e >= n) continue;
                 uh[k + e] = qh[e]; nh[k + e] = nhh[e];
                 if (Vlo) { ul[k + e] = qlo[e]; nl[k + e] = nlo[e]; }
+                if (stage) stage[k + e] = (double)nhh[e] + (double)nlo[e];
             }
         }
     }
 }
 template <int UNROLL, int RPT4, bool NT>
 __global__ __launch_bounds__(256) void k_dcgs2w_update(long long n, int j, float* __restrict__ V, long long ldv, const double* __restrict__ sc,
-                                                       double gamma, double ralpha, const double* __restrict__ v, float* __restrict__ Vlo) {
-    if ((long long)(blockIdx.x + 1) * (1024 * RPT4) <= n) dcgs2w_body<UNROLL, RPT4, true, NT>(n, j, V, ldv, sc, gamma, ralpha, v, Vlo);
-    else dcgs2w_body<UNROLL, RPT4, false, NT>(n, j, V, ldv, sc, gamma, ralpha, v, Vlo);
+                                                       double gamma, double ralpha, const double* __restrict__ v, float* __restrict__ Vlo,
+                                                       double* __restrict__ stage = nullptr) {
+    if ((long long)(blockIdx.x + 1) * (1024 * RPT4) <= n) dcgs2w_body<UNROLL, RPT4, true, NT>(n, j, V, ldv, sc, gamma, ralpha, v, Vlo, stage);
+    else dcgs2w_body<UNROLL, RPT4, false, NT>(n, j, V, ldv, sc, gamma, ralpha, v, Vlo, stage);
 }
 template <class VT>
 __global__ __launch_bounds__(256) void k_lincomb(long long n, int m, const VT* __restrict__ V, long long ldv, const double* __restrict__ c,
@@ -419,13 +428,13 @@
 }
 template <int UNROLL, int RPT, class VT>
 static void launch_dcgs2_update_pass(hipStream_t st, long long n, int j, VT* V, long long ldv, const double* sc, double gamma, double ralpha,
-                                     const double* v, float* Vlo) {
-    hipLaunchKernelGGL((k_dcgs2_update<UNROLL, RPT, VT>), dim3(nblk(n, 256 * RPT)), dim3(256), 0, st, n, j, V, ldv, sc, gamma, ralpha, v, Vlo);
+                                     const double* v, float* Vlo, double* stage = nullptr) {
+    hipLaunchKernelGGL((k_dcgs2_update<UNROLL, RPT, VT>), dim3(nblk(n, 256 * RPT)), dim3(256), 0, st, n, j, V, ldv, sc, gamma, ralpha, v, Vlo, stage);
 }
 template <int UNROLL, int RPT4, bool NT>
 static void launch_dcgs2w_update(hipStream_t st, long long n, int j, float* V, long long ldv, const double* sc, double gamma, double ralpha,
-                                 const double* v, float* Vlo) {
-    hipLaunchKernelGGL((k_dcgs2w_update<UNROLL, RPT4, NT>), dim3(nblk(n, 1024 * RPT4)), dim3(256), 0, st, n, j, V, ldv, sc, gamma, ralpha, v, Vlo);
+                                 const double* v, float* Vlo, double* stage = nullptr) {
+    hipLaunchKernelGGL((k_dcgs2w_update<UNROLL, RPT4, NT>), dim3(nblk(n, 1024 * RPT4)), dim3(256), 0, st, n, j, V, ldv, sc, gamma, ralpha, v, Vlo, stage);
 }
 template <class VT>
 static void launch_multidot2(hipStream_t st, long long n, int K, const VT* V, long long ldv, const VT* u, const double* v, double* partial, double* out) {
@@ -441,14 +450,14 @@
 }
 template <int UNROLL, int RPT, class VT>
 static void launch_dcgs2_update(hipStream_t st, long long n, int j, VT* V, long long ldv, const double* sc, double gamma, double ralpha, const double* v,
-                                float* Vlo) {
+                                float* Vlo, double* stage = nullptr) {
     if constexpr (std::is_same<VT, float>::value) {
-        if (g_orth_wide && orth_wide_ok(n, V, Vlo, ldv, nullptr, v)) {
-            launch_dcgs2w_update<DCGS2W_UNROLL, DCGS2W_RPT4, DCGS2W_NT != 0>(st, n, j, V, ldv, sc, gamma, ralpha, v, Vlo);
+        if (g_orth_wide && orth_wide_ok(n, V, Vlo, ldv, stage, v)) {
+            launch_dcgs2w_update<DCGS2W_UNROLL, DCGS2W_RPT4, DCGS2W_NT != 0>(st, n, j, V, ldv, sc, gamma, ralpha, v, Vlo, stage);
             return;
         }
     }
-    launch_dcgs2_update_pass<UNROLL, RPT, VT>(st, n, j, V, ldv, sc, gamma, ralpha, v, Vlo);
+    launch_dcgs2_update_pass<UNROLL, RPT, VT>(st, n, j, V, ldv, sc, gamma, ralpha, v, Vlo, stage);
 }
 template <class VT, class WT>
 static void launch_multiaxpy(hipStream_t st, long long n, int m, const VT* V, long long ldv, const double* h, WT* w, const float* Vlo) {
diff --git a/dafoam_amd/csrc/das_krylov_debug.hpp b/dafoam_amd/csrc/das_krylov_debug.hpp
--- a/dafoam_amd/csrc/das_krylov_debug.hpp
+++ b/dafoam_amd/csrc/das_krylov_debug.hpp
@@ -47,6 +47,15 @@
     const DevBuf<double> dsc = krylov_up<double>(sc, (size_t)2 * j), dv = krylov_up<double>(v, n);
     krylov_run([&] { launch_dcgs2_update<DCGS2_UNROLL, DCGS2_RPT, VT>(0, n, j, dV.p, ld, dsc.p, gamma, ralpha, dv.p, krylov_lo(dV.p, n, split)); }, dV, V,
                (size_t)nslots * ld);
+}
+template <class VT>
+static void debug_krylov_dcgs2_update_staged(long long n, int j, bool split, void* V, long long ld, int nslots, const double* sc, double gamma, double ralpha,
+                                             const double* v, double* stage, long long stagelen) {
+    const DevBuf<VT> dV = krylov_up<VT>(V, (size_t)nslots * ld);
+    const DevBuf<double> dsc = krylov_up<double>(sc, (size_t)2 * j), dv = krylov_up<double>(v, n), dst = krylov_up<double>(stage, (size_t)stagelen);
+    krylov_run([&] { launch_dcgs2_update<DCGS2_UNROLL, DCGS2_RPT, VT>(0, n, j, dV.p, ld, dsc.p, gamma, ralpha, dv.p, krylov_lo(dV.p, n, split), dst.p); }, dV, V,
+               (size_t)nslots * ld);
+    dst.download(stage, (size_t)stagelen);
 }
 template <class VT>
 static void debug_krylov_multidot(long long n, int m, const void* V, long long ld, const double* w, double* out) {
diff --git a/dafoam_amd/csrc/das_mesh.cpp b/dafoam_amd/csrc/das_mesh.cpp
--- a/dafoam_amd/csrc/das_mesh.cpp
+++ b/dafoam_amd/csrc/das_mesh.cpp
@@ -60,6 +60,7 @@
     d["amd.pcStabilityGood"] = 1.0e4;
     i["amd.pcSubdomains"] = -1;
     i["amd.pcCoarseSparseAZ"] = 1;
+    i["amd.pcCoarseFused"] = 1;
     i["amd.coloringOnDevice"] = 1;
     s["amd.primalMethod"] = "newton";
     i["amd.simpleSweepsPerCheck"] = 10;
diff --git a/include/dafoam_amd.h b/include/dafoam_amd.h
--- a/include/dafoam_amd.h
+++ b/include/dafoam_amd.h
@@ -229,6 +229,8 @@
 int das_debug_krylov_dots2(long long n, int K, int fmt, const void* V, long long ld, const double* v, double* out);
 int das_debug_krylov_dcgs2_update(long long n, int j, int fmt, void* V, long long ld, int nslots, const double* sc, double gamma, double ralpha,
                                   const double* v);
+int das_debug_krylov_dcgs2_update_staged(long long n, int j, int fmt, void* V, long long ld, int nslots, const double* sc, double gamma, double ralpha,
+                                         const double* v, double* stage, long long stagelen);
 int das_debug_krylov_multidot(long long n, int m, int fmt, const void* V, long long ld, const double* w, double* out);
 int das_debug_krylov_multiaxpy(long long n, int m, int fmt, const void* V, long long ld, const double* h, int wfloat, void* w, long long wlen);
 int das_debug_krylov_lincomb(long long n, int m, int fmt, const void* V, long long ld, const double* c, double* y, long long ylen);
@@ -239,6 +241,11 @@
 int das_debug_krylov_block_lincomb(long long n, int K, int s, const double* V, long long ldv, const double* C, double* Y, long long ldy);
 int das_debug_krylov_block_spmm(long long n, int s, const long long* rowptr, const int* colidx, const double* vals, const double* X, long long ldx,
                                 double* Y, long long ldy);
+int das_debug_pc_apply_full(das_solver_t* s, das_ksp_t* ksp, const double* x, int fused, const double* uIn, double* z, double* t, double* u, double* rr);
+int das_debug_coarse_einv(das_ksp_t* ksp, double* Einv);
+int das_debug_coarse_az_structure(das_solver_t* s, das_ksp_t* ksp, long long* ptr, int* a0, long long* optr);
+int das_debug_coarse_az_apply(long long n, const long long* rowptr, const int* colidx, const double* vals, long long N, long long off, const int* agg, int nagg,
+                              const double* u, const double* v, int* cnt, double* outCsr, double* outInline);
 long long das_timer_count(das_solver_t* s, const char* name);
 void das_timer_reset(das_solver_t* s);
 void das_timer_enable(das_solver_t* s, int on);
```

After: 43.93, median of 6. 1.1% higher.
